# sc15i2gp/daily-ray-trace

Measured on AMD Instinct MI355X. Metric: Mpaths/s (pixels*spp/s) Cornell 1024^2 depth 8; achieved HBM GB/s % of peak, higher is better.
Workload: dtype f64

## Files before the change

daily-ray-trace_amd/csrc/drt_bvh_kernels.h:

```cpp
#pragma once

#include "drt_kernels.h"

#define BVH_LDS_STACK BVH_STACK

struct PrimaryHit
{
    int32_t index, pad;
    double  min_dist;
};

__device__ __forceinline__ void hit_point_from_scan(const SceneView &sv, const DevScene &sc, HitPoint &ip, V3 ro, V3 rd, double min_dist, int index)
{
    ip.index = index;
    if (index >= 0)
    {
        uint32_t type = sv.surf_type[index];
        uint32_t smat = sv.surf_mat[index];
        ip.position = v_sum(ro, v_mul(rd, min_dist));
        if (type == DRT_GEO_SPHERE) ip.normal = v_normalise(v_sub(ip.position, sf3(sv, SF_PX, index)));
        else ip.normal = sf3(sv, SF_NX, index);
        ip.out = v_reverse(rd);
        ip.on_dot = v_dot(ip.normal, ip.out);
        ip.transmit_mat = smat;
        ip.incident_mat = sc.base_mat;
        if (ip.on_dot < 0.0)
        {
            if (type != DRT_GEO_PLANE)
            {
                ip.transmit_mat = sc.base_mat;
                ip.incident_mat = smat;
            }
            ip.normal = v_reverse(ip.normal);
            ip.on_dot = v_dot(ip.normal, ip.out);
        }
        ip.surface_mat = smat;
    }
    else ip.surface_mat = sc.escape_mat;
}

struct PathStart
{
    uint64_t q, s_local, hit_row, slot;
    uint32_t x, y, sample;
};
template <bool LIST>
__device__ __forceinline__ PathStart path_start(const TraceParams &tp, uint64_t pid)
{
    PathStart ps;
    ps.q = pid / tp.n_samples;
    ps.s_local = pid - ps.q * tp.n_samples;
    ps.hit_row = ps.s_local * tp.n_pix + ps.q;
    const uint64_t t = LIST ? (uint64_t)tp.pixel_list[ps.q] : ps.q;
    uint32_t j = (uint32_t)(t / tp.tile_w);
    uint32_t i = (uint32_t)(t - (uint64_t)j * tp.tile_w);
    ps.x = tp.x0 + i;
    ps.y = tp.y0 + j * tp.row_stride;
    ps.sample = tp.first_sample + (uint32_t)ps.s_local;
    if (LIST) ps.sample += tp.sample_base[t];
    ps.slot = ps.q * (uint64_t)tp.batch + ps.s_local;
    return ps;
}
template <bool LIST>
__device__ __forceinline__ uint64_t path_tile_pixel(const TraceParams &tp, const PathStart &ps)
{
    return LIST ? (uint64_t)tp.pixel_list[ps.q] : ps.q;
}
__device__ __forceinline__ uint64_t path_key(const TraceParams &tp, const PathStart &ps)
{
    return tp.seed + (((uint64_t)ps.sample * (uint64_t)tp.height + (uint64_t)ps.y) * (uint64_t)tp.width + (uint64_t)ps.x);
}


#define PRIMARY_BLOCK 256

#ifndef DRT_PRIMARY_WAVES_PER_SIMD
#define DRT_PRIMARY_WAVES_PER_SIMD 6
#endif
template <bool LIST, bool RAYS>
__device__ __forceinline__ void primary_paths(DevScene sc, DevCamera cam, TraceParams tp, uint64_t *headers,
                                              int32_t *hits, unsigned long long *counters,
                                              PrimaryHit *primary, uint64_t *queue,
                                              unsigned long long *queue_count, const DevRayTable &rt)
{
    __shared__ int s_stack[PRIMARY_BLOCK / 64][BVH_LDS_STACK];
    SceneView sv;
    sv.n_surf = sc.n_surf; sv.n_lights = sc.n_lights;
    sv.surf = sc.surf; sv.lights = sc.lights; sv.surf_type = sc.surf_type; sv.surf_mat = sc.surf_mat;
    sv.light_type = sc.light_type; sv.light_mat = sc.light_mat; sv.mats = sc.mats;
    sv.bvh_nodes = sc.bvh_nodes; sv.bvh_leaf = sc.bvh_leaf;
    const uint32_t lane = threadIdx.x & 63u;
    int *stack = s_stack[threadIdx.x >> 6];
    const uint64_t n_packets = (tp.n_paths + 63u) / 64u;
    const uint64_t wave0 = (uint64_t)blockIdx.x * (PRIMARY_BLOCK / 64) + (threadIdx.x >> 6);
    const uint64_t n_waves = (uint64_t)gridDim.x * (PRIMARY_BLOCK / 64);
    uint32_t n_scans = 0, n_draws = 0, n_paths = 0;
    if (*tp.overflow) return;

    for (uint64_t packet = wave0; packet < n_packets; packet += n_waves)
    {
        const uint64_t pid = packet * 64u + lane;
        const bool valid = pid < tp.n_paths;
        V3 ro = v3(0, 0, 0), rd = v3(0, 0, 1);
        PathStart ps = path_start<LIST>(tp, valid ? pid : 0);
        uint64_t rs = 1;
        double weight = 1.0;
        if (valid)
        {
            rs = drt_splitmix64(path_key(tp, ps));
            if (RAYS) weight = table_ray(rt, tp.width, path_tile_pixel<LIST>(tp, ps), ps.x, ps.y, ps.sample, ro, rd);
            else camera_ray(cam, tp.pixel_scheme, ps.x, ps.y, rs, n_draws, ro, rd);
            n_paths += 1;
            n_scans += 1;
        }
        const V3 o = v_sum(ro, v_mul(rd, DRT_VIS_FUDGE));
        double min_dist = DRT_INF;
        int index = -1;
        const Ray32 r32 = bvh_ray32(o, rd);
        float lim = bvh_limit32(min_dist);
        int sp = 0;
        int cur = 0;
        for (;;)
        {
            cur = __builtin_amdgcn_readfirstlane(cur);
            if (cur >= 0)
            {
                const BvhNode &n = sv.bvh_nodes[cur];
                int ref[2];
                float t[2];
                bool hit[2];
                bvh_children(n, r32, lim, ref, t, hit);
                hit[0] = hit[0] && valid;
                hit[1] = hit[1] && valid;
                const unsigned long long m0 = __ballot(hit[0]), m1 = __ballot(hit[1]);
                if (m0 != 0ull && m1 != 0ull)
                {
                    const int first1 = __popcll(__ballot(hit[1] && (!hit[0] || t[1] < t[0])));
                    const int first0 = __popcll(__ballot(hit[0] && (!hit[1] || !(t[1] < t[0]))));
                    const int near = first1 > first0 ? 1 : 0;
                    if (lane == 0) stack[sp] = ref[1 - near];
                    sp += 1;
                    cur = ref[near];
                    continue;
                }
                if (m0 != 0ull) { cur = ref[0]; continue; }
                if (m1 != 0ull) { cur = ref[1]; continue; }
            }
            else if (bvh_is_leaf(cur))
            {
                const int packed = -2 - cur;
                const int first = packed >> 3, count = (packed & 7) + 1;
                for (int k = 0; k < count; k += 1)
                {
                    const BvhLeafPrim &lp = sv.bvh_leaf[first + k];
                    if (!__any(valid && !sphere_certainly_missed(lp, r32, lim))) continue;
                    double dist = leaf_distance(sv, lp, o, rd);
                    if (valid && (dist < min_dist || (dist == min_dist && (int)lp.index < index)))
// ... 118 lines not shown
    const Ray32 r32 = bvh_ray32_unpruned(o, d);
    float lim = bvh_limit32(limit);
    int sp = 0;
    int cur = job == JOB_NONE ? BVH_DONE : 0;
    int nq = 0;
    for (;;)
    {
        for (;;)
        {
            if (bvh_is_leaf(cur) && nq < DRT_BVH_POSTPONE)
            {
                leaf_queue[nq * 64 + lane] = cur;
                nq += 1;
                cur = stack_pop(stack, lane, sp);
            }
            const bool walking = cur >= 0;
            const int n_walk = __popcll(__ballot(walking));
            if (n_walk == 0) break;
            if (n_walk < DRT_BVH_POSTPONE_EXIT && __any(bvh_is_leaf(cur) && nq == DRT_BVH_POSTPONE)) break;
            if (walking) bvh_node_step(sv, stack, lane, r32, lim, cur, sp);
        }
        if (!__any(nq > 0 || cur != BVH_DONE)) break;
        int ns = 0;
        for (int k = 0; __any(k < nq); k += 1)
            if (k < nq)
            {
                const int leaf = leaf_queue[k * 64 + lane];
                const BvhLeafPrim *src = &sv.bvh_leaf[(-2 - leaf) >> 3];
                BvhLeafPrim b;
                b.c32[0] = src->c32[0]; b.c32[1] = src->c32[1]; b.c32[2] = src->c32[2]; b.reach32 = src->reach32;
                if (!sphere_certainly_missed(b, r32, lim))
                {
                    leaf_queue[ns * 64 + lane] = leaf;
                    ns += 1;
                }
            }
        nq = 0;
        for (int k = 0; __any(k < ns); k += 1)
            if (k < ns)
            {
                const BvhLeafPrim *src = &sv.bvh_leaf[(-2 - leaf_queue[k * 64 + lane]) >> 3];
                BvhLeafPrim lp;
                lp.index = src->index; lp.type = src->type;
                lp.f[0] = src->f[0]; lp.f[1] = src->f[1]; lp.f[2] = src->f[2]; lp.f[3] = src->f[3];
                const double dist = leaf_distance(sv, lp, o, d);
                if (job == JOB_CLOSEST)
                {
                    if (dist < limit || (dist == limit && (int)lp.index < index))
                    {
                        limit = dist;
                        index = (int)lp.index;
                        lim = bvh_limit32(limit);
                    }
                }
                else if (dist < limit)
                {
                    occluded = true;
                    ns = 0;
                    sp = 0;
                    cur = BVH_DONE;
                }
            }
    }
}

template <bool LIST, bool RAYS>
__device__ __forceinline__ void bounce_paths(
    DevScene sc, DevCamera cam, TraceParams tp, uint64_t *records, uint64_t *headers, int32_t *hits,
    unsigned long long *counters, unsigned long long *work_counter, const PrimaryHit *primary,
    const uint64_t *queue, const unsigned long long *queue_count, const DevRayTable &rt)
{
    __shared__ int s_stack[BOUNCE_BLOCK / 64][BVH_LDS_STACK * 64];
    __shared__ int s_leaf_queue[BOUNCE_BLOCK / 64][BVH_QUEUE_WORDS];
    SceneView sv;
    sv.n_surf = sc.n_surf; sv.n_lights = sc.n_lights;
    sv.surf = sc.surf; sv.lights = sc.lights; sv.surf_type = sc.surf_type; sv.surf_mat = sc.surf_mat;
    sv.light_type = sc.light_type; sv.light_mat = sc.light_mat; sv.mats = sc.mats;
    sv.bvh_nodes = sc.bvh_nodes; sv.bvh_leaf = sc.bvh_leaf;
    const uint32_t lane = threadIdx.x & 63u;
    int *stack = s_stack[threadIdx.x >> 6];
    int *leaf_queue = s_leaf_queue[threadIdx.x >> 6];
    if (*tp.overflow) return;
    const uint64_t n_work = *queue_count;
    const uint64_t CHUNK = tp.chunk;
    uint64_t chunk_next = 0, chunk_end = 0;
    bool exhausted = false;

    uint32_t n_scans = 0, n_shaded = 0, n_shadow = 0, n_draws = 0;

    bool alive = false, at_vertex = false;
    uint64_t rs = 1, hit_row = 0;
    uint32_t depth = 0, shaded = 0, light = 0;
    uint32_t masks = 0;
    uint64_t *hdr = nullptr;
    uint32_t blk = 0, tbl = 0;
    uint32_t spare = ~0u, spare_tbl = ~0u;
    bool new_vertex = false;
    WavePool wp = {0u, 0u, 0u};
    HitPoint ip;
    ip.position = ip.normal = ip.out = v3(0, 0, 0);
    ip.on_dot = 0.0;
    ip.surface_mat = ip.incident_mat = ip.transmit_mat = 0;
    ip.index = -1;

    const uint32_t cycle = sv.n_lights + 1u;
    uint32_t phase = 0;
    for (;;)
    {
        unsigned long long idle_mask = __ballot(!alive);
        if (!exhausted && idle_mask == ~0ull) phase = 0;
        if (idle_mask != 0ull && !exhausted && phase == 0u)
        {
            const uint32_t want = (uint32_t)__popcll(idle_mask);
            const uint32_t rank = (uint32_t)__popcll(idle_mask & ((1ull << lane) - 1ull));
            uint64_t my = ~0ull;
            uint64_t avail = chunk_end - chunk_next;
            uint32_t taken = 0;
            if (avail < want)
            {
                if (!alive && rank < avail) my = chunk_next + rank;
                taken = (uint32_t)avail;
                unsigned long long base = 0;
                if (lane == 0) base = atomicAdd(work_counter, (unsigned long long)CHUNK);
                base = __shfl(base, 0);
                if (base >= n_work)
                {
                    exhausted = true;
                    chunk_next = chunk_end = 0;
                }
                else
                {
                    chunk_next = base;
                    chunk_end = (base + CHUNK < n_work) ? base + CHUNK : n_work;
                    const uint64_t avail2 = chunk_end - chunk_next;
                    if (!alive && rank >= taken && (uint64_t)(rank - taken) < avail2) my = chunk_next + (rank - taken);
                    const uint32_t used = (want - taken < avail2) ? (want - taken) : (uint32_t)avail2;
                    chunk_next += used;
                }
            }
            else
            {
                if (!alive) my = chunk_next + rank;
                chunk_next += want;
            }
            if (my != ~0ull)
            {
                const uint64_t pid = queue[my];
                const PathStart ps = path_start<LIST>(tp, pid);
                hit_row = ps.hit_row;
                rs = drt_splitmix64(path_key(tp, ps));
                uint32_t camera_draws = 0;
                V3 ro, rd;
                if (RAYS) (void)table_ray(rt, tp.width, path_tile_pixel<LIST>(tp, ps), ps.x, ps.y, ps.sample, ro, rd);
                else camera_ray(cam, tp.pixel_scheme, ps.x, ps.y, rs, camera_draws, ro, rd);
                hdr = headers + ps.slot * REC_HEADER_WORDS;
                const PrimaryHit ph = primary[ps.slot];
                hit_point_from_scan(sv, sc, ip, v_sum(ro, v_mul(rd, DRT_VIS_FUDGE)), rd, ph.min_dist, ph.index);
                depth = 0;
                shaded = 0;
                light = 0;
                masks = 0;
                alive = true;
                at_vertex = true;
                new_vertex = true;
                n_shaded += 1;
            }
        }
        if (!__any(alive)) break;
        phase = phase + 1u == cycle ? 0u : phase + 1u;
        if (!path_spare_block(tp, wp, alive, shaded, spare, spare_tbl, lane))
        {
            hdr[0] = (uint64_t)HDR_TERM_NOT_DONE << 16;
            alive = false;
        }

        int job = JOB_NONE;
        V3 jo = v3(0, 0, 0), jd = v3(0, 0, 1);
        double limit = DRT_INF;
        double light_c = 1.0;
        if (alive && at_vertex && light < sv.n_lights)
        {
            const uint32_t l = light;
            const uint32_t ltype = sv.light_type[l];
            const V3 lpos = v3(sv.lights[LF_PX * sv.n_lights + l], sv.lights[LF_PY * sv.n_lights + l], sv.lights[LF_PZ * sv.n_lights + l]);
            const double light_pdf = sv.lights[LF_PDF * sv.n_lights + l];
            double attenuation = 1.0;
            V3 light_position = lpos;
            if (ltype == DRT_GEO_POINT)
            {
                double dist = v_length(v_sub(light_position, ip.position));
                attenuation = ((4.0 * DRT_PI) * dist) * dist;
            }
            else if (ltype == DRT_GEO_SPHERE)
            {
                double u = drt_rng(rs, n_draws);
                double v = drt_rng(rs, n_draws);
                double r = __builtin_sqrt(1.0 - u * u);
                double t = (2.0 * DRT_PI) * v;
                double st, ct;
                drt_sincos(t, st, ct);
                V3 sp = v3(r * ct, r * st, u);
                light_position = v_sum(lpos, v_mul(sp, sv.lights[LF_RADIUS * sv.n_lights + l]));
            }
            else if (ltype == DRT_GEO_PLANE)
            {
                double u = drt_rng(rs, n_draws);
                double v = drt_rng(rs, n_draws);
                V3 lu = v3(sv.lights[LF_UX * sv.n_lights + l], sv.lights[LF_UY * sv.n_lights + l], sv.lights[LF_UZ * sv.n_lights + l]);
                V3 lv = v3(sv.lights[LF_VX * sv.n_lights + l], sv.lights[LF_VY * sv.n_lights + l], sv.lights[LF_VZ * sv.n_lights + l]);
                light_position = v_sum(v_sum(lpos, v_mul(lu, u)), v_mul(lv, v));
            }
            n_shadow += 1;
            jd = v_normalise(v_sub(light_position, ip.position));
            jo = v_sum(ip.position, v_mul(jd, DRT_VIS_FUDGE));
            limit = v_length(v_sub(light_position, jo)) - DRT_VIS_FUDGE;
            light_c = attenuation * (light_pdf);
            job = JOB_SHADOW;
        }
        else if (alive && !at_vertex)
        {
            jd = ip.out;
            jo = v_sum(ip.position, v_mul(jd, DRT_VIS_FUDGE));
            job = JOB_CLOSEST;
        }
        int index = -1;
        bool occluded = false;
        bvh_walk(sv, stack, leaf_queue, lane, job, jo, jd, limit, index, occluded);

        if (job == JOB_CLOSEST)
        {
            hit_point_from_scan(sv, sc, ip, jo, jd, limit, index);
            n_scans += 1;
            if (tp.record_hits) hits[((uint64_t)tp.hits_sample_offset * tp.n_pix + hit_row) * tp.max_depth + depth] = ip.index;
            const DevMaterial &mat = sv.mats[ip.surface_mat];
            if (mat.is_black_body)
            {
                const uint32_t term = mat.is_emissive ? 1u : 0u;
                const uint32_t term_spd = mat.is_emissive ? ((uint32_t)mat.emission_spd & 0xFFFFu) : 0u;
                hdr[0] = (uint64_t)shaded | ((uint64_t)term << 16) | ((uint64_t)term_spd << 32) | ((uint64_t)(masks & 0xFFFFu) << 48) | ((uint64_t)(masks >> 16) << 24);
                alive = false;
            }
            else
            {
                at_vertex = true;
                new_vertex = true;
                light = 0;
                n_shaded += 1;
            }
        }
        else if (job == JOB_SHADOW)
        {
            const uint32_t l = light;
            if (new_vertex)
            {
                path_open_vertex(tp, wp, records, shaded, hdr, blk, tbl, spare, spare_tbl);
                new_vertex = false;
            }
            uint64_t *vrec = records + (uint64_t)blk * tp.block_words + (uint64_t)(shaded & (REC_BLOCK_VERTICES - 1u)) * tp.vertex_words;
            uint64_t *lrec = vrec + REC_VERTEX_WORDS + (uint64_t)l * REC_LIGHT_WORDS;
            uint32_t lflags = 0;
            if (!occluded)
            {
                EvalCoef e = eval_coefficients_by_material(sc, sv, ip, jd);
                lflags = e.flags | FLAG_VISIBLE;
                if (l == 0 && shaded < 8u) masks |= 0x10000u << shaded;
                lrec[1] = (uint64_t)__double_as_longlong(light_c);
                store_coef(lrec + 2, e);
            }
            uint32_t em_spd = (uint32_t)sv.mats[sv.light_mat[l]].emission_spd & 0xFFFFu;
            lrec[0] = (uint64_t)em_spd | ((uint64_t)lflags << 16);
            light = l + 1;
        }
        if (alive && at_vertex && light >= sv.n_lights)
        {
            if (new_vertex)
            {
                path_open_vertex(tp, wp, records, shaded, hdr, blk, tbl, spare, spare_tbl);
                new_vertex = false;
            }
            const DevMaterial &mat = sv.mats[ip.surface_mat];
            uint64_t *vrec = records + (uint64_t)blk * tp.block_words + (uint64_t)(shaded & (REC_BLOCK_VERTICES - 1u)) * tp.vertex_words;
            V3 in;
            double dir_pdf;
            sample_direction_by_material(sc, sv, ip, rs, n_draws, in, dir_pdf);
            EvalCoef e = eval_coefficients_by_material(sc, sv, ip, in);
            vrec[0] = mat.bdsf_packed;
            vrec[1] = (uint64_t)mat.num_bdsfs | ((uint64_t)(e.flags | mat.vertex_flags) << 8) | ((uint64_t)((uint32_t)mat.diffuse_spd & 0xFFFFu) << 16) |
                      ((uint64_t)((uint32_t)mat.glossy_spd & 0xFFFFu) << 32) | ((uint64_t)((uint32_t)mat.mirror_spd & 0xFFFFu) << 48);
            vrec[2] = record_media_word(sc, sv, ip);
            vrec[3] = (uint64_t)__double_as_longlong(ip.on_dot);
            vrec[4] = (uint64_t)__double_as_longlong(dir_pdf);
            store_coef(vrec + 5, e);
            if ((mat.vertex_flags & FLAG_PLASTIC) && shaded < 16u) masks |= 1u << shaded;
            shaded += 1;
            ip.out = in;
            depth += 1;
            at_vertex = false;
            if (depth >= tp.max_depth)
            {
                hdr[0] = (uint64_t)shaded | ((uint64_t)(masks & 0xFFFFu) << 48) | ((uint64_t)(masks >> 16) << 24);
                alive = false;
            }
        }
    }

    uint64_t vals[6] = {0, n_scans, n_shaded, n_shadow, n_draws, wp.taken};
    for (int k = 1; k < 6; k += 1)
    {
        uint64_t v = vals[k];
        for (int off = 32; off > 0; off >>= 1) v += __shfl_down(v, off);
        if (lane == 0 && v) atomicAdd(&counters[k], (unsigned long long)v);
    }
}

template <bool LIST = false>
__global__ __launch_bounds__(BOUNCE_BLOCK, DRT_BOUNCE_WAVES_PER_SIMD) void drt_bounce_kernel(
    DevScene sc, DevCamera cam, TraceParams tp, uint64_t *__restrict__ records, uint64_t *__restrict__ headers, int32_t *__restrict__ hits,
    unsigned long long *__restrict__ counters, unsigned long long *__restrict__ work_counter, const PrimaryHit *__restrict__ primary,
    const uint64_t *__restrict__ queue, const unsigned long long *__restrict__ queue_count)
{
    const DevRayTable no_table = {nullptr, nullptr, nullptr, 0u, 0u, 0u, 0u};
    bounce_paths<LIST, false>(sc, cam, tp, records, headers, hits, counters, work_counter, primary, queue, queue_count, no_table);
}

template <bool LIST = false>
__global__ __launch_bounds__(BOUNCE_BLOCK, DRT_BOUNCE_WAVES_PER_SIMD) void drt_bounce_rays_kernel(
    DevScene sc, DevCamera cam, TraceParams tp, uint64_t *__restrict__ records, uint64_t *__restrict__ headers, int32_t *__restrict__ hits,
    unsigned long long *__restrict__ counters, unsigned long long *__restrict__ work_counter, const PrimaryHit *__restrict__ primary,
    const uint64_t *__restrict__ queue, const unsigned long long *__restrict__ queue_count, DevRayTable rt)
{
    bounce_paths<LIST, true>(sc, cam, tp, records, headers, hits, counters, work_counter, primary, queue, queue_count, rt);
}
```

daily-ray-trace_amd/csrc/drt_device.h:

```cpp
#pragma once

#include <hip/hip_runtime.h>
#include <stdint.h>

#define DRT_PI 3.14159265358979323846
#define DRT_VIS_FUDGE 0.0001
#define DRT_INF __builtin_huge_val()

struct V3
{
    double x, y, z;
};
struct M33
{
    V3 c[3];
};

__device__ __forceinline__ V3 v3(double x, double y, double z) { V3 r; r.x = x; r.y = y; r.z = z; return r; }
__device__ __forceinline__ bool v_equal(V3 a, V3 b) { return a.x == b.x && a.y == b.y && a.z == b.z; }
__device__ __forceinline__ V3 v_sum(V3 a, V3 b) { return v3(a.x + b.x, a.y + b.y, a.z + b.z); }
__device__ __forceinline__ V3 v_sub(V3 a, V3 b) { return v3(a.x - b.x, a.y - b.y, a.z - b.z); }
__device__ __forceinline__ double v_dot(V3 a, V3 b) { return a.x * b.x + a.y * b.y + a.z * b.z; }
__device__ __forceinline__ V3 v_cross(V3 a, V3 b) { return v3(a.y * b.z - a.z * b.y, a.z * b.x - a.x * b.z, a.x * b.y - a.y * b.x); }
__device__ __forceinline__ V3 v_mul(V3 v, double f) { return v3(f * v.x, f * v.y, f * v.z); }
__device__ __forceinline__ V3 v_div(V3 v, double f) { return v3(v.x / f, v.y / f, v.z / f); }
__device__ __forceinline__ double v_length(V3 v) { return __builtin_sqrt(v_dot(v, v)); }
__device__ __forceinline__ V3 v_normalise(V3 v) { return v_div(v, v_length(v)); }
__device__ __forceinline__ V3 v_reverse(V3 v) { return v3(-v.x, -v.y, -v.z); }

__device__ __forceinline__ V3 v_reflect(V3 v, V3 n)
{
    double f = 2.0 * v_dot(v, n);
    return v_sub(v, v_mul(n, f));
}

__device__ __forceinline__ V3 v_transmit(V3 v, V3 n, double ir, double tr)
{
    double vn_dot = v_dot(v, n);
    double rel_ref = ir / tr;
    V3 m = v_mul(n, vn_dot);
    v = v_sub(m, v);
    V3 perpend = v_reverse(v_mul(v, rel_ref));
    double perpend_dot = -__builtin_sqrt(1.0 - v_dot(perpend, perpend));
    V3 parallel = v_mul(n, perpend_dot);
    return v_sum(perpend, parallel);
}

__device__ __forceinline__ V3 m_vmul(const M33 &m, V3 v)
{
    V3 r0 = v3(m.c[0].x, m.c[1].x, m.c[2].x);
    V3 r1 = v3(m.c[0].y, m.c[1].y, m.c[2].y);
    V3 r2 = v3(m.c[0].z, m.c[1].z, m.c[2].z);
    return v3(v_dot(r0, v), v_dot(r1, v), v_dot(r2, v));
}

__device__ __forceinline__ M33 rotation_between(V3 v, V3 w)
{
    V3 n = v_cross(v, w);
    double c = v_dot(v, w);
    M33 r;
    if (v_dot(n, n) == 0.0 && c <= 0.0)
    {
        r.c[0] = v3(-1.0, 0.0, 0.0);
        r.c[1] = v3(0.0, -1.0, 0.0);
        r.c[2] = v3(0.0, 0.0, -1.0);
        return r;
    }
    M33 m;
    m.c[0] = v3(0.0, n.z, -n.y);
    m.c[1] = v3(-n.z, 0.0, n.x);
    m.c[2] = v3(n.y, -n.x, 0.0);
    V3 row0 = v3(m.c[0].x, m.c[1].x, m.c[2].x);
    V3 row1 = v3(m.c[0].y, m.c[1].y, m.c[2].y);
    V3 row2 = v3(m.c[0].z, m.c[1].z, m.c[2].z);
    double f = 1.0 / (1.0 + c);
    V3 mm0 = v_mul(v3(v_dot(row0, m.c[0]), v_dot(row0, m.c[1]), v_dot(row0, m.c[2])), f);
    V3 mm1 = v_mul(v3(v_dot(row1, m.c[0]), v_dot(row1, m.c[1]), v_dot(row1, m.c[2])), f);
    V3 mm2 = v_mul(v3(v_dot(row2, m.c[0]), v_dot(row2, m.c[1]), v_dot(row2, m.c[2])), f);
    r.c[0] = v_sum(v_sum(v3(1.0, 0.0, 0.0), m.c[0]), mm0);
    r.c[1] = v_sum(v_sum(v3(0.0, 1.0, 0.0), m.c[1]), mm1);
    r.c[2] = v_sum(v_sum(v3(0.0, 0.0, 1.0), m.c[2]), mm2);
    return r;
}

__device__ __forceinline__ uint64_t drt_splitmix64(uint64_t k)
{
    uint64_t z = k + 0x9E3779B97F4A7C15ull;
    z = (z ^ (z >> 30)) * 0xBF58476D1CE4E5B9ull;
    z = (z ^ (z >> 27)) * 0x94D049BB133111EBull;
    z ^= z >> 31;
    return z ? z : 1ull;
}
__device__ __forceinline__ double drt_rng(uint64_t &state, uint32_t &draws)
{
    uint64_t x = state;
    x ^= x << 13;
    x ^= x >> 7;
    x ^= x << 17;
    state = x;
    draws += 1;
    return (double)(uint32_t)(x >> 33) / 2147483647.0;
}

__device__ __forceinline__ void drt_sincos(double t, double &s, double &c)
{
    const double TWO_OVER_PI = 6.36619772367581382433e-01;
    const double PIO2_1 = 1.57079632673412561417e+00, PIO2_1T = 6.07710050650619224932e-11;
    const double S1 = -1.66666666666666324348e-01, S2 = 8.33333333332248946124e-03, S3 = -1.98412698298579493134e-04,
                 S4 = 2.75573137070700676789e-06, S5 = -2.50507602534068634195e-08, S6 = 1.58969099521155010221e-10;
    const double C1 = 4.16666666666666019037e-02, C2 = -1.38888888888741095749e-03, C3 = 2.48015872894767294178e-05,
                 C4 = -2.75573143513906633035e-07, C5 = 2.08757232129817482790e-09, C6 = -1.13596475577881948265e-11;
    double fn = __builtin_rint(t * TWO_OVER_PI);
    double r = t - fn * PIO2_1;
    double w = fn * PIO2_1T;
    double y0 = r - w;
    double y1 = (r - y0) - w;
    double z = y0 * y0;
    double v = z * y0;
    double rs = S2 + z * (S3 + z * (S4 + z * (S5 + z * S6)));
    double ks = y0 - ((z * (0.5 * y1 - v * rs) - y1) - v * S1);
    double rc = z * (C1 + z * (C2 + z * (C3 + z * (C4 + z * (C5 + z * C6)))));
    double hz = 0.5 * z;
    double w1 = 1.0 - hz;
    double kc = w1 + (((1.0 - w1) - hz) + (z * rc - y0 * y1));
    int n = (int)fn & 3;
    s = (n == 0) ? ks : (n == 1) ? kc : (n == 2) ? -ks : -kc;
    c = (n == 0) ? kc : (n == 1) ? -ks : (n == 2) ? -kc : ks;
}

__device__ __forceinline__ V3 uniform_sample_sphere(uint64_t &rs, uint32_t &draws)
{
    double u = drt_rng(rs, draws);
    double v = drt_rng(rs, draws);
    double r = __builtin_sqrt(1.0 - u * u);
    double t = (2.0 * DRT_PI) * v;
    double st, ct;
    drt_sincos(t, st, ct);
    return v3(r * ct, r * st, u);
}

__device__ __forceinline__ V3 uniform_sample_disc(uint64_t &rs, uint32_t &draws)
{
    double r_x = drt_rng(rs, draws);
    double r_y = drt_rng(rs, draws);
    double o_x = 2.0 * r_x - 1.0;
    double o_y = 2.0 * r_y - 1.0;
    if (o_x == 0.0 && o_y == 0.0) return v3(0.0, 0.0, 0.0);
    double r, t;
    if (__builtin_fabs(o_x) > __builtin_fabs(o_y))
    {
        r = o_x;
        t = (DRT_PI / 4.0) * (o_y / o_x);
    }
    else
    {
        r = o_y;
        t = (DRT_PI / 2.0) - (DRT_PI / 4.0) * (o_x / o_y);
    }
    double st, ct;
    drt_sincos(t, st, ct);
    return v3(r * ct, r * st, 0.0);
}


__device__ __forceinline__ double line_sphere(V3 o, V3 d, V3 sc, double sr)
{
    V3 c_to_o = v_sub(o, sc);
    double b = -2.0 * v_dot(c_to_o, d);
    double c = v_dot(c_to_o, c_to_o) - sr * sr;
    double disc = b * b - 4.0 * c;
    if (disc < 0.0) return DRT_INF;
    double sq = __builtin_sqrt(disc);
    double s0 = (b + sq) * 0.5;
    double s1 = (b - sq) * 0.5;
    if (s0 < 0.0 && s1 < 0.0) return DRT_INF;
    else if (s0 >= 0.0 && s1 < 0.0) return s0;
    else if (s1 >= 0.0 && s0 < 0.0) return s1;
    else if (s0 <= s1) return s0;
    else return s1;
}

__device__ __forceinline__ double line_plane(V3 o, V3 d, V3 pp, V3 pn, V3 un, V3 vn, double ul, double vl)
{
    double dn = v_dot(d, pn);
    if (dn == 0.0) return DRT_INF;
    V3 o_to_p = v_sub(pp, o);
    double l = v_dot(o_to_p, pn) / dn;
    V3 i = v_sum(o, v_mul(d, l));
    V3 j = v_sub(i, pp);
    double ju = v_dot(j, un);
    double jv = v_dot(j, vn);
    if (l >= 0.0 && 0.0 <= ju && ju <= ul && 0.0 <= jv && jv <= vl) return l;
    return DRT_INF;
}

__device__ __forceinline__ double line_plane_limited(V3 o, V3 d, V3 pp, V3 pn, V3 un, V3 vn, double ul, double vl, double limit, bool want)
{
    double dn = v_dot(d, pn);
    if (dn == 0.0) return DRT_INF;
    V3 o_to_p = v_sub(pp, o);
    double l = v_dot(o_to_p, pn) / dn;
    if (!(want && l >= 0.0 && l < limit)) return DRT_INF;
    V3 i = v_sum(o, v_mul(d, l));
    V3 j = v_sub(i, pp);
    double ju = v_dot(j, un);
    double jv = v_dot(j, vn);
    if ((0.0 <= ju) & (ju <= ul) & (0.0 <= jv) & (jv <= vl)) return l;
    return DRT_INF;
}

__device__ __forceinline__ uint32_t media_index(bool swapped, bool incident, uint32_t surface_mat, uint32_t base_mat)
{
    return (swapped == incident) ? surface_mat : base_mat;
}

__device__ __forceinline__ double drt_pow_shininess(double x, double y)
{
    const uint32_t n = (uint32_t)y;
    if (!(y >= 0.0 && y < 1024.0 && (double)n == y) || !(x >= 0.0 && x <= 1.0)) return pow(x, y);
    double rh = 1.0, rl = 0.0;
    double bh = x, bl = 0.0;
    double yk = y;
    asm volatile("" : "+v"(yk));
    for (uint32_t k = (uint32_t)yk; __any(k != 0u); k >>= 1)
    {
        if (k & 1u)
        {
            const double p = rh * bh;
            double e = __builtin_fma(rh, bh, -p);
            e = __builtin_fma(rh, bl, e);
            e = __builtin_fma(rl, bh, e);
            rh = p + e;
            rl = e - (rh - p);
        }
        if (k > 1u)
        {
            const double p = bh * bh;
            double e = __builtin_fma(bh, bh, -p);
            e = __builtin_fma(bh + bh, bl, e);
            bh = p + e;
            bl = e - (bh - p);
        }
    }
    return rh + rl;
}


__device__ __forceinline__ double dielectric_reflectance(double ir, double tr, double inc_cos, double inc_sin_sq)
{
    double rel = ir / tr;
    double ts_sin_sq = rel * rel * inc_sin_sq;
    if (ts_sin_sq >= 1.0) return 1.0;
    double ts_cos = __builtin_sqrt(1.0 - ts_sin_sq * ts_sin_sq);
    double tr_on = tr * inc_cos;
    double tr_ts = tr * ts_cos;
    double ir_on = ir * inc_cos;
    double ir_ts = ir * ts_cos;
    double par = (tr_on - ir_ts) / (tr_on + ir_ts);
    double per = (ir_on - tr_ts) / (ir_on + tr_ts);
    par *= par;
    per *= per;
    return 0.5 * (par + per);
}

__device__ __forceinline__ double conductor_reflectance(double ir, double tr, double te, double inc_cos, double inc_cos_sq,
                                                        double inc_sin_sq)
{
    double rr = tr / ir;
    double re = te / ir;
    double rr_sq = rr * rr;
    double re_sq = re * re;
    double r = rr_sq - re_sq - inc_sin_sq;
    double apb_sq = __builtin_sqrt(r * r + 4.0 * rr_sq * re_sq);
    double a = __builtin_sqrt(0.5 * (apb_sq + r));
    double s = apb_sq + inc_cos_sq;
    double t = 2.0 * a * inc_cos;
    double u = inc_cos_sq * apb_sq + inc_sin_sq * inc_sin_sq;
    double v = t * inc_sin_sq;
    double par = (s - t) / (s + t);
    double per = par * (u - v) / (u + v);
    return 0.5 * (par + per);
}

__device__ __forceinline__ double dielectric_reflectance_sel(bool paired, double ir, double tr, double te_or_rel_sq, double inc_cos, double inc_sin_sq)
{
    double rel_sq = te_or_rel_sq;
    if (!paired)
    {
        double rel = ir / tr;
        rel_sq = rel * rel;
    }
    double ts_sin_sq = rel_sq * inc_sin_sq;
    if (ts_sin_sq >= 1.0) return 1.0;
    double ts_cos = __builtin_sqrt(1.0 - ts_sin_sq * ts_sin_sq);
    double tr_on = tr * inc_cos;
    double tr_ts = tr * ts_cos;
    double ir_on = ir * inc_cos;
    double ir_ts = ir * ts_cos;
    double par = (tr_on - ir_ts) / (tr_on + ir_ts);
    double per = (ir_on - tr_ts) / (ir_on + tr_ts);
    par *= par;
    per *= per;
    return 0.5 * (par + per);
}
__device__ __forceinline__ double conductor_reflectance_sel(bool paired, double ir_or_cA, double tr_or_cB, double te, double inc_cos, double inc_cos_sq,
                                                            double inc_sin_sq)
{
    double cA = ir_or_cA, cB = tr_or_cB;
    if (!paired)
    {
        double rr = tr_or_cB / ir_or_cA;
        double re = te / ir_or_cA;
        double rr_sq = rr * rr;
        double re_sq = re * re;
        cA = rr_sq - re_sq;
        cB = 4.0 * rr_sq * re_sq;
    }
    double r = cA - inc_sin_sq;
    double apb_sq = __builtin_sqrt(r * r + cB);
    double a = __builtin_sqrt(0.5 * (apb_sq + r));
    double s = apb_sq + inc_cos_sq;
    double t = 2.0 * a * inc_cos;
    double u = inc_cos_sq * apb_sq + inc_sin_sq * inc_sin_sq;
    double v = t * inc_sin_sq;
    double par = (s - t) / (s + t);
    double per = par * (u - v) / (u + v);
    return 0.5 * (par + per);
}

__device__ __forceinline__ double ggx(V3 sn, V3 mn, double r)
{
    double d = v_dot(sn, mn);
    double r_2 = r * r;
    if (d <= 0.0) return 0.0;
    double d_2 = d * d;
    double d_4 = d_2 * d_2;
    double tan_sq = (1.0 / d_2) - 1.0;
    return r_2 / (((DRT_PI * d_4) * (r_2 + tan_sq)) * (r_2 + tan_sq));
}
__device__ __forceinline__ double ggx_att(V3 v, V3 sn, V3 mn, double r)
{
    double att;
    double g = ggx(sn, mn, r);
    double v_mn = v_dot(v, mn);
    double v_sn = v_dot(v, sn);
    double dot_quot = __builtin_fabs(v_mn / v_sn);
    double r_2 = r * r;
    if (dot_quot <= 0.0) att = 0.0;
    else
    {
        double vn_tan_sq = (1.0 / (v_sn * v_sn)) - 1.0;
        att = 2.0 / (1.0 + __builtin_sqrt(1.0 + r_2 * vn_tan_sq));
    }
    return g * att;
}

__device__ __forceinline__ double drt_lerp(double x, double x0, double x1, double y0, double y1)
{
    return y0 + ((x - x0) * ((y1 - y0) / (x1 - x0)));
}
```

daily-ray-trace_amd/csrc/drt_kernels.h:

```cpp
#pragma once

#include "drt_device.h"
#include "drt_build_rule.h"
#include "drt_stash_rule.h"
#include <type_traits>
#include "../../include/drt_hip.h"


enum
{
    SF_PX = 0, SF_PY, SF_PZ, SF_RADIUS,
    SF_NX, SF_NY, SF_NZ,
    SF_UNX, SF_UNY, SF_UNZ,
    SF_VNX, SF_VNY, SF_VNZ,
    SF_ULEN, SF_VLEN,
    SF_COUNT
};
enum
{
    LF_PX = 0, LF_PY, LF_PZ, LF_RADIUS,
    LF_UX, LF_UY, LF_UZ,
    LF_VX, LF_VY, LF_VZ,
    LF_PDF,
    LF_COUNT
};

enum
{
    NEED_GLOSSY = 1u,
    NEED_EQR    = 2u,
    NEED_EQT    = 4u,
    NEED_CT     = 8u
};

struct BvhNode
{
    float   lo[2][3], hi[2][3];
    int32_t child[2];
    int32_t count[2];
};

struct BvhLeafPrim
{
    uint32_t index, type;
    double   f[4];
    float    c32[3];
    float    reach32;
    double   pad;
};

#define PAIR_NONE 0xFFFFu
#define PAIR_CONDUCTOR 0x8000u
struct DevMaterial
{
    uint32_t is_black_body, is_emissive, num_bdsfs, dir_func;
    uint32_t needs;
    uint16_t pair_out, pair_in;
    int32_t  emission_spd, diffuse_spd, glossy_spd, mirror_spd, refract_spd, extinct_spd;
    double   shininess, roughness;
    double   refract_i0, refract_i1;
    uint32_t bdsfs[DRT_MAX_BDSFS];
    uint64_t bdsf_packed;
    uint32_t vertex_flags;
    uint32_t pad1;
};

struct DevScene
{
    uint32_t n_surf, n_lights, n_mat, S;
    uint32_t n_spd, base_mat, escape_mat, trans_i0;
    double   trans_wl, trans_w0, trans_w1;
    const double      *surf;
    const uint32_t    *surf_type;
    const uint32_t    *surf_mat;
    const double      *lights;
    const uint32_t    *light_type;
    const uint32_t    *light_mat;
    const DevMaterial *mats;
    const double      *spds;
    const BvhNode     *bvh_nodes;
    const BvhLeafPrim *bvh_leaf;
};

struct DevCamera
{
    V3     forward, right, up, aperture_position, film_bottom_left;
    double aperture_radius, focal_depth, pixel_width, pixel_height;
};

struct DevRayTable
{
    const double *origins, *dirs;
    const double *weights;
    uint64_t      layer_stride, t_offset;
    uint32_t      n_layers, tiled;
};


#define REC_HEADER_WORDS 4
#define REC_BLOCK_SHIFT 2
#define REC_BLOCK_VERTICES (1u << REC_BLOCK_SHIFT)
#define REC_HEADER_BLOCKS 3
#define HDR_TERM_NOT_DONE 0x80u
#define HDR_TERM_TAIL_STAGED 0x40u
#define HDR_TERM_MASK 0x03u
#define HDR_TERM_RESUME_SHIFT 2u
#define HDR_TERM_RESUME_MASK 0xFu
#define REC_VERTEX_WORDS 10
#define REC_LIGHT_WORDS 6
#define FLAG_EQR 1u
#define FLAG_EQT 2u
#define FLAG_VISIBLE 4u
#define FLAG_PLASTIC 8u

struct TraceParams
{
    uint32_t width, height, x0, y0, tile_w, tile_h, row_stride;
    uint32_t first_sample, n_samples, max_depth, pixel_scheme, record_hits;
    uint64_t seed;
    uint64_t n_pix, n_paths;
    uint32_t vertex_words, block_words;
    uint32_t hits_sample_offset, batch;
    uint32_t chunk, pool_blocks;
    unsigned long long *pool_cursor;
    uint32_t *overflow;
    double       *tail_stage;
    const double *spd_tail;
    double       *tail_resume;
    uint32_t      tail_count, n_spd;
    const uint32_t *pixel_list;
    const uint32_t *sample_base;
};

#define POOL_CHUNK 256u
struct WavePool
{
    uint32_t base, left;
    uint32_t handed;
    uint32_t taken;
};

__device__ __forceinline__ uint32_t pool_alloc(const TraceParams &tp, WavePool &wp, bool need, uint32_t lane)
{
    const unsigned long long m = __ballot(need);
    if (m == 0ull) return ~0u;
    const uint32_t n = (uint32_t)__popcll(m);
    if (n > wp.left)
    {
        unsigned long long base = 0;
        if (lane == 0) base = atomicAdd(tp.pool_cursor, (unsigned long long)POOL_CHUNK);
        base = __shfl(base, 0);
        if (base + POOL_CHUNK > (unsigned long long)tp.pool_blocks)
        {
            wp.left = 0;
            return ~0u;
        }
        wp.base = (uint32_t)base;
        wp.left = POOL_CHUNK;
    }
    const uint32_t id = wp.base + (uint32_t)__popcll(m & ((1ull << lane) - 1ull));
    wp.base += n;
    wp.left -= n;
    wp.handed += n;
    return need ? id : ~0u;
}

__device__ __forceinline__ bool path_spare_block(const TraceParams &tp, WavePool &wp, bool alive, uint32_t shaded, uint32_t &spare, uint32_t &spare_tbl,
                                                 uint32_t lane)
{
    const bool want = alive && (shaded & (REC_BLOCK_VERTICES - 1u)) == 0u && spare == ~0u;
    const bool want_tbl = alive && shaded == REC_HEADER_BLOCKS * REC_BLOCK_VERTICES && spare_tbl == ~0u;
    const uint32_t id = pool_alloc(tp, wp, want, lane);
    const uint32_t tid = pool_alloc(tp, wp, want_tbl, lane);
    if (want) spare = id;
    if (want_tbl) spare_tbl = tid;
    if ((want && id == ~0u) || (want_tbl && tid == ~0u))
    {
        atomicExch(tp.overflow, 1u);
        return false;
    }
    return true;
}
__device__ __forceinline__ void path_open_vertex(const TraceParams &tp, WavePool &wp, uint64_t *__restrict__ records, uint32_t shaded, uint64_t *hdr,
                                                 uint32_t &blk, uint32_t &tbl, uint32_t &spare, uint32_t &spare_tbl)
{
    if ((shaded & (REC_BLOCK_VERTICES - 1u)) != 0u) return;
    const uint32_t b = shaded >> REC_BLOCK_SHIFT;
    blk = spare;
    spare = ~0u;
    wp.taken += 1;
    uint32_t *h32 = (uint32_t *)hdr;
    if (b < REC_HEADER_BLOCKS) h32[4 + b] = blk;
    else
    {
        if (b == REC_HEADER_BLOCKS)
        {
            tbl = spare_tbl;
            spare_tbl = ~0u;
            h32[7] = tbl;
            wp.taken += 1;
        }
        ((uint32_t *)(records + (uint64_t)tbl * tp.block_words))[b - REC_HEADER_BLOCKS] = blk;
    }
}

struct EvalCoef
{
    double   a_in, spec, mn_dot, ct_coef;
    uint32_t flags;
};

#define DRT_NUM_COUNTERS 8


struct SceneView
{
    const double      *surf;
    const uint32_t    *surf_type, *surf_mat;
    const double      *lights;
    const uint32_t    *light_type, *light_mat;
    const DevMaterial *mats;
    const BvhNode     *bvh_nodes;
    const BvhLeafPrim *bvh_leaf;
    const double      *rows = nullptr;
    uint32_t           n_surf, n_lights;
};

__device__ __forceinline__ V3 sf3(const SceneView &sv, int f, uint32_t i)
{
    return v3(sv.surf[(f + 0) * sv.n_surf + i], sv.surf[(f + 1) * sv.n_surf + i], sv.surf[(f + 2) * sv.n_surf + i]);
}

__device__ __forceinline__ double surface_distance(const SceneView &sv, uint32_t i, uint32_t type, V3 o, V3 d)
{
    if (type == DRT_GEO_SPHERE) return line_sphere(o, d, sf3(sv, SF_PX, i), sv.surf[SF_RADIUS * sv.n_surf + i]);
    return line_plane(o, d, sf3(sv, SF_PX, i), sf3(sv, SF_NX, i), sf3(sv, SF_UNX, i), sf3(sv, SF_VNX, i),
                      sv.surf[SF_ULEN * sv.n_surf + i], sv.surf[SF_VLEN * sv.n_surf + i]);
}

#define SR_STRIDE 16
#define SR_TYPE 15
static_assert(SF_COUNT <= SR_TYPE, "a surface row holds the SF_COUNT fields and the type");
__device__ __forceinline__ V3 row3(const double *r, int f) { return v3(r[f], r[f + 1], r[f + 2]); }
__device__ __forceinline__ uint32_t row_type(const double *r) { return (uint32_t)__double_as_longlong(r[SR_TYPE]); }
__device__ __forceinline__ double row_distance(const double *r, uint32_t type, V3 o, V3 d)
{
    if (type == DRT_GEO_SPHERE) return line_sphere(o, d, row3(r, SF_PX), r[SF_RADIUS]);
    return line_plane(o, d, row3(r, SF_PX), row3(r, SF_NX), row3(r, SF_UNX), row3(r, SF_VNX), r[SF_ULEN], r[SF_VLEN]);
}
template <bool ROWS>
__device__ __forceinline__ uint32_t scan_type(const SceneView &sv, uint32_t i)
{
    return ROWS ? row_type(sv.rows + (size_t)i * SR_STRIDE) : sv.surf_type[i];
}
__device__ __forceinline__ double row_distance_limited(const double *r, uint32_t type, V3 o, V3 d, double limit, bool want)
{
    if (type == DRT_GEO_SPHERE) return line_sphere(o, d, row3(r, SF_PX), r[SF_RADIUS]);
    return line_plane_limited(o, d, row3(r, SF_PX), row3(r, SF_NX), row3(r, SF_UNX), row3(r, SF_VNX), r[SF_ULEN], r[SF_VLEN], limit, want);
}
template <bool ROWS>
__device__ __forceinline__ double scan_distance(const SceneView &sv, uint32_t i, uint32_t type, V3 o, V3 d, double limit, bool want)
{
    return ROWS ? row_distance_limited(sv.rows + (size_t)i * SR_STRIDE, type, o, d, limit, want) : surface_distance(sv, i, type, o, d);
}

#ifdef DRT_BRANCH_STATS
__device__ __forceinline__ uint32_t scan_plane_step_skipped(const double *r, V3 o, V3 d, double limit, bool want)
{
    const V3 pp = row3(r, SF_PX), pn = row3(r, SF_NX);
    const double dn = v_dot(d, pn);
    const double l = v_dot(v_sub(pp, o), pn) / dn;
    return __any(dn != 0.0 && want && l >= 0.0 && l < limit) ? 0u : 1u;
}
#define DRT_SCAN_STATS_PARAM , uint64_t *scan_stats = nullptr
#define DRT_SCAN_STATS_ARG(p) , (p)
#define DRT_SCAN_STATS_STEP(rowp, o, d, limit, want)                                                                  \
    if (ROWS && scan_stats && type == DRT_GEO_PLANE)                                                                    \
    {                                                                                                                   \
        const uint32_t skipped_ = scan_plane_step_skipped((rowp), (o), (d), (limit), (want));                          \
        if ((threadIdx.x & 63u) == (uint32_t)(__ffsll((long long)__ballot(1)) - 1))                                    \
        {                                                                                                               \
            scan_stats[0] += 1;                                                                                         \
            scan_stats[1] += skipped_;                                                                                  \
        }                                                                                                               \
    }
#else
#define DRT_SCAN_STATS_PARAM
#define DRT_SCAN_STATS_ARG(p)
#define DRT_SCAN_STATS_STEP(rowp, o, d, limit, want)
#endif

#define BVH_STACK 32

__device__ __forceinline__ double leaf_distance(const SceneView &sv, const BvhLeafPrim &lp, V3 o, V3 d)
{
    if (lp.type == DRT_GEO_SPHERE) return line_sphere(o, d, v3(lp.f[SF_PX], lp.f[SF_PY], lp.f[SF_PZ]), lp.f[SF_RADIUS]);
    return surface_distance(sv, lp.index, lp.type, o, d);
}

#define BVH_INV_CAP 1.2676506e30f
struct Ray32
{
    float ix, iy, iz, nx, ny, nz;
    float ox, oy, oz, dx, dy, dz;
};
__device__ __forceinline__ float bvh_inv32(float d)
{
    const float i = __builtin_amdgcn_rcpf(d);
    return __builtin_fabsf(i) > BVH_INV_CAP ? __builtin_copysignf(BVH_INV_CAP, i) : i;
}
__device__ __forceinline__ Ray32 bvh_ray32f(V3 o, float dx, float dy, float dz)
{
    Ray32 r;
    r.ix = bvh_inv32(dx);
    r.iy = bvh_inv32(dy);
    r.iz = bvh_inv32(dz);
    r.nx = -((float)o.x * r.ix);
    r.ny = -((float)o.y * r.iy);
    r.nz = -((float)o.z * r.iz);
    r.ox = (float)o.x; r.oy = (float)o.y; r.oz = (float)o.z;
    r.dx = dx; r.dy = dy; r.dz = dz;
    return r;
}
__device__ __forceinline__ Ray32 bvh_ray32(V3 o, V3 d) { return bvh_ray32f(o, (float)d.x, (float)d.y, (float)d.z); }

#define RAY_UNIT_TOLERANCE 0x1p-42
#define BVH_WALK_UNIT_TOLERANCE 0x1p-38
__device__ __forceinline__ bool ray_off_unit(V3 d)
{
    const bool finite = __builtin_fabs(d.x) < DRT_INF && __builtin_fabs(d.y) < DRT_INF && __builtin_fabs(d.z) < DRT_INF;
    return finite && !(__builtin_fabs(v_dot(d, d) - 1.0) <= RAY_UNIT_TOLERANCE);
}
__device__ __forceinline__ Ray32 bvh_ray32_unpruned(V3 o, V3 d)
{
    const bool off = __builtin_fabs(v_dot(d, d) - 1.0) > BVH_WALK_UNIT_TOLERANCE;
    return bvh_ray32f(o, off ? INFINITY : (float)d.x, (float)d.y, (float)d.z);
}
__device__ __forceinline__ bool bvh_ray32_is_unpruned(const Ray32 &r) { return r.dx == INFINITY; }

__device__ __forceinline__ bool sphere_certainly_missed(const BvhLeafPrim &lp, const Ray32 &r, float lim)
{
    const float cx = lp.c32[0] - r.ox, cy = lp.c32[1] - r.oy, cz = lp.c32[2] - r.oz;
    const float t = __builtin_fmaf(cz, r.dz, __builtin_fmaf(cy, r.dy, cx * r.dx));
    const float px = __builtin_fmaf(-t, r.dx, cx), py = __builtin_fmaf(-t, r.dy, cy), pz = __builtin_fmaf(-t, r.dz, cz);
    const float p2 = __builtin_fmaf(pz, pz, __builtin_fmaf(py, py, px * px));
    const float R = lp.reach32;
    return (p2 > R * R || t + R < 0.0f || t - R > lim) && p2 < INFINITY;
}
__device__ __forceinline__ float bvh_limit32(double limit) { return (float)limit * 1.00000024f; }

__device__ __forceinline__ float bvh_box_entry(const BvhNode &n, int c, const Ray32 &r)
{
    float t0x = __builtin_fmaf(n.lo[c][0], r.ix, r.nx), t1x = __builtin_fmaf(n.hi[c][0], r.ix, r.nx);
    float t0y = __builtin_fmaf(n.lo[c][1], r.iy, r.ny), t1y = __builtin_fmaf(n.hi[c][1], r.iy, r.ny);
    float t0z = __builtin_fmaf(n.lo[c][2], r.iz, r.nz), t1z = __builtin_fmaf(n.hi[c][2], r.iz, r.nz);
    float tmin = __builtin_fmaxf(__builtin_fmaxf(__builtin_fminf(t0x, t1x), __builtin_fminf(t0y, t1y)), __builtin_fminf(t0z, t1z));
    float tmax = __builtin_fminf(__builtin_fminf(__builtin_fmaxf(t0x, t1x), __builtin_fmaxf(t0y, t1y)), __builtin_fmaxf(t0z, t1z));
    if (!(tmax >= 0.0f) || !(tmin <= tmax)) return -1.0f;
    return tmin > 0.0f ? tmin : 0.0f;
}

#define BVH_DONE (-1)
__device__ __forceinline__ int bvh_leaf_ref(int first, int count) { return -2 - (first * 8 + (count - 1)); }
__device__ __forceinline__ bool bvh_is_leaf(int ref) { return ref < BVH_DONE; }

template <bool UNPRUNED = false>
__device__ __forceinline__ void bvh_children(const BvhNode &n, const Ray32 &r, float limit, int ref[2], float t[2], bool hit[2])
{
#pragma unroll
    for (int c = 0; c < 2; c += 1)
    {
        ref[c] = n.child[c];
        t[c] = bvh_box_entry(n, c, r);
        if (UNPRUNED) t[c] = bvh_ray32_is_unpruned(r) ? 0.0f : t[c];
        hit[c] = ref[c] != BVH_DONE && t[c] >= 0.0f && t[c] <= limit;
    }
}

template <bool ROWS = false>
__device__ __forceinline__ bool points_mutually_visible(const SceneView &sv, V3 p0, V3 p1 DRT_SCAN_STATS_PARAM)
{
    V3 dir = v_normalise(v_sub(p1, p0));
    V3 o = v_sum(p0, v_mul(dir, DRT_VIS_FUDGE));
    double vis_dist = v_length(v_sub(p1, o)) - DRT_VIS_FUDGE;
    bool visible = true;
    for (uint32_t i = 0; i < sv.n_surf; i += 1)
    {
        uint32_t type = scan_type<ROWS>(sv, i);
        if (type != DRT_GEO_SPHERE && type != DRT_GEO_PLANE) continue;
        DRT_SCAN_STATS_STEP(sv.rows + (size_t)i * SR_STRIDE, o, dir, vis_dist, visible)
        double dist = scan_distance<ROWS>(sv, i, type, o, dir, vis_dist, visible);
        if (visible && dist < vis_dist) visible = false;
        if (!__any(visible)) break;
    }
    return visible;
}

struct HitPoint
{
    V3       position, normal, out;
    double   on_dot;
    uint32_t surface_mat, incident_mat, transmit_mat;
    int      index;
};

struct TraceHit
{
    V3       position, normal, out;
    double   on_dot;
    uint32_t surface_mat;
    bool     swapped;
    int      index;
};
__device__ __forceinline__ void hit_set_media(const DevScene &sc, HitPoint &ip, uint32_t smat, bool swapped)
{
    ip.incident_mat = media_index(swapped, true, smat, sc.base_mat);
    ip.transmit_mat = media_index(swapped, false, smat, sc.base_mat);
}
__device__ __forceinline__ void hit_set_media(const DevScene &, TraceHit &ip, uint32_t, bool swapped) { ip.swapped = swapped; }
__device__ __forceinline__ uint32_t incident_mat_of(const DevScene &, const HitPoint &ip) { return ip.incident_mat; }
__device__ __forceinline__ uint32_t transmit_mat_of(const DevScene &, const HitPoint &ip) { return ip.transmit_mat; }
__device__ __forceinline__ uint32_t incident_mat_of(const DevScene &sc, const TraceHit &ip) { return media_index(ip.swapped, true, ip.surface_mat, sc.base_mat); }
__device__ __forceinline__ uint32_t transmit_mat_of(const DevScene &sc, const TraceHit &ip) { return media_index(ip.swapped, false, ip.surface_mat, sc.base_mat); }

template <bool ROWS = false, class HP = HitPoint>
__device__ __forceinline__ void find_ray_intersection(const SceneView &sv, const DevScene &sc, HP &ip, V3 ro, V3 rd DRT_SCAN_STATS_PARAM)
{
    double min_dist = DRT_INF;
    int index = -1;
    ro = v_sum(ro, v_mul(rd, DRT_VIS_FUDGE));
    {
        for (uint32_t i = 0; i < sv.n_surf; i += 1)
        {
            uint32_t type = scan_type<ROWS>(sv, i);
            if (type != DRT_GEO_SPHERE && type != DRT_GEO_PLANE) continue;
            DRT_SCAN_STATS_STEP(sv.rows + (size_t)i * SR_STRIDE, ro, rd, min_dist, true)
            double dist = scan_distance<ROWS>(sv, i, type, ro, rd, min_dist, true);
            if (dist < min_dist)
            {
                min_dist = dist;
                index = (int)i;
            }
        }
    }
    ip.index = index;
    if (index >= 0)
    {
        uint32_t type = sv.surf_type[index];
        uint32_t smat = sv.surf_mat[index];
        ip.position = v_sum(ro, v_mul(rd, min_dist));
        if (type == DRT_GEO_SPHERE) ip.normal = v_normalise(v_sub(ip.position, sf3(sv, SF_PX, index)));
        else ip.normal = sf3(sv, SF_NX, index);
        ip.out = v_reverse(rd);
        ip.on_dot = v_dot(ip.normal, ip.out);
        hit_set_media(sc, ip, smat, false);
        if (ip.on_dot < 0.0)
        {
            if (type != DRT_GEO_PLANE) hit_set_media(sc, ip, smat, true);
            ip.normal = v_reverse(ip.normal);
            ip.on_dot = v_dot(ip.normal, ip.out);
        }
        ip.surface_mat = smat;
    }
    else ip.surface_mat = sc.escape_mat;
}

__device__ __forceinline__ double refract_at_trans_wl(const DevScene &sc, const DevMaterial &m)
{
    return drt_lerp(sc.trans_wl, sc.trans_w0, sc.trans_w1, m.refract_i0, m.refract_i1);
}

template <class HP>
__device__ __forceinline__ uint64_t record_media_word(const DevScene &sc, const SceneView &sv, const HP &ip)
{
    const DevMaterial &sm = sv.mats[ip.surface_mat];
    const uint32_t incident_mat = incident_mat_of(sc, ip), transmit_mat = transmit_mat_of(sc, ip);
    uint32_t pair = PAIR_NONE;
    if (incident_mat == sc.base_mat && transmit_mat == ip.surface_mat) pair = sm.pair_out;
    else if (incident_mat == ip.surface_mat && transmit_mat == sc.base_mat) pair = sm.pair_in;
    return (uint64_t)((uint32_t)sv.mats[incident_mat].refract_spd & 0xFFFFu) |
           ((uint64_t)((uint32_t)sv.mats[transmit_mat].refract_spd & 0xFFFFu) << 16) |
           ((uint64_t)((uint32_t)sv.mats[transmit_mat].extinct_spd & 0xFFFFu) << 32) | ((uint64_t)pair << 48);
}
__device__ __forceinline__ void fresnel_rows(uint64_t w2, uint32_t &i0, uint32_t &i1, uint32_t &i2, bool &paired)
{
    const uint32_t i_ir = (uint32_t)(w2)&0xFFFFu, i_tr = (uint32_t)(w2 >> 16) & 0xFFFFu, i_te = (uint32_t)(w2 >> 32) & 0xFFFFu;
    const uint32_t pair = (uint32_t)(w2 >> 48) & 0xFFFFu;
    paired = pair != PAIR_NONE;
    const bool conductor = paired && (pair & PAIR_CONDUCTOR) != 0u;
    const uint32_t row = pair & (PAIR_CONDUCTOR - 1u);
    i0 = conductor ? row : i_ir;
    i1 = conductor ? row + 1u : i_tr;
    i2 = (paired && !conductor) ? row : i_te;
}

struct VertexDirs
{
    V3 refl, trans;
};

__device__ __forceinline__ bool dirs_need_refl(const DevMaterial &m)
{
    return (m.needs & NEED_EQR) || m.dir_func == DRT_DIRF_sample_specular_direction || m.dir_func == DRT_DIRF_sample_reflect_or_transmit_direction;
}
__device__ __forceinline__ bool dirs_need_trans(const DevMaterial &m)
{
    return (m.needs & NEED_EQT) || m.dir_func == DRT_DIRF_sample_transmit_direction || m.dir_func == DRT_DIRF_sample_reflect_or_transmit_direction;
}

template <class HP>
__device__ __forceinline__ VertexDirs vertex_dirs(const DevScene &sc, const SceneView &sv, const HP &ip)
{
    const DevMaterial &mat = sv.mats[ip.surface_mat];
    VertexDirs vd;
    vd.refl = v3(0.0, 0.0, 0.0);
    vd.trans = v3(0.0, 0.0, 0.0);
    const V3 w = v_reverse(ip.out);
    if (dirs_need_refl(mat)) vd.refl = v_reflect(w, ip.normal);
    if (dirs_need_trans(mat))
    {
        double ir = refract_at_trans_wl(sc, sv.mats[incident_mat_of(sc, ip)]);
        double tr = refract_at_trans_wl(sc, sv.mats[transmit_mat_of(sc, ip)]);
        vd.trans = v_transmit(w, ip.normal, ir, tr);
    }
    return vd;
}

template <class HP>
__device__ __forceinline__ EvalCoef eval_coefficients(const SceneView &sv, const HP &ip, const VertexDirs &vd, V3 in)
{
    const DevMaterial &mat = sv.mats[ip.surface_mat];
    EvalCoef e;
    e.a_in = __builtin_fabs(v_dot(ip.normal, in));
    e.spec = 0.0;
    e.mn_dot = 0.0;
    e.ct_coef = 0.0;
    e.flags = 0;
    uint32_t needs = mat.needs;
    V3 half = v3(0.0, 0.0, 0.0);
    double n_half = 0.0;
    if (needs & (NEED_GLOSSY | NEED_CT))
    {
        half = v_normalise(v_sum(ip.out, in));
        n_half = v_dot(ip.normal, half);
    }
    if (needs & NEED_GLOSSY) e.spec = drt_pow_shininess((0.0 > n_half) ? 0.0 : n_half, mat.shininess);
    if ((needs & NEED_EQR) && v_equal(in, vd.refl)) e.flags |= FLAG_EQR;
    if ((needs & NEED_EQT) && v_equal(in, vd.trans)) e.flags |= FLAG_EQT;
    if (needs & NEED_CT)
    {
        e.mn_dot = __builtin_fabs(n_half);
        e.ct_coef = ggx_att(ip.out, ip.normal, half, mat.roughness) * (1.0 / (4.0 * ip.on_dot));
    }
    return e;
}

template <class HP>
__device__ __forceinline__ void sample_direction(const DevScene &sc, const SceneView &sv, const HP &ip, const VertexDirs &vd, uint64_t &rs,
                                                 uint32_t &draws, V3 &dir, double &recip_pdf)
{
    const DevMaterial &mat = sv.mats[ip.surface_mat];
    const uint32_t df = mat.dir_func;
    const bool disc = df == DRT_DIRF_cos_weighted_sample_hemisphere;
    const bool sphere = df == DRT_DIRF_uniform_sample_hemisphere;
    const bool ggx_mn = df == DRT_DIRF_sample_ct_direction;
    const bool coin = df == DRT_DIRF_sample_reflect_or_transmit_direction;
    dir = v3(0.0, 0.0, 0.0);
    recip_pdf = 0.0;
    if (df == DRT_DIRF_sample_specular_direction)
    {
        dir = vd.refl;
        recip_pdf = 1.0;
    }
    if (df == DRT_DIRF_sample_transmit_direction)
    {
        dir = vd.trans;
        recip_pdf = 1.0;
    }
    double num = 0.0, den = 1.0;
    if (coin)
    {
        const DevMaterial &im = sv.mats[incident_mat_of(sc, ip)];
        const DevMaterial &tm = sv.mats[transmit_mat_of(sc, ip)];
        double inc_sin_sq = 1.0 - ip.on_dot * ip.on_dot;
        double r0 = dielectric_reflectance(im.refract_i0, tm.refract_i0, ip.on_dot, inc_sin_sq);
        double r1 = dielectric_reflectance(im.refract_i1, tm.refract_i1, ip.on_dot, inc_sin_sq);
        double rd = drt_lerp(sc.trans_wl, sc.trans_w0, sc.trans_w1, r0, r1);
        double f = drt_rng(rs, draws);
        const bool reflect = f < rd;
        dir = reflect ? vd.refl : vd.trans;
        num = 1.0;
        den = reflect ? rd : 1.0 - rd;
    }
    if (disc || sphere || ggx_mn)
    {
        const M33 r = rotation_between(v3(0.0, 0.0, 1.0), ip.normal);
        const double rough = mat.roughness;
        bool accepted;
        double o_mn_dot = 0.0, d = 1.0;
        do
        {
            const double u = drt_rng(rs, draws);
            const double v = drt_rng(rs, draws);
            const double o_x = 2.0 * u - 1.0;
            const double o_y = 2.0 * v - 1.0;
            const bool x_major = __builtin_fabs(o_x) > __builtin_fabs(o_y);
            const double sqrt_u = __builtin_sqrt(sphere ? 1.0 - u * u : u);
            const double q_num = ggx_mn ? rough * sqrt_u : (x_major ? o_y : o_x);
            const double q_den = ggx_mn ? __builtin_sqrt(1.0 - u) : (x_major ? o_x : o_y);
            const double q = q_num / q_den;
            double t = x_major ? (DRT_PI / 4.0) * q : (DRT_PI / 2.0) - (DRT_PI / 4.0) * q;
            if (!disc) t = (2.0 * DRT_PI) * v;
            double radius = x_major ? o_x : o_y;
            double z = u;
            if (sphere) radius = sqrt_u;
            if (ggx_mn)
            {
                const double cos_mn = 1.0 / __builtin_sqrt(1.0 + q * q);
                radius = __builtin_sqrt(1.0 - cos_mn * cos_mn);
                z = cos_mn;
            }
            double st, ct;
            drt_sincos(t, st, ct);
            V3 p = v3(radius * ct, radius * st, 0.0);
            if (disc)
            {
                if (o_x == 0.0 && o_y == 0.0) p = v3(0.0, 0.0, 0.0);
                const double qq = v_dot(p, p);
                accepted = qq < 1.0;
                z = __builtin_sqrt(1.0 - qq);
            }
            p.z = z;
            V3 w = m_vmul(r, p);
            dir = w;
            if (sphere)
            {
                recip_pdf = 2.0 * DRT_PI;
                accepted = true;
            }
            if (ggx_mn)
            {
                double sn_mn_dot = v_dot(ip.normal, w);
                if (sn_mn_dot < 0.0)
                {
                    w = v_reverse(w);
                    sn_mn_dot = -sn_mn_dot;
                }
                o_mn_dot = v_dot(ip.out, w);
                dir = v_reflect(v_reverse(ip.out), w);
                d = ggx(ip.normal, w, rough) * sn_mn_dot;
                accepted = !(v_dot(dir, ip.normal) < 0.0);
            }
        } while (!accepted);
        if (disc)
        {
            num = DRT_PI;
            den = v_dot(ip.normal, dir);
        }
        if (ggx_mn)
        {
            num = 4.0 * o_mn_dot;
            den = d;
        }
    }
    if (disc || ggx_mn || coin) recip_pdf = num / den;
}

__device__ __forceinline__ EvalCoef eval_coefficients_by_material(const DevScene &sc, const SceneView &sv, const HitPoint &ip, V3 in)
{
    const DevMaterial &mat = sv.mats[ip.surface_mat];
    EvalCoef e;
    e.a_in = __builtin_fabs(v_dot(ip.normal, in));
    e.spec = 0.0;
    e.mn_dot = 0.0;
    e.ct_coef = 0.0;
    e.flags = 0;
    uint32_t needs = mat.needs;
    if (needs & NEED_GLOSSY)
    {
        V3 bisector = v_normalise(v_sum(ip.out, in));
        double nb = v_dot(ip.normal, bisector);
        e.spec = drt_pow_shininess((0.0 > nb) ? 0.0 : nb, mat.shininess);
    }
    if (needs & NEED_EQR)
    {
        if (v_equal(in, v_reflect(v_reverse(ip.out), ip.normal))) e.flags |= FLAG_EQR;
    }
    if (needs & NEED_EQT)
    {
        double ir = refract_at_trans_wl(sc, sv.mats[ip.incident_mat]);
        double tr = refract_at_trans_wl(sc, sv.mats[ip.transmit_mat]);
        if (v_equal(in, v_transmit(v_reverse(ip.out), ip.normal, ir, tr))) e.flags |= FLAG_EQT;
    }
    if (needs & NEED_CT)
    {
        V3 micro_normal = v_normalise(v_sum(ip.out, in));
        e.mn_dot = __builtin_fabs(v_dot(ip.normal, micro_normal));
        e.ct_coef = ggx_att(ip.out, ip.normal, micro_normal, mat.roughness) * (1.0 / (4.0 * ip.on_dot));
    }
    return e;
}

__device__ __forceinline__ void sample_direction_by_material(const DevScene &sc, const SceneView &sv, const HitPoint &ip, uint64_t &rs,
                                                 uint32_t &draws, V3 &dir, double &recip_pdf)
{
    const DevMaterial &mat = sv.mats[ip.surface_mat];
    const V3 zaxis = v3(0.0, 0.0, 1.0);
    switch (mat.dir_func)
    {
        case DRT_DIRF_cos_weighted_sample_hemisphere:
        {
            V3 q;
            for (;;)
            {
                q = uniform_sample_disc(rs, draws);
                if (v_dot(q, q) < 1.0) break;
            }
            q.z = __builtin_sqrt(1.0 - v_dot(q, q));
            M33 r = rotation_between(zaxis, ip.normal);
            dir = m_vmul(r, q);
            recip_pdf = DRT_PI / v_dot(ip.normal, dir);
            break;
        }
        case DRT_DIRF_uniform_sample_hemisphere:
        {
            V3 s = uniform_sample_sphere(rs, draws);
            M33 r = rotation_between(zaxis, ip.normal);
            dir = m_vmul(r, s);
            recip_pdf = 2.0 * DRT_PI;
            break;
        }
        case DRT_DIRF_sample_specular_direction:
        {
            dir = v_reflect(v_reverse(ip.out), ip.normal);
            recip_pdf = 1.0;
            break;
        }
        case DRT_DIRF_sample_transmit_direction:
        {
            double ir = refract_at_trans_wl(sc, sv.mats[ip.incident_mat]);
            double tr = refract_at_trans_wl(sc, sv.mats[ip.transmit_mat]);
            dir = v_transmit(v_reverse(ip.out), ip.normal, ir, tr);
            recip_pdf = 1.0;
            break;
        }
        case DRT_DIRF_sample_reflect_or_transmit_direction:
        {
            const DevMaterial &im = sv.mats[ip.incident_mat];
            const DevMaterial &tm = sv.mats[ip.transmit_mat];
            double inc_sin_sq = 1.0 - ip.on_dot * ip.on_dot;
            double r0 = dielectric_reflectance(im.refract_i0, tm.refract_i0, ip.on_dot, inc_sin_sq);
            double r1 = dielectric_reflectance(im.refract_i1, tm.refract_i1, ip.on_dot, inc_sin_sq);
            double rd = drt_lerp(sc.trans_wl, sc.trans_w0, sc.trans_w1, r0, r1);
            double ir = refract_at_trans_wl(sc, im);
            double tr = refract_at_trans_wl(sc, tm);
            double f = drt_rng(rs, draws);
            V3 w = v_reverse(ip.out);
            if (f < rd)
            {
                dir = v_reflect(w, ip.normal);
                recip_pdf = 1.0 / rd;
            }
            else
            {
                dir = v_transmit(w, ip.normal, ir, tr);
                recip_pdf = 1.0 / (1.0 - rd);
            }
            break;
        }
        case DRT_DIRF_sample_ct_direction:
        {
            do
            {
                double f = drt_rng(rs, draws);
                double g = drt_rng(rs, draws);
                double phi_mn = (2.0 * DRT_PI) * g;
                double tan_mn = (mat.roughness * __builtin_sqrt(f)) / __builtin_sqrt(1.0 - f);
                double cos_mn = 1.0 / __builtin_sqrt(1.0 + tan_mn * tan_mn);
                double sin_mn = __builtin_sqrt(1.0 - cos_mn * cos_mn);
                double sp, cp;
                drt_sincos(phi_mn, sp, cp);
                V3 micro_normal = v3(sin_mn * cp, sin_mn * sp, cos_mn);
                M33 r = rotation_between(zaxis, ip.normal);
                micro_normal = m_vmul(r, micro_normal);
                double sn_mn_dot = v_dot(ip.normal, micro_normal);
                if (sn_mn_dot < 0.0)
                {
                    micro_normal = v_reverse(micro_normal);
                    sn_mn_dot = -sn_mn_dot;
                }
                double o_mn_dot = v_dot(ip.out, micro_normal);
                dir = v_reflect(v_reverse(ip.out), micro_normal);
                double d = ggx(ip.normal, micro_normal, mat.roughness) * sn_mn_dot;
                recip_pdf = ((4.0 * o_mn_dot) / d);
            } while (v_dot(dir, ip.normal) < 0.0);
            break;
        }
        default:
            dir = v3(0.0, 0.0, 0.0);
            recip_pdf = 0.0;
            break;
    }
}

__device__ __forceinline__ void store_coef(uint64_t *w, const EvalCoef &e)
{
    w[0] = (uint64_t)__double_as_longlong(e.a_in);
    w[1] = (uint64_t)__double_as_longlong(e.spec);
    w[2] = (uint64_t)__double_as_longlong(e.mn_dot);
    w[3] = (uint64_t)__double_as_longlong(e.ct_coef);
}

__device__ __forceinline__ void camera_ray(const DevCamera &cam, uint32_t scheme, uint32_t x, uint32_t y, uint64_t &rs,
                                           uint32_t &draws, V3 &ro, V3 &rd)
{
    double px = 0.0, py = 0.0;
    if (scheme == DRT_FILM_SAMPLE_CENTER) { px = 0.5; py = 0.5; }
    else if (scheme == DRT_FILM_SAMPLE_RANDOM) { px = drt_rng(rs, draws); py = drt_rng(rs, draws); }
    double film_x = ((double)x + px) * cam.pixel_width;
    double film_y = ((double)y + py) * cam.pixel_height;
    V3 bottom = v_mul(cam.up, film_y);
    V3 left = v_mul(cam.right, film_x);
    V3 pixel_point = v_sum(v_sum(left, bottom), cam.film_bottom_left);
    if (cam.aperture_radius > 0.0)
    {
        V3 focus_dir = v_normalise(v_sub(cam.aperture_position, pixel_point));
        focus_dir = v_mul(focus_dir, cam.focal_depth / v_dot(focus_dir, cam.forward));
        V3 focus_point = v_sum(pixel_point, focus_dir);
        M33 r = rotation_between(v3(0.0, 0.0, 1.0), cam.forward);
        V3 disc_point = v_mul(uniform_sample_disc(rs, draws), cam.aperture_radius);
        V3 lens_point = m_vmul(r, disc_point);
        ro = v_sum(cam.aperture_position, lens_point);
        rd = v_normalise(v_sub(focus_point, ro));
    }
    else
    {
        ro = pixel_point;
        rd = v_normalise(v_sub(cam.aperture_position, ro));
    }
}

__device__ __forceinline__ double table_ray(const DevRayTable &rt, uint32_t width, uint64_t t, uint32_t x, uint32_t y, uint32_t sample,
                                            V3 &ro, V3 &rd)
{
    const uint32_t l = sample % rt.n_layers;
    const uint64_t r = (uint64_t)l * rt.layer_stride + (rt.tiled ? rt.t_offset + t : (uint64_t)y * (uint64_t)width + (uint64_t)x);
    const double *o = rt.origins + 3u * r, *d = rt.dirs + 3u * r;
    ro = v3(o[0], o[1], o[2]);
    rd = v3(d[0], d[1], d[2]);
    return rt.weights ? rt.weights[r] : 1.0;
}

struct PathPos
{
    uint64_t q;
    uint32_t s;
};
__device__ __forceinline__ PathPos path_pos_of_id(uint64_t id, uint32_t n_samples)
{
    PathPos p;
    p.q = id / n_samples;
    p.s = (uint32_t)(id - p.q * n_samples);
    return p;
}
__device__ __forceinline__ PathPos path_pos_step(PathPos p, uint32_t r, uint32_t n_samples)
{
    const uint32_t room = n_samples - p.s;
    if (r < room) p.s += r;
    else
    {
        const uint32_t over = r - room;
        uint32_t dq = 0u;
        if (over >= n_samples) dq = over / n_samples;
        p.q += 1u + dq;
        p.s = over - dq * n_samples;
    }
    return p;
}
__device__ __forceinline__ void tile_pixel_ij(uint64_t t, uint32_t tile_w, uint32_t &i, uint32_t &j)
{
    if (t <= 0xFFFFFFFFull)
    {
        const uint32_t t32 = (uint32_t)t;
        j = t32 / tile_w;
        i = t32 - j * tile_w;
    }
    else
    {
        j = (uint32_t)(t / tile_w);
        i = (uint32_t)(t - (uint64_t)j * tile_w);
    }
}


#define TRACE_BLOCK 256

struct TraceConst
{
    DevScene    sc;
    DevCamera   cam;
    TraceParams tp;
    uint64_t           *records, *headers;
    int32_t            *hits;
    unsigned long long *counters, *work_counter;
};
static_assert(sizeof(DevScene) % 8 == 0 && sizeof(DevCamera) % 8 == 0 && sizeof(TraceParams) % 8 == 0,
              "TraceConst mirrors the kernarg segment only while every argument ends on an 8-byte boundary");
struct TraceRaysConst
{
    TraceConst  k;
    DevRayTable rt;
};
static_assert(sizeof(TraceConst) % 8 == 0 && sizeof(DevRayTable) % 8 == 0, "the table follows the last pointer without padding");
#ifndef DRT_TRACE_CONST
#define DRT_TRACE_CONST 2
#endif
#if DRT_TRACE_CONST == 1
#define TRACE_CONST_BYTES ((sizeof(TraceConst) + 127u) & ~(size_t)127u)
#else
#define TRACE_CONST_BYTES ((size_t)0)
#endif
__device__ __forceinline__ uint32_t pinned_scalar(uint32_t v)
{
    asm volatile("" : "+s"(v));
    return v;
}
__device__ __forceinline__ const TraceConst &trace_const(const double *lds)
{
#if DRT_TRACE_CONST == 2
    uint32_t off = 0;
    asm volatile("" : "+s"(off));
    return *(const TraceConst *)((const char *)__builtin_amdgcn_kernarg_segment_ptr() + off);
#else
    uint32_t off = 0;
    asm volatile("" : "+v"(off));
    return *(const TraceConst *)((const char *)lds + off);
#endif
}
#define TRACE_LANE_ROWS 2u
#define TRACE_LW_BLK 0u
#define TRACE_LW_DRAWS 1u
#define TRACE_LW_SCANS 128u
#define TRACE_LW_SHADED 129u
__device__ __forceinline__ void lane_word_add(uint32_t *w, uint32_t v)
{
    (void)__hip_atomic_fetch_add(w, v, __ATOMIC_RELAXED, __HIP_MEMORY_SCOPE_WAVEFRONT);
}
#define TRACE_ST_OX 0u
#define TRACE_ST_DX 3u
#define TRACE_ST_RS 6u
#define TRACE_ST_VIG 7u
#define TRACE_ST_Q 8u
#define TRACE_ST_SD 9u
#define TRACE_STASH_ROWS 10u
#define TRACE_STASH_WAVE_WORDS (TRACE_STASH_ROWS * 64u + 2u)
#define TRACE_STASH_BYTES ((size_t)(TRACE_BLOCK / 64) * TRACE_STASH_WAVE_WORDS * 8u)
#define DRT_TRACE_TAIL_MAX 8u
#ifndef DRT_TRACE_WAVES_PER_SIMD
#define DRT_TRACE_WAVES_PER_SIMD 3
#endif


#ifdef DRT_BRANCH_STATS
#define DRT_BS_WORDS 23
__device__ unsigned long long drt_branch_stats[DRT_BS_WORDS];
__device__ unsigned int drt_branch_waves_done;
#endif

template <bool SCENE_IN_LDS, bool TAIL, bool LIST, bool RAYS, bool STASH>
__device__ __forceinline__ void trace_paths_form(DevScene k_sc, DevCamera k_cam, TraceParams k_tp,
                                            uint64_t *records, uint64_t *headers,
                                            int32_t *k_hits, unsigned long long *k_counters,
                                            unsigned long long *k_work_counter, const DevRayTable &k_rt)
{
    extern __shared__ double lds_raw[];
#if DRT_TRACE_CONST == 1
    if (threadIdx.x == 0)
    {
        TraceConst *c = (TraceConst *)lds_raw;
        c->sc = k_sc;
        c->cam = k_cam;
        c->tp = k_tp;
        c->hits = k_hits;
        c->counters = k_counters;
        c->work_counter = k_work_counter;
    }
#endif
#if DRT_TRACE_CONST == 0
    const TraceConst k_all = {k_sc, k_cam, k_tp, records, headers, k_hits, k_counters, k_work_counter};
#define LC k_all
#else
#define LC trace_const(lds_raw)
#endif
#if DRT_TRACE_CONST == 2
#define LC_RT (((const TraceRaysConst &)trace_const(lds_raw)).rt)
#else
#define LC_RT k_rt
#endif
    SceneView sv;
    double *l_spd_tail = nullptr, *tail_state = nullptr;
    double *lane_area = nullptr;
    double *stash = nullptr;
    uint32_t *lane_words = nullptr;
    uint32_t TR, max_depth, vertex_words, block_words;
    bool tail_on, record_hits;
    {
    const DevScene &sc = k_sc;
    const TraceParams &tp = k_tp;
    sv.n_surf = sc.n_surf;
    sv.n_lights = sc.n_lights;
    if (SCENE_IN_LDS)
    {
        double *l_rows = lds_raw + TRACE_CONST_BYTES / 8;
        double *l_surf = l_rows + (size_t)SR_STRIDE * sc.n_surf;
        for (uint32_t k = threadIdx.x; k < SR_STRIDE * sc.n_surf; k += TRACE_BLOCK)
        {
            const uint32_t i = k / SR_STRIDE, f = k % SR_STRIDE;
            l_rows[k] = f < SF_COUNT ? sc.surf[f * sc.n_surf + i] : f == SR_TYPE ? __longlong_as_double((long long)sc.surf_type[i]) : 0.0;
        }
        double *l_lights = l_surf + (size_t)SF_COUNT * sc.n_surf;
        uint32_t *l_u32 = (uint32_t *)(l_lights + (size_t)LF_COUNT * sc.n_lights);
        uint32_t n_u32 = 2 * sc.n_surf + 2 * sc.n_lights;
        DevMaterial *l_mats = (DevMaterial *)((char *)l_u32 + (((size_t)n_u32 * 4 + 7) & ~(size_t)7));
        for (uint32_t k = threadIdx.x; k < SF_COUNT * sc.n_surf; k += TRACE_BLOCK) l_surf[k] = sc.surf[k];
        for (uint32_t k = threadIdx.x; k < LF_COUNT * sc.n_lights; k += TRACE_BLOCK) l_lights[k] = sc.lights[k];
        for (uint32_t k = threadIdx.x; k < sc.n_surf; k += TRACE_BLOCK)
        {
            l_u32[k] = sc.surf_type[k];
            l_u32[sc.n_surf + k] = sc.surf_mat[k];
        }
        for (uint32_t k = threadIdx.x; k < sc.n_lights; k += TRACE_BLOCK)
        {
            l_u32[2 * sc.n_surf + k] = sc.light_type[k];
            l_u32[2 * sc.n_surf + sc.n_lights + k] = sc.light_mat[k];
        }
        const uint64_t *src = (const uint64_t *)sc.mats;
        uint64_t *dst = (uint64_t *)l_mats;
        for (uint32_t k = threadIdx.x; k < sc.n_mat * (uint32_t)(sizeof(DevMaterial) / 8); k += TRACE_BLOCK) dst[k] = src[k];
        __syncthreads();
        sv.surf = l_surf;
        sv.lights = l_lights;
        sv.surf_type = l_u32;
        sv.surf_mat = l_u32 + sc.n_surf;
        sv.light_type = l_u32 + 2 * sc.n_surf;
        sv.light_mat = l_u32 + 2 * sc.n_surf + sc.n_lights;
        sv.mats = l_mats;
        sv.rows = l_rows;
        sv.bvh_nodes = nullptr;
        sv.bvh_leaf = nullptr;
    }
    else
    {
        sv.surf = sc.surf;
        sv.lights = sc.lights;
        sv.surf_type = sc.surf_type;
        sv.surf_mat = sc.surf_mat;
        sv.light_type = sc.light_type;
        sv.light_mat = sc.light_mat;
        sv.mats = sc.mats;
        sv.bvh_nodes = sc.bvh_nodes;
        sv.bvh_leaf = sc.bvh_leaf;
        __syncthreads();
    }

    TR = tp.tail_count;
    tail_on = TAIL && SCENE_IN_LDS && tp.tail_stage != nullptr;
    lane_area = SCENE_IN_LDS ? (double *)(sv.mats + sc.n_mat) : lds_raw + TRACE_CONST_BYTES / 8;
    if (tail_on)
    {
        l_spd_tail = lane_area;
        for (uint32_t k = threadIdx.x; k < tp.n_spd * TR; k += TRACE_BLOCK) l_spd_tail[k] = tp.spd_tail[k];
        lane_area += (size_t)tp.n_spd * TR;
    }
    if (STASH) stash = lane_area + (size_t)(TRACE_BLOCK / 64) * ((TRACE_LANE_ROWS + (tail_on ? 1u + 2u * TR : 0u)) * 64u) + (size_t)(threadIdx.x >> 6) * TRACE_STASH_WAVE_WORDS;
    lane_area += (size_t)(threadIdx.x >> 6) * ((TRACE_LANE_ROWS + (tail_on ? 1u + 2u * TR : 0u)) * 64u) + (threadIdx.x & 63u);
    lane_words = (uint32_t *)lane_area;
    lane_words[TRACE_LW_BLK] = 0u;
    lane_words[TRACE_LW_DRAWS] = 0u;
    lane_words[TRACE_LW_SCANS] = 0u;
    lane_words[TRACE_LW_SHADED] = 0u;
    if (tail_on)
    {
        tail_state = lane_area + (TRACE_LANE_ROWS + 1u) * 64u;
        __syncthreads();
    }
    max_depth = tp.max_depth;
    vertex_words = tp.vertex_words;
    block_words = tp.block_words;
    record_hits = tp.record_hits != 0u;
    if (*tp.overflow) return;
    }
    bool tail_ok = false;
    const uint32_t lane = threadIdx.x & 63u;
    uint64_t chunk_next = 0, chunk_end = 0;
    PathPos chunk_pos = {0, 0};
    StashState st = {0u, 0u};

    uint32_t w_paths = 0;
#ifdef DRT_BRANCH_STATS
    uint64_t bs[DRT_BS_WORDS] = {};
#endif

    bool alive = false;
    bool exhausted = false;
    uint64_t rs = 1, hit_row = 0;
    uint32_t depth = 0, shaded = 0;
    uint32_t vis0_mask = 0;
    uint32_t plastic_mask = 0;
    V3 ro = v3(0, 0, 0), rd = v3(0, 0, 0);
    uint64_t *hdr = nullptr;
    uint32_t tbl = 0;
    uint32_t spare = ~0u, spare_tbl = ~0u;
    WavePool wp = {0u, 0u, 0u, 0u};

    for (;;)
    {
        unsigned long long idle_mask = __ballot(!alive);
        if constexpr (STASH)
        {
        if (idle_mask != 0ull && !exhausted)
        {
            const uint32_t want = (uint32_t)__popcll(idle_mask);
            const uint32_t rank = (uint32_t)__popcll(idle_mask & ((1ull << lane) - 1ull));
            bool started = false;
            auto pick = [&](uint32_t entry) __attribute__((always_inline)) {
                const TraceConst &c = LC;
                const double *e = stash + entry;
                ro = v3(e[(TRACE_ST_OX + 0u) * 64u], e[(TRACE_ST_OX + 1u) * 64u], e[(TRACE_ST_OX + 2u) * 64u]);
                rd = v3(e[(TRACE_ST_DX + 0u) * 64u], e[(TRACE_ST_DX + 1u) * 64u], e[(TRACE_ST_DX + 2u) * 64u]);
                rs = (uint64_t)__double_as_longlong(e[TRACE_ST_RS * 64u]);
                const double vignette = e[TRACE_ST_VIG * 64u];
                const uint64_t q = (uint64_t)__double_as_longlong(e[TRACE_ST_Q * 64u]);
                const uint64_t sd = (uint64_t)__double_as_longlong(e[TRACE_ST_SD * 64u]);
                const uint64_t s_local = sd & 0xFFFFFFFFull;
                lane_word_add(lane_words + TRACE_LW_DRAWS, (uint32_t)(sd >> 32));
                if (record_hits) hit_row = s_local * c.tp.n_pix + q;
                const uint64_t slot = q * (uint64_t)c.tp.batch + s_local;
                hdr = headers + slot * REC_HEADER_WORDS;
                hdr[1] = (uint64_t)__double_as_longlong(vignette);
                if (tail_on) lane_area[TRACE_LANE_ROWS * 64u] = vignette;
                started = true;
            };
            const int32_t e1 = stash_first_entry(st, want, rank);
            if (!alive && e1 >= 0) pick((uint32_t)e1);
            const uint32_t take1 = stash_after_first(st, want);
            if (take1 < want)
            {
                uint64_t *pos_slot = (uint64_t *)(stash + TRACE_STASH_ROWS * 64u);
                if (chunk_next == chunk_end)
                {
                    const TraceConst &c = LC;
                    const uint64_t CHUNK = c.tp.chunk, n_paths_all = c.tp.n_paths;
                    unsigned long long base = 0;
                    if (lane == 0) base = atomicAdd(c.work_counter, (unsigned long long)CHUNK);
                    base = (unsigned long long)(uint32_t)__builtin_amdgcn_readfirstlane((int)(uint32_t)base) |
                           ((unsigned long long)(uint32_t)__builtin_amdgcn_readfirstlane((int)(uint32_t)(base >> 32)) << 32);
                    if (base >= n_paths_all)
                    {
                        exhausted = true;
                        chunk_next = chunk_end = 0;
                    }
                    else
                    {
                        chunk_next = base;
                        chunk_end = (base + CHUNK < n_paths_all) ? base + CHUNK : n_paths_all;
                        const PathPos p0 = path_pos_of_id(base, c.tp.n_samples);
                        if (lane == 0)
                        {
                            pos_slot[0] = p0.q;
                            pos_slot[1] = (uint64_t)p0.s;
                        }
                        __builtin_amdgcn_fence(__ATOMIC_SEQ_CST, "wavefront");
                        __builtin_amdgcn_wave_barrier();
                    }
                }
                if (!exhausted)
                {
                    const uint32_t n = stash_fill_size(chunk_next, chunk_end);
                    PathPos from;
                    from.q = pos_slot[0];
                    from.s = (uint32_t)pos_slot[1];
                    const uint32_t n_samples = LC.tp.n_samples;
                    if (lane < n)
                    {
                        const TraceConst &c = LC;
                        const PathPos me = path_pos_step(from, lane, n_samples);
                        const uint64_t q = me.q;
                        const uint64_t s_local = me.s;
                        const uint64_t t = LIST ? (uint64_t)c.tp.pixel_list[q] : q;
                        uint32_t i, j;
                        tile_pixel_ij(t, c.tp.tile_w, i, j);
                        const uint32_t x = c.tp.x0 + i;
// ... 106 lines not shown
                        ahead = rank - taken;
                    }
                    uint32_t used = (want - taken < avail2) ? (want - taken) : (uint32_t)avail2;
                    chunk_next += used;
                    chunk_pos = path_pos_step(chunk_pos, used, n_samples);
                }
            }
            else
            {
                if (!alive) alive = true;
                chunk_next += want;
                chunk_pos = path_pos_step(chunk_pos, want, n_samples);
            }
            bool started = alive && ((idle_mask >> lane) & 1ull);
            w_paths += (uint32_t)__popcll(__ballot(started));
#ifdef DRT_BRANCH_STATS
            {
                const unsigned long long m_started = __ballot(started);
                if (m_started != 0ull && lane == 0u)
                {
                    bs[20] += 1;
                    bs[21] += __popcll(m_started);
                }
            }
#endif
            if (started)
            {
                const TraceConst &c = LC;
                const PathPos me = path_pos_step(from, ahead, n_samples);
                const uint64_t q = me.q;
                const uint64_t s_local = me.s;
                if (record_hits) hit_row = s_local * c.tp.n_pix + q;
                const uint64_t t = LIST ? (uint64_t)c.tp.pixel_list[q] : q;
                uint32_t i, j;
                tile_pixel_ij(t, c.tp.tile_w, i, j);
                uint32_t x = c.tp.x0 + i;
                uint32_t y = c.tp.y0 + j * c.tp.row_stride;
                uint32_t sample = c.tp.first_sample + (uint32_t)s_local;
                if (LIST) sample += c.tp.sample_base[t];
                uint64_t key = c.tp.seed + (((uint64_t)sample * (uint64_t)c.tp.height + (uint64_t)y) * (uint64_t)c.tp.width + (uint64_t)x);
                rs = drt_splitmix64(key);
                double weight = 1.0;
                if (RAYS) weight = table_ray(LC_RT, c.tp.width, t, x, y, sample, ro, rd);
                else
                {
                    uint32_t drawn = 0;
                    camera_ray(c.cam, c.tp.pixel_scheme, x, y, rs, drawn, ro, rd);
                    lane_word_add(lane_words + TRACE_LW_DRAWS, drawn);
                }
                depth = 0;
                shaded = 0;
                plastic_mask = 0;
                vis0_mask = 0;
                tail_ok = tail_on;
                if (tail_on)
                {
                    const uint32_t tr = pinned_scalar(TR);
#pragma unroll
                    for (uint32_t j = 0; j < DRT_TRACE_TAIL_MAX; j += 1)
                    {
                        if (j >= tr) break;
                        tail_state[(2u * j) * 64u] = 1.0;
                        tail_state[(2u * j + 1u) * 64u] = 0.0;
                    }
                }
                uint64_t slot = q * (uint64_t)c.tp.batch + s_local;
                hdr = headers + slot * REC_HEADER_WORDS;
                const double vignette = (RAYS ? weight : v_dot(rd, c.cam.forward)) * 1.0;
                hdr[1] = (uint64_t)__double_as_longlong(vignette);
                if (tail_on) lane_area[TRACE_LANE_ROWS * 64u] = vignette;
                if (record_hits)
                {
                    int32_t *h = c.hits + ((uint64_t)c.tp.hits_sample_offset * c.tp.n_pix + hit_row) * max_depth;
                    for (uint32_t d = 0; d < max_depth; d += 1) h[d] = -2;
                }
            }
        }
        if (!__any(alive)) break;
#ifdef DRT_BRANCH_STATS
        if (lane == 0u) bs[22] += 1;
#endif

        if (!path_spare_block(LC.tp, wp, alive, shaded, spare, spare_tbl, lane))
        {
            hdr[0] = (uint64_t)HDR_TERM_NOT_DONE << 16;
            alive = false;
            lane_word_add(lane_words + TRACE_LW_SCANS, depth);
            lane_word_add(lane_words + TRACE_LW_SHADED, shaded);
        }
        if (alive)
        {
            TraceHit ip;
            find_ray_intersection<SCENE_IN_LDS>(sv, LC.sc, ip, ro, rd DRT_SCAN_STATS_ARG(bs + 16));
            if (record_hits)
            {
                const TraceConst &c = LC;
                c.hits[((uint64_t)c.tp.hits_sample_offset * c.tp.n_pix + hit_row) * max_depth + depth] = ip.index;
            }
            const DevMaterial &mat = sv.mats[ip.surface_mat];
            bool terminal = false;
            uint32_t term = 0, term_spd = 0;
            if (mat.is_black_body && !mat.is_emissive) terminal = true;
            else if (mat.is_black_body && mat.is_emissive)
            {
                terminal = true;
                term = 1;
                term_spd = (uint32_t)mat.emission_spd;
            }
            else
            {
                uint32_t blk = lane_words[TRACE_LW_BLK];
                path_open_vertex(LC.tp, wp, records, shaded, hdr, blk, tbl, spare, spare_tbl);
                lane_words[TRACE_LW_BLK] = blk;
                uint64_t *vrec = records + (uint64_t)blk * block_words + (uint64_t)(shaded & (REC_BLOCK_VERTICES - 1u)) * vertex_words;
                const VertexDirs vd = vertex_dirs(LC.sc, sv, ip);
                bool t_vis = false;
                double t_c = 0.0, t_a_in = 0.0, t_spec = 0.0;
                uint32_t t_em = 0, t_flags = 0;
                for (uint32_t l = 0; l < sv.n_lights; l += 1)
                {
                    uint32_t ltype = sv.light_type[l];
                    V3 lpos = v3(sv.lights[LF_PX * sv.n_lights + l], sv.lights[LF_PY * sv.n_lights + l], sv.lights[LF_PZ * sv.n_lights + l]);
                    double light_pdf = sv.lights[LF_PDF * sv.n_lights + l];
                    double attenuation = 1.0;
                    V3 light_position = lpos;
                    if (ltype == DRT_GEO_POINT)
                    {
                        double dist = v_length(v_sub(light_position, ip.position));
                        attenuation = ((4.0 * DRT_PI) * dist) * dist;
                    }
                    else if (ltype == DRT_GEO_SPHERE)
                    {
                        uint32_t drawn = 0;
                        double u = drt_rng(rs, drawn);
                        double v = drt_rng(rs, drawn);
                        lane_word_add(lane_words + TRACE_LW_DRAWS, drawn);
                        double r = __builtin_sqrt(1.0 - u * u);
                        double t = (2.0 * DRT_PI) * v;
                        double st, ct;
                        drt_sincos(t, st, ct);
                        V3 sp = v3(r * ct, r * st, u);
                        light_position = v_sum(lpos, v_mul(sp, sv.lights[LF_RADIUS * sv.n_lights + l]));
                    }
                    else if (ltype == DRT_GEO_PLANE)
                    {
                        uint32_t drawn = 0;
                        double u = drt_rng(rs, drawn);
                        double v = drt_rng(rs, drawn);
                        lane_word_add(lane_words + TRACE_LW_DRAWS, drawn);
                        V3 lu = v3(sv.lights[LF_UX * sv.n_lights + l], sv.lights[LF_UY * sv.n_lights + l], sv.lights[LF_UZ * sv.n_lights + l]);
                        V3 lv = v3(sv.lights[LF_VX * sv.n_lights + l], sv.lights[LF_VY * sv.n_lights + l], sv.lights[LF_VZ * sv.n_lights + l]);
                        light_position = v_sum(v_sum(lpos, v_mul(lu, u)), v_mul(lv, v));
                    }
                    bool visible = points_mutually_visible<SCENE_IN_LDS>(sv, ip.position, light_position DRT_SCAN_STATS_ARG(bs + 18));
                    uint64_t *lrec = vrec + REC_VERTEX_WORDS + (uint64_t)l * REC_LIGHT_WORDS;
                    uint32_t lflags = 0;
                    if (visible)
                    {
                        V3 incoming = v_normalise(v_sub(light_position, ip.position));
                        EvalCoef e = eval_coefficients(sv, ip, vd, incoming);
                        lflags = e.flags | FLAG_VISIBLE;
                        if (l == 0 && shaded < 8u) vis0_mask |= 1u << shaded;
                        double c = attenuation * (light_pdf);
                        lrec[1] = (uint64_t)__double_as_longlong(c);
                        store_coef(lrec + 2, e);
                        if (l == 0) { t_vis = true; t_c = c; t_a_in = e.a_in; t_spec = e.spec; t_flags = e.flags; }
                    }
                    uint32_t em_spd = (uint32_t)sv.mats[sv.light_mat[l]].emission_spd & 0xFFFFu;
                    lrec[0] = (uint64_t)em_spd | ((uint64_t)lflags << 16);
                    if (l == 0) t_em = em_spd;
                }
                V3 in;
                double dir_pdf;
                uint32_t drawn = 0;
                sample_direction(LC.sc, sv, ip, vd, rs, drawn, in, dir_pdf);
                lane_word_add(lane_words + TRACE_LW_DRAWS, drawn);
                EvalCoef e = eval_coefficients(sv, ip, vd, in);
#ifdef DRT_BRANCH_STATS
                {
                    const uint32_t df = mat.dir_func;
                    const bool in_loop = df == DRT_DIRF_cos_weighted_sample_hemisphere || df == DRT_DIRF_uniform_sample_hemisphere ||
                                         df == DRT_DIRF_sample_ct_direction;
                    const unsigned long long m_all = __ballot(1);
                    const unsigned long long m_disc = __ballot(df == DRT_DIRF_cos_weighted_sample_hemisphere);
                    const unsigned long long m_ggx = __ballot(df == DRT_DIRF_sample_ct_direction);
                    const unsigned long long m_coin = __ballot(df == DRT_DIRF_sample_reflect_or_transmit_direction);
                    const unsigned long long m_spec = __ballot(df == DRT_DIRF_sample_specular_direction);
                    const unsigned long long m_loop = __ballot(in_loop);
                    const unsigned long long m_again = __ballot(in_loop && drawn > 2u);
                    const unsigned long long m_half = __ballot((mat.needs & (NEED_GLOSSY | NEED_CT)) != 0u);
                    const unsigned long long m_eqt = __ballot((mat.needs & NEED_EQT) != 0u);
                    if (lane == (uint32_t)(__ffsll((long long)m_all) - 1))
                    {
                        bs[0] += 1;
                        bs[1] += __popcll(m_all);
                        bs[2] += m_disc != 0ull;
                        bs[3] += __popcll(m_disc);
                        bs[4] += m_ggx != 0ull;
                        bs[5] += __popcll(m_ggx);
                        bs[6] += m_coin != 0ull;
                        bs[7] += __popcll(m_coin);
                        bs[8] += m_spec != 0ull;
                        bs[9] += __popcll(m_spec);
                        bs[10] += (m_disc != 0ull && m_ggx != 0ull && m_coin != 0ull && m_spec != 0ull);
                        bs[11] += m_loop != 0ull;
                        bs[12] += m_again != 0ull;
                        bs[13] += m_half != 0ull;
                        bs[14] += m_eqt != 0ull;
                        bs[15] += (m_disc == m_all || m_ggx == m_all || m_coin == m_all || m_spec == m_all);
                    }
                }
#endif
                if (tail_ok)
                {
                    if (mat.vertex_flags & FLAG_PLASTIC)
                    {
                        const double *row_d = l_spd_tail + ((uint32_t)mat.diffuse_spd & 0xFFFFu) * TR;
                        const double *row_g = l_spd_tail + ((uint32_t)mat.glossy_spd & 0xFFFFu) * TR;
                        const double *row_e = l_spd_tail + t_em * TR;
                        const uint32_t tr = pinned_scalar(TR);
#pragma unroll
                        for (uint32_t j = 0; j < DRT_TRACE_TAIL_MAX; j += 1)
                        {
                            if (j >= tr) break;
                            const double diffuse_pi = row_d[j], glossy = row_g[j];
                            double throughput = tail_state[(2u * j) * 64u], dst = tail_state[(2u * j + 1u) * 64u];
                            double contribution = 0.0;
                            if (t_vis)
                            {
                                double reflectance = diffuse_pi * t_a_in + 0.0;
                                reflectance = (glossy * t_spec) * t_a_in + reflectance;
                                contribution = contribution + reflectance;
                                contribution = contribution * row_e[j];
                                contribution = contribution * t_c;
                            }
                            dst = dst + throughput * contribution;
                            double reflectance = diffuse_pi * e.a_in + 0.0;
                            reflectance = (glossy * e.spec) * e.a_in + reflectance;
                            reflectance = reflectance * dir_pdf;
                            throughput = throughput * reflectance;
                            tail_state[(2u * j) * 64u] = throughput;
                            tail_state[(2u * j + 1u) * 64u] = dst;
                        }
                    }
                    else if (mat.num_bdsfs == 1u && mat.bdsfs[0] == DRT_BDSF_mirror_bdsf)
                    {
                        const double *row_m = l_spd_tail + ((uint32_t)mat.mirror_spd & 0xFFFFu) * TR;
                        const double *row_e = l_spd_tail + t_em * TR;
                        const uint32_t tr = pinned_scalar(TR);
#pragma unroll
                        for (uint32_t j = 0; j < DRT_TRACE_TAIL_MAX; j += 1)
                        {
                            if (j >= tr) break;
                            const double mirror = row_m[j];
                            double throughput = tail_state[(2u * j) * 64u], dst = tail_state[(2u * j + 1u) * 64u];
                            double contribution = 0.0;
                            if (t_vis)
                            {
                                double bdsf_result = (t_flags & FLAG_EQR) ? mirror : 0.0;
                                double reflectance = bdsf_result + 0.0;
                                contribution = contribution + reflectance;
                                contribution = contribution * row_e[j];
                                contribution = contribution * t_c;
                            }
                            dst = dst + throughput * contribution;
                            double bdsf_result = (e.flags & FLAG_EQR) ? mirror : 0.0;
                            double reflectance = bdsf_result + 0.0;
                            reflectance = reflectance * dir_pdf;
                            throughput = throughput * reflectance;
                            tail_state[(2u * j) * 64u] = throughput;
                            tail_state[(2u * j + 1u) * 64u] = dst;
                        }
                    }
                    else
                    {
                        tail_ok = false;
                        if (shaded <= HDR_TERM_RESUME_MASK) plastic_mask |= shaded << 16;
                    }
                }
                vrec[0] = mat.bdsf_packed;
                vrec[1] = (uint64_t)mat.num_bdsfs | ((uint64_t)(e.flags | mat.vertex_flags) << 8) | ((uint64_t)((uint32_t)mat.diffuse_spd & 0xFFFFu) << 16) |
                          ((uint64_t)((uint32_t)mat.glossy_spd & 0xFFFFu) << 32) | ((uint64_t)((uint32_t)mat.mirror_spd & 0xFFFFu) << 48);
                vrec[2] = record_media_word(LC.sc, sv, ip);
                vrec[3] = (uint64_t)__double_as_longlong(ip.on_dot);
                vrec[4] = (uint64_t)__double_as_longlong(dir_pdf);
                store_coef(vrec + 5, e);
                if ((mat.vertex_flags & FLAG_PLASTIC) && shaded < 16u) plastic_mask |= 1u << shaded;
                shaded += 1;
                rd = in;
                ro = ip.position;
            }
            depth += 1;
            if (terminal || depth >= max_depth)
            {
                uint32_t staged = 0;
                if (tail_ok)
                {
                    const double vignette = lane_area[TRACE_LANE_ROWS * 64u];
                    double *st = LC.tp.tail_stage + (uint64_t)(hdr - headers) / REC_HEADER_WORDS * TR;
                    const double *row_t = l_spd_tail + (term_spd & 0xFFFFu) * TR;
                    const uint32_t tr = pinned_scalar(TR);
#pragma unroll
                    for (uint32_t j = 0; j < DRT_TRACE_TAIL_MAX; j += 1)
                    {
                        if (j >= tr) break;
                        double dst = tail_state[(2u * j + 1u) * 64u];
                        if (term == 1) dst = dst + tail_state[(2u * j) * 64u] * row_t[j];
                        st[j] = dst * vignette;
                    }
                    staged = HDR_TERM_TAIL_STAGED;
                }
                else if (TAIL && (plastic_mask >> 16) != 0u)
// ... 1290 lines not shown
        next += n;
    }
}

__global__ void drt_selftest_kernel(int op, const double *a, const double *b, double *out, uint64_t n)
{
    uint64_t i = (uint64_t)blockIdx.x * blockDim.x + threadIdx.x;
    if (i >= n) return;
    switch (op)
    {
        case 0: out[i] = __builtin_sqrt(a[i]); break;
        case 1: out[i] = a[i] / b[i]; break;
        case 2:
        {
            double s, c;
            drt_sincos(a[i], s, c);
            out[2 * i] = s;
            out[2 * i + 1] = c;
            break;
        }
        case 3: out[i] = pow(a[i], b[i]); break;
        case 7: out[i] = drt_pow_shininess(a[i], b[i]); break;
        case 4:
        {
            uint64_t key = (uint64_t)__double_as_longlong(a[i]);
            uint64_t rs = drt_splitmix64(key);
            uint32_t draws = 0;
            double v = 0.0;
            for (int k = 0; k < 4; k += 1) v = drt_rng(rs, draws);
            out[i] = v;
            break;
        }
        case 5:
        case 6:
        {
            double x = a[i], y = b[i];
            if (op == 5 || (threadIdx.x & 63u) < 5u)
            {
                for (int k = 0; k < 65536; k += 1) x = __builtin_fma(x, y, 1.0e-3);
            }
            out[i] = x;
            break;
        }
        default: out[i] = 0.0; break;
    }
}

enum
{
    DRT_UNIT_LINE_SPHERE = 0,
    DRT_UNIT_LINE_PLANE,
    DRT_UNIT_REFLECT,
    DRT_UNIT_TRANSMIT,
    DRT_UNIT_ROTATION_BETWEEN,
    DRT_UNIT_SAMPLE_SPHERE,
    DRT_UNIT_SAMPLE_DISC,
    DRT_UNIT_GGX,
    DRT_UNIT_GGX_ATT,
    DRT_UNIT_FS_DIELECTRIC,
    DRT_UNIT_FS_CONDUCTOR,
    DRT_UNIT_SEED_AND_DRAW,
    DRT_UNIT_BVH_BOX,
    DRT_UNIT_LINE_PLANE_LIMITED,
    DRT_UNIT_BVH_SPHERE,
    DRT_UNIT_COUNT
};

__global__ void drt_unit_kernel(int func, const double *__restrict__ in, uint32_t in_stride, double *__restrict__ out,
                                uint32_t out_stride, uint64_t n)
{
    uint64_t i = (uint64_t)blockIdx.x * blockDim.x + threadIdx.x;
    if (i >= n) return;
    const double *a = in + i * in_stride;
    double *o = out + i * out_stride;
    auto V = [&](int k) { return v3(a[k], a[k + 1], a[k + 2]); };
    auto put = [&](int k, V3 v) { o[k] = v.x; o[k + 1] = v.y; o[k + 2] = v.z; };
    switch (func)
    {
        case DRT_UNIT_LINE_SPHERE: o[0] = line_sphere(V(0), V(3), V(6), a[9]); break;
        case DRT_UNIT_LINE_PLANE:
        {
            V3 u = V(12), v = V(15);
            double ul = v_length(u), vl = v_length(v);
            o[0] = line_plane(V(0), V(3), V(6), V(9), v_div(u, ul), v_div(v, vl), ul, vl);
            break;
        }
        case DRT_UNIT_REFLECT: put(0, v_reflect(V(0), V(3))); break;
        case DRT_UNIT_TRANSMIT: put(0, v_transmit(V(0), V(3), a[6], a[7])); break;
        case DRT_UNIT_ROTATION_BETWEEN:
        {
            M33 m = rotation_between(V(0), V(3));
            put(0, m.c[0]); put(3, m.c[1]); put(6, m.c[2]);
            break;
        }
        case DRT_UNIT_SAMPLE_SPHERE:
        case DRT_UNIT_SAMPLE_DISC:
        {
            uint64_t rs = (uint64_t)__double_as_longlong(a[0]);
            uint32_t draws = 0;
            put(0, func == DRT_UNIT_SAMPLE_SPHERE ? uniform_sample_sphere(rs, draws) : uniform_sample_disc(rs, draws));
            o[3] = __longlong_as_double((long long)rs);
            break;
        }
        case DRT_UNIT_GGX: o[0] = ggx(V(0), V(3), a[6]); break;
        case DRT_UNIT_GGX_ATT: o[0] = ggx_att(V(0), V(3), V(6), a[9]); break;
        case DRT_UNIT_FS_DIELECTRIC: o[0] = dielectric_reflectance(a[0], a[1], a[2], 1.0 - a[2] * a[2]); break;
        case DRT_UNIT_FS_CONDUCTOR:
        {
            double c2 = a[3] * a[3];
            o[0] = conductor_reflectance(a[0], a[1], a[2], a[3], c2, 1.0 - c2);
            break;
        }
        case DRT_UNIT_SEED_AND_DRAW:
        {
            uint64_t rs = drt_splitmix64((uint64_t)__double_as_longlong(a[0]));
            uint32_t draws = 0;
            o[0] = __longlong_as_double((long long)rs);
            o[1] = drt_rng(rs, draws);
            break;
        }
        case DRT_UNIT_BVH_BOX:
        {
            BvhNode n;
            for (int k = 0; k < 3; k += 1)
            {
                n.lo[0][k] = (float)a[6 + k];
                n.hi[0][k] = (float)a[9 + k];
            }
            o[0] = (double)bvh_box_entry(n, 0, bvh_ray32(V(0), V(3)));
            break;
        }
        case DRT_UNIT_LINE_PLANE_LIMITED:
        {
            V3 u = V(12), v = V(15);
            double ul = v_length(u), vl = v_length(v);
            o[0] = line_plane_limited(V(0), V(3), V(6), V(9), v_div(u, ul), v_div(v, vl), ul, vl, a[18], a[19] != 0.0);
            break;
        }
        case DRT_UNIT_BVH_SPHERE:
        {
            BvhLeafPrim lp;
            for (int k = 0; k < 3; k += 1) lp.c32[k] = (float)a[6 + k];
            lp.reach32 = bvh_sphere_reach32(a[9], a[10]);
            o[0] = sphere_certainly_missed(lp, bvh_ray32(V(0), V(3)), bvh_limit32(a[11])) ? 1.0 : 0.0;
            o[1] = line_sphere(V(0), V(3), V(6), a[9]);
            break;
        }
        default: break;
    }
}

enum
{
    DRT_MAT_EVALUATE = 0,
    DRT_MAT_SAMPLE,
    DRT_MAT_COUNT
};
#define DRT_MAT_EVAL_IN 18
#define DRT_MAT_SAMPLE_IN 15
#define DRT_MAT_SAMPLE_OUT 6
#define DRT_MAT_MODE_UNPAIRED 1u
#define DRT_MAT_MODE_SIMPLE 2u
#define DRT_MAT_VARIANTS (DRT_NUM_BDSFS + DRT_NUM_DIRFS)

__global__ void drt_material_kernel(DevScene sc, const DevMaterial *__restrict__ variants, int func, const double *__restrict__ in,
                                    uint32_t in_stride, double *__restrict__ out, uint32_t out_stride, uint64_t n)
{
    uint64_t i = (uint64_t)blockIdx.x * blockDim.x + threadIdx.x;
    if (i >= n) return;
    const double *a = in + i * in_stride;
    double *o = out + i * out_stride;
    SceneView sv;
    sv.surf = sc.surf;
    sv.lights = sc.lights;
    sv.surf_type = sc.surf_type;
    sv.surf_mat = sc.surf_mat;
    sv.light_type = sc.light_type;
    sv.light_mat = sc.light_mat;
    sv.bvh_nodes = sc.bvh_nodes;
    sv.bvh_leaf = sc.bvh_leaf;
    sv.n_surf = sc.n_surf;
    sv.n_lights = sc.n_lights;
    HitPoint ip;
    ip.position = v3(a[0], a[1], a[2]);
    ip.normal = v3(a[3], a[4], a[5]);
    ip.out = v3(a[6], a[7], a[8]);
    ip.on_dot = a[9];
    ip.surface_mat = (uint32_t)a[10];
    ip.incident_mat = (uint32_t)a[11];
    ip.transmit_mat = (uint32_t)a[12];
    ip.index = 0;
    const int sel = (int)a[13];
    if (func == DRT_MAT_SAMPLE)
    {
        sv.mats = sel < 0 ? sc.mats : variants + (uint64_t)(DRT_NUM_BDSFS + sel) * sc.n_mat;
        uint64_t rs = (uint64_t)__double_as_longlong(a[14]);
        uint32_t draws = 0;
        V3 dir;
        double recip_pdf;
        sample_direction(sc, sv, ip, vertex_dirs(sc, sv, ip), rs, draws, dir, recip_pdf);
        o[0] = dir.x; o[1] = dir.y; o[2] = dir.z;
        o[3] = recip_pdf;
        o[4] = __longlong_as_double((long long)rs);
        o[5] = (double)draws;
        return;
    }
    sv.mats = sel < 0 ? sc.mats : variants + (uint64_t)sel * sc.n_mat;
    const uint32_t mode = (uint32_t)a[17];
    const V3 incoming = v3(a[14], a[15], a[16]);
    const DevMaterial &mat = sv.mats[ip.surface_mat];
    const EvalCoef e = eval_coefficients(sv, ip, vertex_dirs(sc, sv, ip), incoming);
    uint64_t w2 = record_media_word(sc, sv, ip);
    if (mode & DRT_MAT_MODE_UNPAIRED) w2 |= (uint64_t)PAIR_NONE << 48;
    const uint32_t flags = e.flags | mat.vertex_flags;
    uint32_t i_ir, i_tr, i_te;
    bool paired;
    fresnel_rows(w2, i_ir, i_tr, i_te, paired);
    const uint32_t i_diffuse = (uint32_t)mat.diffuse_spd & 0xFFFFu, i_glossy = (uint32_t)mat.glossy_spd & 0xFFFFu;
    const uint32_t i_mirror = (uint32_t)mat.mirror_spd & 0xFFFFu;
    const bool simple = (mode & DRT_MAT_MODE_SIMPLE) != 0u;
    for (uint32_t lam = 0; lam < sc.S; lam += 1)
    {
        const double diffuse = spd_at(sc.spds, sc.S, i_diffuse, lam), glossy = spd_at(sc.spds, sc.S, i_glossy, lam);
        const double mirror = spd_at(sc.spds, sc.S, i_mirror, lam);
        double r;
        if (simple) r = bdsf_at_wavelength<true>(mat.bdsf_packed, mat.num_bdsfs, diffuse, glossy, mirror, 0.0, 0.0, 0.0, ip.on_dot, e.a_in,
                                                 e.spec, e.mn_dot, e.ct_coef, flags, paired);
        else
        {
            const double ir = spd_at(sc.spds, sc.S, i_ir, lam), tr = spd_at(sc.spds, sc.S, i_tr, lam), te = spd_at(sc.spds, sc.S, i_te, lam);
            r = bdsf_at_wavelength<false>(mat.bdsf_packed, mat.num_bdsfs, diffuse, glossy, mirror, ir, tr, te, ip.on_dot, e.a_in, e.spec,
                                          e.mn_dot, e.ct_coef, flags, paired);
        }
        o[lam] = r;
    }
    o[sc.S] = (double)e.flags;
}
```

daily-ray-trace_amd/csrc/drt_launcher.hip:

```cpp
#include "drt_kernels.h"
#include "drt_bvh_kernels.h"
#include "drt_adaptive_kernels.h"
#include "drt_sample_map_kernels.h"
#include "drt_denoise_kernels.h"
#include "drt_feature_kernels.h"
#include "drt_matte_kernels.h"
#include "drt_ray_kernels.h"
#include "drt_update_kernels.h"
#include "drt_build_kernels.h"
#include "drt_material_kernels.h"
#include "drt_depth_kernels.h"
#include "drt_window_kernels.h"
#include "drt_window_rule.h"
#include "drt_pair_rule.h"
#include "drt_owned.h"

#include <algorithm>
#include <cmath>
#include <cstdarg>
#include <cstdio>
#include <cstdlib>
#include <cstring>
#include <map>
#include <string>
// ... 5118 lines not shown

#define BUILD_SELFTEST_MAX (1u << 24)
#define BUILD_SELFTEST_GUARD 64u

extern "C" int drt_selftest_build_sort(int device, const uint64_t *keys, uint32_t m, uint64_t *keys_out, uint32_t *pos_out)
{
    g_last_error.clear();
    if (!keys || !keys_out || !pos_out) return fail(-1, "drt_selftest_build_sort: null argument");
    if (m == 0u || m > BUILD_SELFTEST_MAX) return fail(-1, "drt_selftest_build_sort: %u keys, not in 1..%u", m, BUILD_SELFTEST_MAX);
    for (uint32_t k = 0; k < m; k += 1)
        if (keys[k] > BUILD_KEY_UNBOUNDED) return fail(-1, "drt_selftest_build_sort: key %u has bit 63 set", k);
    HIP_TRY(hipSetDevice(device));
    const size_t G = BUILD_SELFTEST_GUARD, room = (size_t)m + 2 * G;
    const uint64_t key_guard = 0xA5A5A5A5A5A5A5A5ull;
    const uint32_t pos_guard = 0xA5A5A5A5u;
    std::vector<uint64_t> hk(room, key_guard);
    std::vector<uint32_t> hp(room, pos_guard);
    DevBuf<uint64_t> dk[2];
    DevBuf<uint32_t> dp[2], d_table;
    uint64_t *d_keys[2];
    uint32_t *d_pos[2];
    for (int k = 0; k < 2; k += 1)
    {
        HIP_TRY(dk[k].need(room));
        HIP_TRY(dp[k].need(room));
        HIP_TRY(hipMemcpy(dk[k], hk.data(), room * sizeof(uint64_t), hipMemcpyHostToDevice));
        HIP_TRY(hipMemcpy(dp[k], hp.data(), room * sizeof(uint32_t), hipMemcpyHostToDevice));
        d_keys[k] = dk[k] + G;
        d_pos[k] = dp[k] + G;
    }
    HIP_TRY(d_table.need((size_t)SORT_DIGITS * ((m + SORT_TILE - 1) / SORT_TILE)));
    for (uint32_t k = 0; k < m; k += 1) hp[G + k] = k;
    HIP_TRY(hipMemcpy(d_keys[0], keys, (size_t)m * sizeof(uint64_t), hipMemcpyHostToDevice));
    HIP_TRY(hipMemcpy(d_pos[0], hp.data() + G, (size_t)m * sizeof(uint32_t), hipMemcpyHostToDevice));
    int rc = hierarchy_enqueue_sort(0, d_keys, d_pos, d_table, m);
    if (rc) return rc;
    HIP_TRY(hipDeviceSynchronize());
    for (int k = 0; k < 2; k += 1)
    {
        HIP_TRY(hipMemcpy(hk.data(), dk[k], room * sizeof(uint64_t), hipMemcpyDeviceToHost));
        HIP_TRY(hipMemcpy(hp.data(), dp[k], room * sizeof(uint32_t), hipMemcpyDeviceToHost));
        for (size_t g = 0; g < G; g += 1)
            if (hk[g] != key_guard || hk[G + m + g] != key_guard || hp[g] != pos_guard || hp[G + m + g] != pos_guard)
                return fail(-3, "drt_selftest_build_sort: buffer %d was written outside its %u elements", k, m);
    }
    HIP_TRY(hipMemcpy(keys_out, d_keys[0], (size_t)m * sizeof(uint64_t), hipMemcpyDeviceToHost));
    HIP_TRY(hipMemcpy(pos_out, d_pos[0], (size_t)m * sizeof(uint32_t), hipMemcpyDeviceToHost));
    return 0;
}

extern "C" int drt_selftest_live_resources(uint64_t out[4])
{
    g_last_error.clear();
    if (!out) return fail(-1, "drt_selftest_live_resources: null argument");
    out[0] = DeviceMem::live();
    out[1] = PinnedMem::live();
    out[2] = Event::live();
    out[3] = Stream::live();
    return 0;
}

extern "C" int drt_selftest_build_topology(int device, const uint64_t *sorted_keys, uint32_t m, int32_t *child, int32_t *count, uint32_t *level_count,
                                           uint32_t *levels_out)
{
    g_last_error.clear();
    if (!sorted_keys || !child || !count || !level_count || (m > 2u && !levels_out)) return fail(-1, "drt_selftest_build_topology: null argument");
    if (m < 2u || m > BUILD_SELFTEST_MAX) return fail(-1, "drt_selftest_build_topology: %u keys, not in 2..%u (a build launches nothing below 2)", m, BUILD_SELFTEST_MAX);
    for (uint32_t k = 0; k < m; k += 1)
        if (sorted_keys[k] > BUILD_KEY_UNBOUNDED || (k > 0u && sorted_keys[k - 1] > sorted_keys[k]))
            return fail(-1, "drt_selftest_build_topology: key %u is out of order or has bit 63 set", k);
    HIP_TRY(hipSetDevice(device));
    DevBuf<uint64_t> d_keys;
    DevBuf<uint32_t> d_same, d_type, d_leaf_parent, d_order;
    DevBuf<BvhNode> d_nodes;
    DevBuf<BvhLeafPrim> d_leaf;
    DevBuf<uint2> d_levels;
    DevBuf<uint4> d_items[2];
    DevBuf<unsigned char> d_status;
    HIP_TRY(d_keys.need(m));
    HIP_TRY(d_same.need(m));
    HIP_TRY(d_type.need(m));
    HIP_TRY(d_leaf_parent.need(m));
    HIP_TRY(d_order.need(m));
    HIP_TRY(d_nodes.need((size_t)m - 1));
    HIP_TRY(d_leaf.need(m));
    HIP_TRY(d_levels.need((size_t)m - 2));
    for (int k = 0; k < 2; k += 1) HIP_TRY(d_items[k].need((size_t)m / 2 + 1));
    HIP_TRY(d_status.need(BUILD_STATUS_BYTES));
    std::vector<uint32_t> same(m), type(m, (uint32_t)DRT_GEO_SPHERE);
    for (uint32_t k = 0; k < m; k += 1) same[k] = k;
    HIP_TRY(hipMemcpy(d_keys, sorted_keys, (size_t)m * sizeof(uint64_t), hipMemcpyHostToDevice));
    HIP_TRY(hipMemcpy(d_same, same.data(), (size_t)m * sizeof(uint32_t), hipMemcpyHostToDevice));
    HIP_TRY(hipMemcpy(d_type, type.data(), (size_t)m * sizeof(uint32_t), hipMemcpyHostToDevice));
    HIP_TRY(hipMemset(d_nodes, 0xFF, ((size_t)m - 1) * sizeof(BvhNode)));
    HIP_TRY(hipMemset(d_levels, 0xFF, std::max<size_t>((size_t)m - 2, 1) * sizeof(uint2)));
    BuildTables bt;
    bt.boxes = nullptr;
    bt.tree_surf = d_same;
    bt.bounds = (unsigned long long *)d_status.get();
    bt.level_count = (uint32_t *)(d_status + BUILD_BOUND_WORDS * 8);
    bt.m = m;
    TopologyTables tt;
    tt.keys = d_keys;
    tt.pos = d_same;
    tt.tree_surf = d_same;
    tt.surf_type = d_type;
    tt.nodes = d_nodes;
    tt.leaf = d_leaf;
    tt.leaf_parent = d_leaf_parent;
    tt.order = d_order;
    tt.levels = d_levels;
    tt.level_count = bt.level_count;
    tt.m = m;
    int rc = hierarchy_enqueue_init(0, bt, d_items[0]);
    uint4 *const items[2] = {d_items[0], d_items[1]};
    if (rc || (rc = hierarchy_enqueue_topology(0, tt, items))) return rc;
    HIP_TRY(hipDeviceSynchronize());
    std::vector<BvhNode> nodes((size_t)m - 1);
    HIP_TRY(hipMemcpy(nodes.data(), d_nodes, nodes.size() * sizeof(BvhNode), hipMemcpyDeviceToHost));
    for (size_t i = 0; i < nodes.size(); i += 1)
        for (int c = 0; c < 2; c += 1)
        {
            child[2 * i + c] = nodes[i].child[c];
            count[2 * i + c] = nodes[i].count[c];
        }
    HIP_TRY(hipMemcpy(level_count, bt.level_count, (BUILD_LEVELS + 1) * sizeof(uint32_t), hipMemcpyDeviceToHost));
    if (m > 2u) HIP_TRY(hipMemcpy(levels_out, d_levels, ((size_t)m - 2) * sizeof(uint2), hipMemcpyDeviceToHost));
    return 0;
}

extern "C" int drt_selftest_unit(int device, int func, const double *in, uint32_t in_stride, double *out, uint32_t out_stride, uint64_t n)
{
    g_last_error.clear();
    if (func < 0 || func >= DRT_UNIT_COUNT) return fail(-1, "unknown unit function %d", func);
    if (!in || !out || in_stride == 0 || out_stride == 0) return fail(-1, "null argument");
    static const uint32_t need_in[DRT_UNIT_COUNT] = {10, 18, 6, 8, 6, 1, 1, 7, 10, 3, 4, 1, 12, 20, 12};
    static const uint32_t need_out[DRT_UNIT_COUNT] = {1, 1, 3, 3, 9, 4, 4, 1, 1, 1, 1, 2, 1, 1, 2};
    if (in_stride < need_in[func] || out_stride < need_out[func])
        return fail(-1, "unit function %d needs %u doubles in and %u out per record", func, need_in[func], need_out[func]);
    if (n == 0) return 0;
    HIP_TRY(hipSetDevice(device));
    DevBuf<double> din, dout;
    HIP_TRY(din.need(n * in_stride));
    HIP_TRY(dout.need(n * out_stride));
    HIP_TRY(hipMemcpy(din, in, n * in_stride * 8, hipMemcpyHostToDevice));
    HIP_TRY(hipMemset(dout, 0, n * out_stride * 8));
    hipLaunchKernelGGL(drt_unit_kernel, dim3((unsigned)((n + 255) / 256)), dim3(256), 0, 0, func, din, in_stride, dout, out_stride, n);
    HIP_TRY(hipGetLastError());
    HIP_TRY(hipDeviceSynchronize());
    HIP_TRY(hipMemcpy(out, dout, n * out_stride * 8, hipMemcpyDeviceToHost));
    return 0;
}

static int bdsf_fresnel_kind(uint32_t b)
{
    if (b == DRT_BDSF_fs_dielectric_reflectance_bdsf || b == DRT_BDSF_fs_dielectric_transmittance_bdsf) return 1;
    if (b == DRT_BDSF_fs_conductor_bdsf || b == DRT_BDSF_ct_conductor_bdsf) return 2;
    return 0;
}

static int material_variants(drt_context *ctx)
{
    int rc = spectra_read_back(ctx);
    if (rc) return rc;
    if (ctx->d_mat_variants && !ctx->variants_stale) return 0;
    const uint32_t n_mat = ctx->dsc.n_mat;
    std::vector<DevMaterial> v((size_t)DRT_MAT_VARIANTS * n_mat);
    for (uint32_t k = 0; k < (uint32_t)DRT_MAT_VARIANTS; k += 1)
        for (uint32_t m = 0; m < n_mat; m += 1)
        {
            DevMaterial dm = ctx->host_mats[m];
            if (k < (uint32_t)DRT_NUM_BDSFS)
            {
                memset(dm.bdsfs, 0, sizeof(dm.bdsfs));
                dm.bdsfs[0] = k;
                dm.num_bdsfs = 1;
                dm.bdsf_packed = k;
                dm.needs = bdsf_needs(k);
                dm.vertex_flags = 0;
                const int rows = dm.pair_out == PAIR_NONE ? 0 : (dm.pair_out & PAIR_CONDUCTOR) ? 2 : 1;
                if (rows == 0 || rows != bdsf_fresnel_kind(k)) dm.pair_out = dm.pair_in = PAIR_NONE;
            }
            else dm.dir_func = k - (uint32_t)DRT_NUM_BDSFS;
            v[(size_t)k * n_mat + m] = dm;
        }
    if (!ctx->d_mat_variants)
    {
        DevBuf<unsigned char> buf;
        HIP_TRY(buf.need(v.size() * sizeof(DevMaterial)));
        ctx->d_mat_variants = (DevMaterial *)(unsigned char *)buf;
        ctx->allocations.push_back(std::move(buf));
    }
    HIP_TRY(hipMemcpy(ctx->d_mat_variants, v.data(), v.size() * sizeof(DevMaterial), hipMemcpyHostToDevice));
    ctx->variants_stale = false;
    return 0;
}

extern "C" int drt_selftest_material(drt_context *ctx, int func, const double *in, uint32_t in_stride, double *out, uint32_t out_stride,
                                     uint64_t n)
{
    g_last_error.clear();
    if (!ctx || !in || !out) return fail(-1, "null argument");
    if (func < 0 || func >= DRT_MAT_COUNT) return fail(-1, "unknown material function %d", func);
    const uint32_t S = ctx->dsc.S, n_mat = ctx->dsc.n_mat;
    const uint32_t need_in = func == DRT_MAT_EVALUATE ? DRT_MAT_EVAL_IN : DRT_MAT_SAMPLE_IN;
    const uint32_t need_out = func == DRT_MAT_EVALUATE ? S + 1u : DRT_MAT_SAMPLE_OUT;
    if (in_stride < need_in || out_stride < need_out)
        return fail(-1, "material function %d needs %u doubles in and %u out per record", func, need_in, need_out);
    auto index_ok = [](double x, double lo, double hi) { return x >= lo && x < hi && x == (double)(int64_t)x; };
    for (uint64_t r = 0; r < n; r += 1)
    {
        const double *a = in + r * in_stride;
        for (int k = 10; k < 13; k += 1)
            if (!index_ok(a[k], 0.0, (double)n_mat)) return fail(-1, "record %llu: material index %g (the scene has %u)", (unsigned long long)r, a[k], n_mat);
        const DevMaterial &sm = ctx->host_mats[(uint32_t)a[10]];
        if (func == DRT_MAT_EVALUATE)
        {
            if (!index_ok(a[13], -1.0, (double)DRT_NUM_BDSFS)) return fail(-1, "record %llu: unknown bdsf id %g", (unsigned long long)r, a[13]);
            if (!index_ok(a[17], 0.0, 4.0)) return fail(-1, "record %llu: unknown mode %g", (unsigned long long)r, a[17]);
            if ((uint32_t)a[17] & DRT_MAT_MODE_SIMPLE)
            {
                bool fresnel = a[13] >= 0.0 ? bdsf_fresnel_kind((uint32_t)a[13]) != 0 : false;
                for (uint32_t j = 0; a[13] < 0.0 && j < sm.num_bdsfs; j += 1) fresnel = fresnel || bdsf_fresnel_kind(sm.bdsfs[j]) != 0;
                if (fresnel) return fail(-1, "record %llu: the SIMPLE instantiation has no Fresnel functions", (unsigned long long)r);
            }
        }
        else
        {
            if (!index_ok(a[13], -1.0, (double)DRT_NUM_DIRFS)) return fail(-1, "record %llu: unknown dir_func id %g", (unsigned long long)r, a[13]);
            if (a[13] < 0.0 && sm.dir_func >= (uint32_t)DRT_NUM_DIRFS)
                return fail(-1, "record %llu: material %u has no direction sampler (dir_func %u)", (unsigned long long)r, (uint32_t)a[10], sm.dir_func);
        }
    }
    if (n == 0) return 0;
    HIP_TRY(hipSetDevice(ctx->device));
    int rc = material_variants(ctx);
    if (rc) return rc;
    DevBuf<double> din, dout;
    HIP_TRY(din.need(n * in_stride));
    HIP_TRY(dout.need(n * out_stride));
    HIP_TRY(hipMemcpy(din, in, n * in_stride * 8, hipMemcpyHostToDevice));
    HIP_TRY(hipMemset(dout, 0, n * out_stride * 8));
    hipLaunchKernelGGL(drt_material_kernel, dim3((unsigned)((n + 255) / 256)), dim3(256), 0, 0, ctx->dsc, ctx->d_mat_variants, func, din, in_stride,
                       dout, out_stride, n);
    HIP_TRY(hipGetLastError());
    HIP_TRY(hipDeviceSynchronize());
    HIP_TRY(hipMemcpy(out, dout, n * out_stride * 8, hipMemcpyDeviceToHost));
    return 0;
}
```

daily-ray-trace_amd/pydrt.py:

```python
import ctypes as C
import os
import sys

import numpy as np

HERE = os.path.dirname(os.path.abspath(__file__))
REPO = os.path.dirname(HERE)

DRT_MAX_BDSFS = 16
GEO_POINT, GEO_SPHERE, GEO_PLANE = 1, 2, 3
FILM_SAMPLE_CENTER, FILM_SAMPLE_RANDOM = 1, 2
MODE_SPECTRAL, MODE_XYZ = 0, 1
FLAG_RECORD_HITS = 1
BATCH_RESIDENT = 0xFFFFFFFF
FLAG_FILM_ZERO = 2
PATH_BVH, PATH_TRACE_TAIL, PATH_RAYS, PATH_RAY_STASH = 1, 2, 4, 8

BDSF_NAMES = ["bp_diffuse_bdsf", "bp_glossy_bdsf", "mirror_bdsf", "fs_conductor_bdsf",
              "fs_dielectric_reflectance_bdsf", "fs_dielectric_transmittance_bdsf", "ct_conductor_bdsf"]
DIRF_NAMES = ["cos_weighted_sample_hemisphere", "uniform_sample_hemisphere", "sample_specular_direction",
              "sample_transmit_direction", "sample_reflect_or_transmit_direction", "sample_ct_direction"]
BDSF = {n: i for i, n in enumerate(BDSF_NAMES)}
DIRF = {n: i for i, n in enumerate(DIRF_NAMES)}

# ... 537 lines not shown

_hip = None


def _share_torch_hip_runtime():
    if os.environ.get("DRT_NO_TORCH_RUNTIME") or "torch" in sys.modules:
        return
    try:
        import importlib.util
        spec = importlib.util.find_spec("torch")
    except (ImportError, ValueError):
        return
    if spec is None or not spec.origin:
        return
    cand = os.path.join(os.path.dirname(spec.origin), "lib", "libamdhip64.so")
    if os.path.exists(cand):
        try:
            C.CDLL(cand, mode=C.RTLD_GLOBAL)
        except OSError:
            pass


def hip_lib():
    global _hip
    if _hip is None:
        path = os.environ.get("DRT_HIP_LIB") or os.path.join(HERE, "libdrt_hip.so")
        if not os.path.exists(path):
            raise RuntimeError("libdrt_hip.so is not built (no fallback exists): run __graft_entry__.build()")
        _share_torch_hip_runtime()
        L = C.CDLL(path)
        L.drt_last_error.restype = C.c_char_p
        L.drt_device_count.restype = C.c_int
        L.drt_create.restype = C.c_void_p
        L.drt_create.argtypes = [C.POINTER(Scene), C.POINTER(Camera), C.POINTER(Params)]
        L.drt_destroy.argtypes = [C.c_void_p]
        L.drt_bind_film.argtypes = [C.c_void_p, C.c_void_p, C.c_void_p, C.c_void_p]
        L.drt_set_stream.argtypes = [C.c_void_p, C.c_void_p]
        L.drt_render.argtypes = [C.c_void_p, C.c_uint32, C.c_uint32]
        L.drt_synchronize.argtypes = [C.c_void_p]
        L.drt_reset_film.argtypes = [C.c_void_p]
        L.drt_film_device_ptrs.argtypes = [C.c_void_p, C.POINTER(C.c_void_p), C.POINTER(C.c_void_p), C.POINTER(C.c_void_p)]
        L.drt_read_film.argtypes = [C.c_void_p, C.POINTER(C.c_double), C.POINTER(C.c_double), C.POINTER(C.c_double)]
        L.drt_read_xyz.argtypes = [C.c_void_p, C.POINTER(C.c_double)]
        L.drt_read_bgra.argtypes = [C.c_void_p, C.c_int, C.POINTER(C.c_uint8)]
        L.drt_group_read_bgra.argtypes = [C.c_void_p, C.c_int, C.POINTER(C.c_uint8)]
        f64p, i32p = C.POINTER(C.c_double), C.POINTER(C.c_int32)
        L.drt_group_create.restype = C.c_void_p
        L.drt_group_create.argtypes = [C.POINTER(Scene), C.POINTER(Camera), C.POINTER(Params), i32p, C.c_uint32]
        L.drt_group_destroy.argtypes = [C.c_void_p]
        L.drt_group_destroy.restype = None
        L.drt_group_size.argtypes = [C.c_void_p]
        L.drt_group_size.restype = C.c_uint32
        L.drt_group_render.argtypes = [C.c_void_p, C.c_uint32, C.c_uint32]
        L.drt_group_synchronize.argtypes = [C.c_void_p]
        L.drt_group_read_film.argtypes = [C.c_void_p, f64p, f64p, f64p]
        L.drt_group_write_film.argtypes = [C.c_void_p, f64p, f64p, f64p]
        L.drt_group_get_stats.argtypes = [C.c_void_p, C.POINTER(Stats)]
        L.drt_render_tile_multi.argtypes = [C.POINTER(Scene), C.POINTER(Camera), C.POINTER(Params), i32p, C.c_uint32, f64p, f64p, f64p,
                                            C.POINTER(Stats)]
        L.drt_write_film.argtypes = [C.c_void_p, C.POINTER(C.c_double), C.POINTER(C.c_double), C.POINTER(C.c_double)]
        L.drt_read_hit_indices.argtypes = [C.c_void_p, C.POINTER(C.c_int32), C.c_uint64]
        L.drt_get_stats.argtypes = [C.c_void_p, C.POINTER(Stats)]
        L.drt_render_adaptive.argtypes = [C.c_void_p, C.POINTER(Adaptive)]
        L.drt_read_sample_counts.argtypes = [C.c_void_p, C.POINTER(C.c_uint32)]
        L.drt_read_active_list.argtypes = [C.c_void_p, C.POINTER(C.c_uint32), C.c_uint32, C.POINTER(C.c_uint32)]
        L.drt_group_render_adaptive.argtypes = [C.c_void_p, C.POINTER(Adaptive)]
        L.drt_group_read_sample_counts.argtypes = [C.c_void_p, C.POINTER(C.c_uint32)]
        L.drt_render_adaptive_continue.argtypes = [C.c_void_p, C.POINTER(Adaptive), C.c_uint32, C.POINTER(C.c_uint32)]
        L.drt_group_render_adaptive_continue.argtypes = [C.c_void_p, C.POINTER(Adaptive), C.c_uint32, C.POINTER(C.c_uint32)]
        if hasattr(L, "drt_render_sample_map"):
            L.drt_render_sample_map.argtypes = [C.c_void_p, C.POINTER(SampleMap)]
            L.drt_group_render_sample_map.argtypes = [C.c_void_p, C.POINTER(SampleMap)]
        if hasattr(L, "drt_denoise_film"):
            L.drt_denoise_film.argtypes = [C.c_void_p, C.POINTER(Denoise)]
            L.drt_read_denoised.argtypes = [C.c_void_p, f64p, f64p]
            L.drt_read_denoised_bgra.argtypes = [C.c_void_p, C.POINTER(C.c_uint8)]
            L.drt_denoise_buffers.argtypes = [C.POINTER(Scene), C.POINTER(Params), C.POINTER(Denoise), f64p, f64p, f64p, f64p, f64p]
            L.drt_group_denoise.argtypes = [C.c_void_p, C.POINTER(Denoise), f64p, f64p]
        if hasattr(L, "drt_render_features"):
            L.drt_render_features.argtypes = [C.c_void_p, C.POINTER(Features)]
            L.drt_read_features.argtypes = [C.c_void_p, f64p, f64p, i32p]
            L.drt_read_feature_bgra.argtypes = [C.c_void_p, C.c_int, C.c_double, C.c_double, C.POINTER(C.c_uint8)]
            L.drt_group_render_features.argtypes = [C.c_void_p, C.POINTER(Features), f64p, f64p, i32p]
        if hasattr(L, "drt_cast_rays"):
            vp = C.c_void_p
            L.drt_cast_rays.argtypes = [C.c_void_p, vp, vp, C.c_uint64, vp, C.c_uint32]
            L.drt_test_visibility.argtypes = [C.c_void_p, vp, vp, C.c_uint64, vp, C.c_uint32]
            L.drt_cast_pixels.argtypes = [C.c_void_p, vp, vp, C.c_uint64, vp, vp, vp, C.c_uint32]
            L.drt_group_cast_rays.argtypes = [C.c_void_p, vp, vp, C.c_uint64, vp]
            L.drt_group_test_visibility.argtypes = [C.c_void_p, vp, vp, C.c_uint64, vp]
            L.drt_group_cast_pixels.argtypes = [C.c_void_p, vp, vp, C.c_uint64, vp, vp, vp]
        if hasattr(L, "drt_render_mattes"):
            u32p = C.POINTER(C.c_uint32)
            L.drt_render_mattes.argtypes = [C.c_void_p, C.POINTER(Mattes)]
            L.drt_read_mattes.argtypes = [C.c_void_p, i32p, u32p, u32p]
            L.drt_read_matte.argtypes = [C.c_void_p, C.c_int, i32p, C.c_uint32, f64p]
            L.drt_read_matte_bgra.argtypes = [C.c_void_p, C.c_int, C.POINTER(C.c_uint8)]
            L.drt_group_render_mattes.argtypes = [C.c_void_p, C.POINTER(Mattes), i32p, u32p, u32p]
        L.drt_batch_spp.restype = C.c_uint32
        if hasattr(L, "drt_bind_rays"):
            L.drt_bind_rays.argtypes = [C.c_void_p, C.POINTER(RayTable)]
            L.drt_group_bind_rays.argtypes = [C.c_void_p, C.POINTER(RayTable)]
        L.drt_batch_spp.argtypes = [C.c_void_p]
        if hasattr(L, "drt_shade_instantiation"):
            L.drt_shade_instantiation.argtypes = [C.c_void_p]
            L.drt_shade_instantiation.restype = C.c_int
        if hasattr(L, "drt_update_surfaces"):
            L.drt_set_camera.argtypes = [C.c_void_p, C.POINTER(Camera)]
            L.drt_update_surfaces.argtypes = [C.c_void_p, C.c_void_p, C.c_uint32, C.c_uint32, C.c_uint32]
            L.drt_get_update_report.argtypes = [C.c_void_p, C.POINTER(UpdateReport)]
            L.drt_group_set_camera.argtypes = [C.c_void_p, C.POINTER(Camera)]
            L.drt_group_update_surfaces.argtypes = [C.c_void_p, C.c_void_p, C.c_uint32, C.c_uint32, C.c_uint32]
            L.drt_group_reset_film.argtypes = [C.c_void_p]
        if hasattr(L, "drt_update_spectra"):
            L.drt_update_spectra.argtypes = [C.c_void_p, C.c_void_p, C.c_uint32, C.c_uint32, C.c_uint32]
            L.drt_update_materials.argtypes = [C.c_void_p, C.c_void_p, C.c_uint32, C.c_uint32, C.c_uint32]
            L.drt_group_update_spectra.argtypes = [C.c_void_p, C.c_void_p, C.c_uint32, C.c_uint32, C.c_uint32]
            L.drt_group_update_materials.argtypes = [C.c_void_p, C.c_void_p, C.c_uint32, C.c_uint32, C.c_uint32]
        if hasattr(L, "drt_bind_depth_cuts"):
            u32p, vpp = C.POINTER(C.c_uint32), C.POINTER(C.c_void_p)
            L.drt_bind_depth_cuts.argtypes = [C.c_void_p, u32p, C.c_uint32]
            L.drt_read_depth_film.argtypes = [C.c_void_p, C.c_uint32, f64p, f64p, f64p]
            L.drt_depth_film_device_ptrs.argtypes = [C.c_void_p, C.c_uint32, vpp, vpp, vpp]
            L.drt_read_depth_xyz.argtypes = [C.c_void_p, C.c_uint32, f64p]
            L.drt_read_depth_bgra.argtypes = [C.c_void_p, C.c_uint32, C.c_int, C.POINTER(C.c_uint8)]
            L.drt_group_bind_depth_cuts.argtypes = [C.c_void_p, u32p, C.c_uint32]
            L.drt_group_read_depth_film.argtypes = [C.c_void_p, C.c_uint32, f64p, f64p, f64p]
        if hasattr(L, "drt_rebuild_hierarchy"):
            L.drt_rebuild_hierarchy.argtypes = [C.c_void_p, C.c_uint32]
            L.drt_group_rebuild_hierarchy.argtypes = [C.c_void_p, C.c_uint32]
            L.drt_get_hierarchy_report.argtypes = [C.c_void_p, C.POINTER(HierarchyReport)]
            L.drt_read_hierarchy.argtypes = [C.c_void_p, C.c_void_p, C.c_uint32, C.POINTER(C.c_uint32), C.c_uint32]
        if hasattr(L, "drt_live_window_of"):
            L.drt_live_window_of.argtypes = [C.POINTER(Scene), C.POINTER(Camera), C.POINTER(Params), C.POINTER(C.c_uint32)]
            L.drt_live_window.argtypes = [C.c_void_p, C.POINTER(C.c_uint32)]
        L.drt_render_tile.argtypes = [C.POINTER(Scene), C.POINTER(Camera), C.POINTER(Params), C.POINTER(C.c_double),
                                      C.POINTER(C.c_double), C.POINTER(C.c_double), C.POINTER(Stats)]
        L.drt_selftest_arith.argtypes = [C.c_int, C.c_int, C.POINTER(C.c_double), C.POINTER(C.c_double),
                                         C.POINTER(C.c_double), C.c_uint64]
        if hasattr(L, "drt_selftest_path_ids"):
            L.drt_selftest_path_ids.argtypes = [C.c_int, C.POINTER(C.c_uint64), C.c_uint32, C.POINTER(C.c_uint32), C.c_uint32, C.c_uint32,
                                                C.c_uint32, C.POINTER(C.c_uint64)]
        L.drt_bvh_stats.argtypes = [C.POINTER(Scene)] + [C.POINTER(C.c_uint32)] * 4
        L.drt_selftest_unit.argtypes = [C.c_int, C.c_int, C.POINTER(C.c_double), C.c_uint32, C.POINTER(C.c_double), C.c_uint32,
                                        C.c_uint64]
        L.drt_selftest_material.argtypes = [C.c_void_p, C.c_int, C.POINTER(C.c_double), C.c_uint32, C.POINTER(C.c_double), C.c_uint32,
                                            C.c_uint64]
        if hasattr(L, "drt_selftest_build_sort"):
            u32p, u64p = C.POINTER(C.c_uint32), C.POINTER(C.c_uint64)
            L.drt_selftest_build_sort.argtypes = [C.c_int, u64p, C.c_uint32, u64p, u32p]
            L.drt_selftest_build_topology.argtypes = [C.c_int, u64p, C.c_uint32, C.POINTER(C.c_int32), C.POINTER(C.c_int32), u32p, u32p]
        if hasattr(L, "drt_selftest_live_resources"):
            L.drt_selftest_live_resources.argtypes = [C.POINTER(C.c_uint64)]
        _hip = L
    return _hip


SHADE_INSTANTIATIONS = ("general", "simple", "closed")

HIP_SYMBOLS = ["drt_shade_instantiation",
               "drt_last_error", "drt_device_count", "drt_create", "drt_destroy", "drt_bind_film", "drt_set_stream",
               "drt_render", "drt_synchronize", "drt_reset_film", "drt_film_device_ptrs", "drt_read_film", "drt_write_film",
               "drt_read_xyz", "drt_read_bgra", "drt_read_hit_indices", "drt_get_stats", "drt_batch_spp", "drt_render_tile", "drt_selftest_arith",
               "drt_selftest_unit", "drt_selftest_material", "drt_selftest_path_ids", "drt_bvh_stats",
               "drt_selftest_build_sort", "drt_selftest_build_topology", "drt_selftest_live_resources",
               "drt_group_create", "drt_group_destroy", "drt_group_size", "drt_group_render", "drt_group_synchronize",
               "drt_group_read_film", "drt_group_write_film", "drt_group_read_bgra", "drt_group_get_stats", "drt_render_tile_multi",
               "drt_render_adaptive", "drt_read_sample_counts", "drt_group_render_adaptive", "drt_group_read_sample_counts",
               "drt_read_active_list", "drt_render_adaptive_continue", "drt_group_render_adaptive_continue",
               "drt_denoise_film", "drt_read_denoised", "drt_read_denoised_bgra", "drt_denoise_buffers", "drt_group_denoise",
               "drt_render_features", "drt_read_features", "drt_read_feature_bgra", "drt_group_render_features",
               "drt_render_mattes", "drt_read_mattes", "drt_read_matte", "drt_read_matte_bgra", "drt_group_render_mattes",
               "drt_cast_rays", "drt_test_visibility", "drt_cast_pixels", "drt_group_cast_rays", "drt_group_test_visibility",
               "drt_group_cast_pixels", "drt_bind_rays", "drt_group_bind_rays",
               "drt_set_camera", "drt_update_surfaces", "drt_get_update_report", "drt_group_set_camera", "drt_group_update_surfaces",
               "drt_group_reset_film",
               "drt_rebuild_hierarchy", "drt_group_rebuild_hierarchy", "drt_get_hierarchy_report", "drt_read_hierarchy",
               "drt_update_spectra", "drt_update_materials", "drt_group_update_spectra", "drt_group_update_materials",
               "drt_bind_depth_cuts", "drt_read_depth_film", "drt_depth_film_device_ptrs", "drt_read_depth_xyz", "drt_read_depth_bgra",
               "drt_group_bind_depth_cuts", "drt_group_read_depth_film",
               "drt_render_sample_map", "drt_group_render_sample_map",
               "drt_live_window_of", "drt_live_window"]

MAX_DEPTH_CUTS = 8


def _depth_array(depths):
    depths = [] if depths is None else [int(d) for d in depths]
    if any(d < 0 or d > 0xFFFFFFFF for d in depths):
        raise ValueError("bind_depth_cuts: depths are unsigned 32-bit numbers")
    return ((C.c_uint32 * len(depths))(*depths) if depths else None), len(depths)


def depth_layers(means):
    m = np.asarray(means, dtype=np.float64)
    if m.ndim < 1 or m.shape[0] < 1:
        raise ValueError("depth_layers: at least one cut")
    out = m.copy()
    out[1:] = m[1:] - m[:-1]
    return out


def _check(rc, what):
    if rc != 0:
        raise RuntimeError("%s failed (%d): %s" % (what, rc, hip_lib().drt_last_error().decode()))


def live_window_of(bundle, params, camera=None):
    out = (C.c_uint32 * 4)()
    cam = bundle.camera if camera is None else camera
    _check(hip_lib().drt_live_window_of(C.byref(bundle.scene), C.byref(cam), C.byref(params), out), "drt_live_window_of")
    return tuple(int(v) for v in out)


class Renderer:

    def __init__(self, bundle, params):
        self.L = hip_lib()
        self.bundle = bundle
        self.params = params
        self.S = bundle.S
        self.n_pixels = int(params.tile_w) * int(params.tile_h)
        self.ctx = self.L.drt_create(C.byref(bundle.scene), C.byref(bundle.camera), C.byref(params))
        if not self.ctx:
            raise RuntimeError("drt_create failed: " + self.L.drt_last_error().decode())

    def close(self):
        if self.ctx:
            self.L.drt_destroy(self.ctx)
            self.ctx = None

    def __del__(self):
        try:
            self.close()
        except Exception:
            pass

    def live_window(self):
        out = (C.c_uint32 * 4)()
        _check(self.L.drt_live_window(self.ctx, out), "drt_live_window")
        return tuple(int(v) for v in out)

    def bind_film(self, d_pixels, d_avgs, d_vars):
        _check(self.L.drt_bind_film(self.ctx, d_pixels, d_avgs, d_vars), "drt_bind_film")

    def set_stream(self, stream_handle):
        _check(self.L.drt_set_stream(self.ctx, stream_handle), "drt_set_stream")

    def render(self, first_sample=None, num_samples=None):
        fs = int(self.params.first_sample) if first_sample is None else first_sample
        ns = int(self.params.spp) if num_samples is None else num_samples
        _check(self.L.drt_render(self.ctx, fs, ns), "drt_render")

    def synchronize(self):
        _check(self.L.drt_synchronize(self.ctx), "drt_synchronize")

    def reset_film(self):
        _check(self.L.drt_reset_film(self.ctx), "drt_reset_film")

    def film_device_ptrs(self):
        a, b, c = C.c_void_p(), C.c_void_p(), C.c_void_p()
        _check(self.L.drt_film_device_ptrs(self.ctx, C.byref(a), C.byref(b), C.byref(c)), "drt_film_device_ptrs")
        return a.value, b.value, c.value

    def read_xyz_film(self):
        acc = np.empty((self.n_pixels, 8), dtype=np.float64)
        _check(self.L.drt_read_film(self.ctx, _ptr(acc, C.c_double), None, None), "drt_read_film")
        return acc

    def write_xyz_film(self, acc):
        acc = np.ascontiguousarray(acc, dtype=np.float64)
        _check(self.L.drt_write_film(self.ctx, _ptr(acc, C.c_double), None, None), "drt_write_film")

    def read_film(self):
        px = np.empty((self.n_pixels, self.S + 1), dtype=np.float64)
        av = np.empty((self.n_pixels, self.S), dtype=np.float64)
        va = np.empty((self.n_pixels, self.S), dtype=np.float64)
        _check(self.L.drt_read_film(self.ctx, _ptr(px, C.c_double), _ptr(av, C.c_double), _ptr(va, C.c_double)), "drt_read_film")
        return px, av, va

    def write_film(self, px, av, va):
        px, av, va = (np.ascontiguousarray(a, dtype=np.float64) for a in (px, av, va))
        _check(self.L.drt_write_film(self.ctx, _ptr(px, C.c_double), _ptr(av, C.c_double), _ptr(va, C.c_double)), "drt_write_film")

    def read_xyz(self):
        xyz = np.empty((self.n_pixels, 3), dtype=np.float64)
        _check(self.L.drt_read_xyz(self.ctx, _ptr(xyz, C.c_double)), "drt_read_xyz")
        return xyz

    def read_bgra(self, which=0):
        out = np.empty((self.n_pixels, 4), dtype=np.uint8)
        _check(self.L.drt_read_bgra(self.ctx, int(which), _ptr(out, C.c_uint8)), "drt_read_bgra")
        return out

    def bind_depth_cuts(self, depths):
        arr, n = _depth_array(depths)
        _check(self.L.drt_bind_depth_cuts(self.ctx, arr, n), "drt_bind_depth_cuts")

    def read_depth_film(self, cut):
        px = np.empty((self.n_pixels, self.S + 1), dtype=np.float64)
        av = np.empty((self.n_pixels, self.S), dtype=np.float64)
        va = np.empty((self.n_pixels, self.S), dtype=np.float64)
        _check(self.L.drt_read_depth_film(self.ctx, int(cut), _ptr(px, C.c_double), _ptr(av, C.c_double), _ptr(va, C.c_double)), "drt_read_depth_film")
        return px, av, va

    def depth_film_device_ptrs(self, cut):
        a, b, c = C.c_void_p(), C.c_void_p(), C.c_void_p()
        _check(self.L.drt_depth_film_device_ptrs(self.ctx, int(cut), C.byref(a), C.byref(b), C.byref(c)), "drt_depth_film_device_ptrs")
        return a.value, b.value, c.value

    def read_depth_xyz(self, cut):
        xyz = np.empty((self.n_pixels, 3), dtype=np.float64)
        _check(self.L.drt_read_depth_xyz(self.ctx, int(cut), _ptr(xyz, C.c_double)), "drt_read_depth_xyz")
        return xyz

    def read_depth_bgra(self, cut, which=0):
        out = np.empty((self.n_pixels, 4), dtype=np.uint8)
        _check(self.L.drt_read_depth_bgra(self.ctx, int(cut), int(which), _ptr(out, C.c_uint8)), "drt_read_depth_bgra")
        return out

    def read_hit_indices(self, num_samples):
        n = self.n_pixels * num_samples
        out = np.empty((n, int(self.params.max_depth)), dtype=np.int32)
        _check(self.L.drt_read_hit_indices(self.ctx, _ptr(out, C.c_int32), n), "drt_read_hit_indices")
        return out

    def batch_spp(self):
        return int(self.L.drt_batch_spp(self.ctx))

    def shade_instantiation(self):
        return SHADE_INSTANTIATIONS[int(self.L.drt_shade_instantiation(self.ctx))]

    def stats(self):
        st = Stats()
        _check(self.L.drt_get_stats(self.ctx, C.byref(st)), "drt_get_stats")
# ... 315 lines not shown
    def test_visibility(self, p0, p1):
        a, b = _rays_f64(p0, "p0"), _rays_f64(p1, "p1")
        if a.shape != b.shape:
            raise ValueError("p0 and p1: the same shape")
        vis = np.zeros(a.shape[0], dtype=np.uint8)
        _check(self.L.drt_group_test_visibility(self.g, a.ctypes.data, b.ctypes.data, a.shape[0], vis.ctypes.data), "drt_group_test_visibility")
        return vis

    def cast_pixels(self, xy, samples):
        xy, samples = _pixels_u32(xy, samples)
        n = xy.shape[0]
        o, d, hits = np.zeros((n, 3)), np.zeros((n, 3)), np.zeros(n, dtype=RAY_HIT_DTYPE)
        _check(self.L.drt_group_cast_pixels(self.g, xy.ctypes.data, samples.ctypes.data, n, o.ctypes.data, d.ctypes.data, hits.ctypes.data),
               "drt_group_cast_pixels")
        return o, d, hits

    def bind_rays(self, origins, dirs=None, weights=None):
        if origins is None:
            _check(self.L.drt_group_bind_rays(self.g, None), "drt_group_bind_rays")
            return
        if _is_tensor(origins) or _is_tensor(dirs) or _is_tensor(weights):
            raise ValueError("Group.bind_rays: numpy arrays (a group takes host pointers only)")
        t, _ = _ray_table(origins, dirs, weights, int(self.params.width), int(self.params.height), 0)
        _check(self.L.drt_group_bind_rays(self.g, C.byref(t)), "drt_group_bind_rays")

    def bind_depth_cuts(self, depths):
        arr, n = _depth_array(depths)
        _check(self.L.drt_group_bind_depth_cuts(self.g, arr, n), "drt_group_bind_depth_cuts")

    def read_depth_film(self, cut):
        px = np.empty((self.n_pixels, self.S + 1)); av = np.empty((self.n_pixels, self.S)); va = np.empty((self.n_pixels, self.S))
        f64p = C.POINTER(C.c_double)
        _check(self.L.drt_group_read_depth_film(self.g, int(cut), px.ctypes.data_as(f64p), av.ctypes.data_as(f64p), va.ctypes.data_as(f64p)),
               "drt_group_read_depth_film")
        return px, av, va

    def reset_film(self):
        _check(self.L.drt_group_reset_film(self.g), "drt_group_reset_film")

    def set_camera(self, camera_or_bundle):
        cam = _camera_of(camera_or_bundle)
        _check(self.L.drt_group_set_camera(self.g, C.byref(cam)), "drt_group_set_camera")

    def update_surfaces(self, surfaces, first=0, rebuild=False):
        if _is_tensor(surfaces):
            raise ValueError("Group.update_surfaces: a Surface array or numpy rows (a group takes host pointers only)")
        ptr, n, flags, _keep = _update_args(surfaces, 0)
        _check(self.L.drt_group_update_surfaces(self.g, ptr, first, n, flags | (SURFACES_REBUILD if rebuild else 0)), "drt_group_update_surfaces")

    def update_spectra(self, rows, first=0):
        if _is_tensor(rows):
            raise ValueError("Group.update_spectra: numpy rows (a group takes host pointers only)")
        ptr, n, flags, _keep = _spectra_args(rows, self.S, 0)
        _check(self.L.drt_group_update_spectra(self.g, ptr, first, n, flags), "drt_group_update_spectra")

    def update_materials(self, materials, first=0):
        ptr, n, _keep = _materials_args(materials)
        _check(self.L.drt_group_update_materials(self.g, ptr, first, n, 0), "drt_group_update_materials")

    def rebuild_hierarchy(self):
        _check(self.L.drt_group_rebuild_hierarchy(self.g, 0), "drt_group_rebuild_hierarchy")

    def close(self):
        if self.g:
            self.L.drt_group_destroy(self.g)
            self.g = None


def render_tile(bundle, params):
    L = hip_lib()
    n = int(params.tile_w) * int(params.tile_h)
    S = bundle.S
    px = np.zeros((n, S + 1), dtype=np.float64)
    av = np.zeros((n, S), dtype=np.float64)
    va = np.zeros((n, S), dtype=np.float64)
    st = Stats()
    rc = L.drt_render_tile(C.byref(bundle.scene), C.byref(bundle.camera), C.byref(params), _ptr(px, C.c_double),
                           _ptr(av, C.c_double), _ptr(va, C.c_double), C.byref(st))
    _check(rc, "drt_render_tile")
    return px, av, va, st


def denoise_buffers(bundle, params, pixels, avgs, vars_, radius=5, patch=1, k=1.0, alpha=1.0):
    n, S = int(params.tile_w) * int(params.tile_h), bundle.S
    px = np.ascontiguousarray(pixels, dtype=np.float64).reshape(n, S + 1)
    av = np.ascontiguousarray(avgs, dtype=np.float64).reshape(n, S)
    va = np.ascontiguousarray(vars_, dtype=np.float64).reshape(n, S)
    d = make_denoise(radius, patch, k, alpha)
    mean = np.empty((n, S), dtype=np.float64)
    var = np.empty((n, S), dtype=np.float64)
    _check(hip_lib().drt_denoise_buffers(C.byref(bundle.scene), C.byref(params), C.byref(d), _ptr(px, C.c_double), _ptr(av, C.c_double),
                                         _ptr(va, C.c_double), _ptr(mean, C.c_double), _ptr(var, C.c_double)), "drt_denoise_buffers")
    return mean, var, {"unusable": d.unusable, "kernel_ms": d.kernel_ms}


def selftest_arith(op, a, b=None, device=0):
    a = np.ascontiguousarray(a, dtype=np.float64)
    n = a.size
    b = np.ascontiguousarray(b if b is not None else np.zeros_like(a), dtype=np.float64)
    out = np.empty(2 * n if op == 2 else n, dtype=np.float64)
    _check(hip_lib().drt_selftest_arith(device, op, _ptr(a, C.c_double), _ptr(b, C.c_double), _ptr(out, C.c_double), n),
           "drt_selftest_arith")
    return out


def selftest_path_ids(bases, steps, n_samples, tile_w, device=0):
    bases = np.ascontiguousarray(bases, dtype=np.uint64)
    steps = np.ascontiguousarray(steps, dtype=np.uint32)
    out = np.zeros((bases.size, int(steps.sum()), 4), dtype=np.uint64)
    _check(hip_lib().drt_selftest_path_ids(device, _ptr(bases, C.c_uint64), bases.size, _ptr(steps, C.c_uint32), steps.size, n_samples,
                                           tile_w, _ptr(out, C.c_uint64)), "drt_selftest_path_ids")
    return out


(UNIT_LINE_SPHERE, UNIT_LINE_PLANE, UNIT_REFLECT, UNIT_TRANSMIT, UNIT_ROTATION_BETWEEN, UNIT_SAMPLE_SPHERE, UNIT_SAMPLE_DISC,
 UNIT_GGX, UNIT_GGX_ATT, UNIT_FS_DIELECTRIC, UNIT_FS_CONDUCTOR, UNIT_SEED_AND_DRAW, UNIT_BVH_BOX, UNIT_LINE_PLANE_LIMITED,
 UNIT_BVH_SPHERE) = range(15)
_UNIT_OUT = {UNIT_LINE_SPHERE: 1, UNIT_LINE_PLANE: 1, UNIT_REFLECT: 3, UNIT_TRANSMIT: 3, UNIT_ROTATION_BETWEEN: 9,
             UNIT_SAMPLE_SPHERE: 4, UNIT_SAMPLE_DISC: 4, UNIT_GGX: 1, UNIT_GGX_ATT: 1, UNIT_FS_DIELECTRIC: 1, UNIT_FS_CONDUCTOR: 1,
             UNIT_SEED_AND_DRAW: 2, UNIT_BVH_BOX: 1, UNIT_LINE_PLANE_LIMITED: 1, UNIT_BVH_SPHERE: 2}


MAT_EVALUATE, MAT_SAMPLE = 0, 1
MAT_MODE_UNPAIRED, MAT_MODE_SIMPLE = 1, 2


def selftest_material(renderer, func, records):
    rec = np.ascontiguousarray(records, dtype=np.float64)
    n, k = rec.shape
    m = renderer.S + 1 if func == MAT_EVALUATE else 6
    out = np.zeros((n, m), dtype=np.float64)
    _check(hip_lib().drt_selftest_material(renderer.ctx, func, _ptr(rec, C.c_double), k, _ptr(out, C.c_double), m, n),
           "drt_selftest_material")
    return out


def bvh_stats(bundle):
    v = [C.c_uint32() for _ in range(4)]
    _check(hip_lib().drt_bvh_stats(C.byref(bundle.scene), *[C.byref(x) for x in v]), "drt_bvh_stats")
    return tuple(x.value for x in v)


def selftest_unit(func, records, device=0):
    rec = np.ascontiguousarray(records, dtype=np.float64)
    if rec.ndim == 1:
        rec = rec.reshape(-1, 1)
    n, k = rec.shape
    m = _UNIT_OUT[func]
    out = np.zeros((n, m), dtype=np.float64)
    _check(hip_lib().drt_selftest_unit(device, func, _ptr(rec, C.c_double), k, _ptr(out, C.c_double), m, n), "drt_selftest_unit")
    return out


BUILD_LEVEL_COUNTS = 33


def selftest_build_sort(keys, keys_out=None, pos_out=None, device=0):
    keys = np.ascontiguousarray(keys, dtype=np.uint64)
    m = keys.size
    keys_out = np.zeros(m, dtype=np.uint64) if keys_out is None else keys_out
    pos_out = np.zeros(m, dtype=np.uint32) if pos_out is None else pos_out
    for a, t in ((keys_out, np.uint64), (pos_out, np.uint32)):
        if a.dtype != t or a.shape != (m,) or not a.flags["C_CONTIGUOUS"] or not a.flags["WRITEABLE"]:
            raise ValueError("selftest_build_sort: an output array is not a contiguous %s[%d]" % (np.dtype(t).name, m))
    _check(hip_lib().drt_selftest_build_sort(device, _ptr(keys, C.c_uint64), m, _ptr(keys_out, C.c_uint64), _ptr(pos_out, C.c_uint32)),
           "drt_selftest_build_sort")
    return keys_out, pos_out


def selftest_build_topology(sorted_keys, device=0):
    keys = np.ascontiguousarray(sorted_keys, dtype=np.uint64)
    m = keys.size
    child, count = np.zeros((max(m - 1, 1), 2), dtype=np.int32), np.zeros((max(m - 1, 1), 2), dtype=np.int32)
    level_count = np.zeros(BUILD_LEVEL_COUNTS, dtype=np.uint32)
    levels = np.zeros((max(m - 2, 0), 2), dtype=np.uint32)
    _check(hip_lib().drt_selftest_build_topology(device, _ptr(keys, C.c_uint64), m, _ptr(child, C.c_int32), _ptr(count, C.c_int32),
                                                 _ptr(level_count, C.c_uint32), _ptr(levels, C.c_uint32) if m > 2 else None),
           "drt_selftest_build_topology")
    return child, count, level_count, levels


def selftest_live_resources():
    out = (C.c_uint64 * 4)()
    _check(hip_lib().drt_selftest_live_resources(out), "drt_selftest_live_resources")
    return tuple(int(v) for v in out)



def _xorshift64_stream(seed):
    x = seed & 0xFFFFFFFFFFFFFFFF
    while True:
        x ^= (x << 13) & 0xFFFFFFFFFFFFFFFF
        x ^= x >> 7
        x ^= (x << 17) & 0xFFFFFFFFFFFFFFFF
        yield (x >> 33) / 2147483647.0


def synthetic_sphere_scene(n_spheres, width, height, seed=0x5EED, spectra_dir=None):
    base = load_scene(os.path.join(REPO, "scenes", "cornell_plane_light.scn"), width, height, spectra_dir=spectra_dir)
    names = base.material_names()
    mats = []
    for i in range(int(base.scene.num_materials)):
        m = base.scene.materials[i]
        mats.append({k: getattr(m, k) for k in ("is_black_body", "is_emissive", "shininess", "roughness", "emission_spd",
                                                 "diffuse_spd", "glossy_spd", "mirror_spd", "refract_spd", "extinct_spd",
                                                 "dir_func")} | {"bdsfs": [m.bdsfs[j] for j in range(m.num_bdsfs)]})
    cycle = [names.index(n) for n in ("blue_plastic", "green_plastic", "red_plastic", "white_plastic", "teal_plastic",
                                      "mirror", "gold")]
    g = _xorshift64_stream(seed)
    surfaces = []
    for i in range(n_spheres):
        cx = -20.0 + 40.0 * next(g)
        cy = -20.0 + 40.0 * next(g)
        cz = -40.0 + 40.0 * next(g)
        r = 0.05 + 0.30 * next(g)
        surfaces.append({"type": GEO_SPHERE, "material": cycle[i % len(cycle)], "position": (cx, cy, cz), "radius": r})
    u, v, n = plane_from_points((-5.0, 25.0, 5.0), (5.0, 25.0, 5.0), (-5.0, 25.0, -5.0))
    surfaces.append({"type": GEO_PLANE, "material": names.index("light"), "position": (-5.0, 25.0, 5.0), "u": u, "v": v, "normal": n})
    cam = init_camera((0.0, 0.0, 30.0), (0.0, 0.0, -20.0), 0.0, 60.0, 6.0, 0.3, 0.0, width, height)
    return build_scene(surfaces, mats, base.spds(), int(base.scene.base_material), int(base.scene.escape_material), cam)
```

include/drt_hip.h:

```cpp
#ifndef DRT_HIP_H
#define DRT_HIP_H

#include <stdint.h>

#ifdef __cplusplus
extern "C" {
#endif

#define DRT_MAX_BDSFS 16

enum
{
    DRT_GEO_NONE   = 0,
    DRT_GEO_POINT  = 1,
    DRT_GEO_SPHERE = 2,
    DRT_GEO_PLANE  = 3
};

enum
{
    DRT_FILM_SAMPLE_CENTER = 1,
    DRT_FILM_SAMPLE_RANDOM = 2
};

// ... 168 lines not shown
int drt_group_render(drt_group *g, uint32_t first_sample, uint32_t num_samples);
int drt_group_synchronize(drt_group *g);
int drt_group_read_film(drt_group *g, double *pixels, double *avgs, double *vars);
int drt_group_write_film(drt_group *g, const double *pixels, const double *avgs, const double *vars);
int drt_group_read_bgra(drt_group *g, int which, uint8_t *bgra);
int drt_group_get_stats(drt_group *g, drt_stats *out);
int drt_render_tile_multi(const drt_scene *scene, const drt_camera *camera, const drt_params *params,
                          const int32_t *devices, uint32_t n_devices,
                          double *dst_pixels, double *dst_avgs, double *dst_vars, drt_stats *stats);

typedef struct drt_adaptive
{
    uint32_t min_spp, max_spp, step, flags;
    double   rel_error, floor;
    uint32_t rounds, pixels_at_max;
    uint64_t paths;
} drt_adaptive;
int drt_render_adaptive(drt_context *ctx, drt_adaptive *a);
int drt_read_sample_counts(drt_context *ctx, uint32_t *counts);
int drt_read_active_list(drt_context *ctx, uint32_t *list, uint32_t capacity, uint32_t *count);
int drt_group_render_adaptive(drt_group *g, drt_adaptive *a);
int drt_group_read_sample_counts(drt_group *g, uint32_t *counts);

int drt_render_adaptive_continue(drt_context *ctx, drt_adaptive *a, uint32_t max_rounds, uint32_t *still_active);
int drt_group_render_adaptive_continue(drt_group *g, drt_adaptive *a, uint32_t max_rounds, uint32_t *still_active);

#define DRT_MAP_DEVICE 1u
#define DRT_MAP_ADD    2u
typedef struct drt_sample_map
{
    const uint32_t *targets;
    uint32_t flags;
    uint32_t rounds, pixels_rendered, pixels_above, max_count;
    uint64_t paths;
} drt_sample_map;
int drt_render_sample_map(drt_context *ctx, drt_sample_map *map);
int drt_group_render_sample_map(drt_group *g, drt_sample_map *map);

typedef struct drt_denoise
{
    uint32_t radius, patch, flags;
    uint32_t unusable;
    double   k, alpha;
    double   kernel_ms;
} drt_denoise;
int drt_denoise_film(drt_context *ctx, drt_denoise *d);
int drt_read_denoised(drt_context *ctx, double *mean, double *var);
int drt_read_denoised_bgra(drt_context *ctx, uint8_t *bgra);
int drt_denoise_buffers(const drt_scene *scene, const drt_params *params, drt_denoise *d, const double *pixels, const double *avgs,
                        const double *vars, double *mean, double *var);
int drt_group_denoise(drt_group *g, drt_denoise *d, double *mean, double *var);

#define DRT_FEATURE_CHANNELS 8
typedef struct drt_features
{
    uint32_t n_samples;
    uint32_t first_sample;
    uint32_t flags;
    uint32_t empty_pixels;
    uint64_t rays;
    double   kernel_ms;
} drt_features;
int drt_render_features(drt_context *ctx, drt_features *f);
int drt_read_features(drt_context *ctx, double *mean, double *m2, int32_t *ids);
int drt_read_feature_bgra(drt_context *ctx, int which, double lo, double hi, uint8_t *bgra);
int drt_group_render_features(drt_group *g, drt_features *f, double *mean, double *m2, int32_t *ids);

#define DRT_MATTE_SLOTS   6
#define DRT_MATTE_ID_MISS (-1)
enum { DRT_MATTE_SURFACE = 0, DRT_MATTE_MATERIAL = 1, DRT_MATTE_LAYERS = 2 };
typedef struct drt_mattes
{
    uint32_t n_samples;
    uint32_t first_sample;
    uint32_t flags;
    uint32_t empty_pixels;
    uint32_t overflow_pixels[2];
    uint64_t rays;
    double   kernel_ms;
} drt_mattes;
int drt_render_mattes(drt_context *ctx, drt_mattes *m);
int drt_read_mattes(drt_context *ctx, int32_t *ids, uint32_t *counts, uint32_t *tail);
int drt_read_matte(drt_context *ctx, int layer, const int32_t *id_list, uint32_t n_ids, double *coverage);
int drt_read_matte_bgra(drt_context *ctx, int layer, uint8_t *bgra);
int drt_group_render_mattes(drt_group *g, drt_mattes *m, int32_t *ids, uint32_t *counts, uint32_t *tail);

typedef struct drt_ray_hit
{
    double   position[3], normal[3], out[3];
    double   on_dot;
    double   distance;
    int32_t  index;
    uint32_t surface_material, incident_material, transmit_material;
} drt_ray_hit;

#define DRT_RAYS_DEVICE 1u

int drt_cast_rays(drt_context *ctx, const double *origins, const double *dirs, uint64_t n, drt_ray_hit *hits, uint32_t flags);
int drt_test_visibility(drt_context *ctx, const double *p0, const double *p1, uint64_t n, uint8_t *visible, uint32_t flags);
int drt_cast_pixels(drt_context *ctx, const uint32_t *xy, const uint32_t *samples, uint64_t n, double *origins, double *dirs, drt_ray_hit *hits,
                    uint32_t flags);
int drt_group_cast_rays(drt_group *g, const double *origins, const double *dirs, uint64_t n, drt_ray_hit *hits);
int drt_group_test_visibility(drt_group *g, const double *p0, const double *p1, uint64_t n, uint8_t *visible);
int drt_group_cast_pixels(drt_group *g, const uint32_t *xy, const uint32_t *samples, uint64_t n, double *origins, double *dirs, drt_ray_hit *hits);

typedef struct drt_ray_table
{
    const double *origins, *dirs, *weights;
    uint32_t      n_layers, flags;
} drt_ray_table;
int drt_bind_rays(drt_context *ctx, const drt_ray_table *t);
int drt_group_bind_rays(drt_group *g, const drt_ray_table *t);

#define DRT_MAX_DEPTH_CUTS 8
int drt_bind_depth_cuts(drt_context *ctx, const uint32_t *depths, uint32_t n);
int drt_read_depth_film(drt_context *ctx, uint32_t cut, double *pixels, double *avgs, double *vars);
int drt_depth_film_device_ptrs(drt_context *ctx, uint32_t cut, void **d_pixels, void **d_avgs, void **d_vars);
int drt_read_depth_xyz(drt_context *ctx, uint32_t cut, double *xyz);
int drt_read_depth_bgra(drt_context *ctx, uint32_t cut, int which, uint8_t *bgra);
int drt_group_bind_depth_cuts(drt_group *g, const uint32_t *depths, uint32_t n);
int drt_group_read_depth_film(drt_group *g, uint32_t cut, double *pixels, double *avgs, double *vars);

#define DRT_SURFACES_DEVICE  1u
#define DRT_SURFACES_REBUILD 2u
int drt_set_camera(drt_context *ctx, const drt_camera *camera);
int drt_update_surfaces(drt_context *ctx, const drt_surface *surfaces, uint32_t first, uint32_t count, uint32_t flags);
int drt_group_reset_film(drt_group *g);
int drt_group_set_camera(drt_group *g, const drt_camera *camera);
int drt_group_update_surfaces(drt_group *g, const drt_surface *surfaces, uint32_t first, uint32_t count, uint32_t flags);
typedef struct drt_update_report
{
    uint32_t updates;
    uint32_t refits_since_build;
    double   extent;
    double   kernel_ms;
} drt_update_report;
int drt_get_update_report(drt_context *ctx, drt_update_report *out);

#define DRT_SPECTRA_DEVICE 1u
int drt_update_spectra(drt_context *ctx, const double *rows , uint32_t first_row, uint32_t count, uint32_t flags);
int drt_update_materials(drt_context *ctx, const drt_material *materials, uint32_t first, uint32_t count, uint32_t flags );
int drt_group_update_spectra(drt_group *g, const double *rows, uint32_t first_row, uint32_t count, uint32_t flags );
int drt_group_update_materials(drt_group *g, const drt_material *materials, uint32_t first, uint32_t count, uint32_t flags );

int drt_bvh_stats(const drt_scene *scene, uint32_t *nodes, uint32_t *leaf_surfaces, uint32_t *depth, uint32_t *stack_entries);

int drt_selftest_arith(int device, int op, const double *a, const double *b, double *out, uint64_t n);

int drt_selftest_path_ids(int device, const uint64_t *bases, uint32_t n_draws, const uint32_t *steps, uint32_t n_steps, uint32_t n_samples,
                          uint32_t tile_w, uint64_t *out);

int drt_selftest_unit(int device, int func, const double *in, uint32_t in_stride, double *out, uint32_t out_stride, uint64_t n);

int drt_selftest_material(drt_context *ctx, int func, const double *in, uint32_t in_stride, double *out, uint32_t out_stride, uint64_t n);

int drt_selftest_build_sort(int device, const uint64_t *keys, uint32_t m, uint64_t *keys_out, uint32_t *pos_out);
int drt_selftest_build_topology(int device, const uint64_t *sorted_keys, uint32_t m, int32_t *child, int32_t *count, uint32_t *level_count,
                                uint32_t *levels_out);
int drt_selftest_live_resources(uint64_t out[4]);

int drt_rebuild_hierarchy(drt_context *ctx, uint32_t flags);
int drt_group_rebuild_hierarchy(drt_group *g, uint32_t flags);
typedef struct drt_hierarchy_report
{
    uint32_t nodes, leaf_surfaces;
    uint32_t depth;
    uint32_t device_builds;
    uint32_t built_by;
    uint32_t pad;
    double   kernel_ms;
} drt_hierarchy_report;
int drt_get_hierarchy_report(drt_context *ctx, drt_hierarchy_report *out);
int drt_read_hierarchy(drt_context *ctx, void *nodes, uint32_t n_nodes, uint32_t *leaf_surface, uint32_t n_leaf);

int drt_live_window_of(const drt_scene *scene, const drt_camera *camera, const drt_params *params, uint32_t out[4]);
int drt_live_window(drt_context *ctx, uint32_t out[4]);

#ifdef __cplusplus
}
#endif
#endif
```

Before: 2203.

## Replace f64 divisions with reciprocal multiplies and precomputed glass index ratios

Swaps the RNG divide by 2^31-1 for an exact FMA-based reciprocal multiply, though the BVH path-tracing kernel keeps the division through a false template flag. Vector normalisation now computes one shared reciprocal and reuses it for all three components, falling back to plain division when the scale factors differ. Per-material refraction ratios are precomputed once into LDS at kernel start, and the shadow direction is reused instead of being normalised twice. The aim is to cut expensive f64 divide sequences on the hot path, at the cost of extra code complexity, a wave-wide __any check, and a larger material struct in LDS.

After: 2240, median of 6. +1.7%, better.

```diff
diff --git a/daily-ray-trace_amd/csrc/drt_bvh_kernels.h b/daily-ray-trace_amd/csrc/drt_bvh_kernels.h
--- a/daily-ray-trace_amd/csrc/drt_bvh_kernels.h
+++ b/daily-ray-trace_amd/csrc/drt_bvh_kernels.h
@@ -3,6 +3,9 @@
 #include "drt_kernels.h"
 
 #define BVH_LDS_STACK BVH_STACK
+
+#define BOUNCE_DRAW_BY_RECIPROCAL false
+__device__ __forceinline__ double bounce_rng(uint64_t &state, uint32_t &draws) { return drt_rng<BOUNCE_DRAW_BY_RECIPROCAL>(state, draws); }
 
 struct PrimaryHit
 {
@@ -427,7 +430,7 @@
                 uint32_t camera_draws = 0;
                 V3 ro, rd;
                 if (RAYS) (void)table_ray(rt, tp.width, path_tile_pixel<LIST>(tp, ps), ps.x, ps.y, ps.sample, ro, rd);
-                else camera_ray(cam, tp.pixel_scheme, ps.x, ps.y, rs, camera_draws, ro, rd);
+                else camera_ray<BOUNCE_DRAW_BY_RECIPROCAL>(cam, tp.pixel_scheme, ps.x, ps.y, rs, camera_draws, ro, rd);
                 hdr = headers + ps.slot * REC_HEADER_WORDS;
                 const PrimaryHit ph = primary[ps.slot];
                 hit_point_from_scan(sv, sc, ip, v_sum(ro, v_mul(rd, DRT_VIS_FUDGE)), rd, ph.min_dist, ph.index);
@@ -468,8 +471,8 @@
             }
             else if (ltype == DRT_GEO_SPHERE)
             {
-                double u = drt_rng(rs, n_draws);
-                double v = drt_rng(rs, n_draws);
+                double u = bounce_rng(rs, n_draws);
+                double v = bounce_rng(rs, n_draws);
                 double r = __builtin_sqrt(1.0 - u * u);
                 double t = (2.0 * DRT_PI) * v;
                 double st, ct;
@@ -479,8 +482,8 @@
             }
             else if (ltype == DRT_GEO_PLANE)
             {
-                double u = drt_rng(rs, n_draws);
-                double v = drt_rng(rs, n_draws);
+                double u = bounce_rng(rs, n_draws);
+                double v = bounce_rng(rs, n_draws);
                 V3 lu = v3(sv.lights[LF_UX * sv.n_lights + l], sv.lights[LF_UY * sv.n_lights + l], sv.lights[LF_UZ * sv.n_lights + l]);
                 V3 lv = v3(sv.lights[LF_VX * sv.n_lights + l], sv.lights[LF_VY * sv.n_lights + l], sv.lights[LF_VZ * sv.n_lights + l]);
                 light_position = v_sum(v_sum(lpos, v_mul(lu, u)), v_mul(lv, v));
@@ -557,7 +560,7 @@
             uint64_t *vrec = records + (uint64_t)blk * tp.block_words + (uint64_t)(shaded & (REC_BLOCK_VERTICES - 1u)) * tp.vertex_words;
             V3 in;
             double dir_pdf;
-            sample_direction_by_material(sc, sv, ip, rs, n_draws, in, dir_pdf);
+            sample_direction_by_material<BOUNCE_DRAW_BY_RECIPROCAL>(sc, sv, ip, rs, n_draws, in, dir_pdf);
             EvalCoef e = eval_coefficients_by_material(sc, sv, ip, in);
             vrec[0] = mat.bdsf_packed;
             vrec[1] = (uint64_t)mat.num_bdsfs | ((uint64_t)(e.flags | mat.vertex_flags) << 8) | ((uint64_t)((uint32_t)mat.diffuse_spd & 0xFFFFu) << 16) |
diff --git a/daily-ray-trace_amd/csrc/drt_const_rule.h b/daily-ray-trace_amd/csrc/drt_const_rule.h
--- /dev/null
+++ b/daily-ray-trace_amd/csrc/drt_const_rule.h
@@ -0,0 +1,48 @@
+#ifndef DRT_CONST_RULE_H
+#define DRT_CONST_RULE_H
+
+#include <cstdint>
+
+#if defined(__HIPCC__) || defined(__CUDACC__)
+#define DRT_CONST_FN __host__ __device__ __forceinline__
+#else
+#define DRT_CONST_FN static inline
+#endif
+
+#define DRT_DRAW_DIVISOR 2147483647.0
+#define DRT_DRAW_RECIPROCAL 0x1.00000002p-31
+static_assert(DRT_DRAW_RECIPROCAL == 1.0 / DRT_DRAW_DIVISOR, "R is the double nearest 1 / (2^31 - 1)");
+
+DRT_CONST_FN double drt_draw_quotient(uint32_t n)
+{
+    const double y = (double)n * 0x1p-31;
+    return __builtin_fma(y, DRT_DRAW_RECIPROCAL, y);
+}
+
+struct DrtGlassConst
+{
+    double at_wl;
+    double rel_out[3];
+    double rel_in[3];
+};
+
+DRT_CONST_FN double drt_glass_index(double wl, double w0, double w1, double i0, double i1)
+{
+    return i0 + ((wl - w0) * ((i1 - i0) / (w1 - w0)));
+}
+
+DRT_CONST_FN DrtGlassConst drt_glass_constants(double wl, double w0, double w1, double base_i0, double base_i1, double i0, double i1)
+{
+    DrtGlassConst g;
+    const double base_wl = drt_glass_index(wl, w0, w1, base_i0, base_i1);
+    g.at_wl = drt_glass_index(wl, w0, w1, i0, i1);
+    g.rel_out[0] = base_i0 / i0;
+    g.rel_out[1] = base_i1 / i1;
+    g.rel_out[2] = base_wl / g.at_wl;
+    g.rel_in[0] = i0 / base_i0;
+    g.rel_in[1] = i1 / base_i1;
+    g.rel_in[2] = g.at_wl / base_wl;
+    return g;
+}
+
+#endif
diff --git a/daily-ray-trace_amd/csrc/drt_device.h b/daily-ray-trace_amd/csrc/drt_device.h
--- a/daily-ray-trace_amd/csrc/drt_device.h
+++ b/daily-ray-trace_amd/csrc/drt_device.h
@@ -2,6 +2,15 @@
 
 #include <hip/hip_runtime.h>
 #include <stdint.h>
+#include "drt_const_rule.h"
+
+#ifndef DRT_DRAW_BY_RECIPROCAL
+#define DRT_DRAW_BY_RECIPROCAL 1
+#endif
+
+#ifndef DRT_GLASS_CONSTANTS
+#define DRT_GLASS_CONSTANTS 1
+#endif
 
 #define DRT_PI 3.14159265358979323846
 #define DRT_VIS_FUDGE 0.0001
@@ -26,6 +35,39 @@
 __device__ __forceinline__ V3 v_div(V3 v, double f) { return v3(v.x / f, v.y / f, v.z / f); }
 __device__ __forceinline__ double v_length(V3 v) { return __builtin_sqrt(v_dot(v, v)); }
 __device__ __forceinline__ V3 v_normalise(V3 v) { return v_div(v, v_length(v)); }
+
+#ifndef DRT_SHARED_RCP_DIV
+#define DRT_SHARED_RCP_DIV 1
+#endif
+__device__ __forceinline__ double drt_div_with_rcp(double x, double f, double d, double r)
+{
+    bool flag;
+    const double n = __builtin_amdgcn_div_scale(x, f, true, &flag);
+    double q = n * r;
+    const double t = __builtin_fma(-d, q, n);
+    q = __builtin_amdgcn_div_fmas(t, r, q, flag);
+    return __builtin_amdgcn_div_fixup(q, f, x);
+}
+__device__ __forceinline__ V3 v_div_shared(V3 v, double f)
+{
+#if DRT_SHARED_RCP_DIV
+    bool unused;
+    const double dx = __builtin_amdgcn_div_scale(v.x, f, false, &unused);
+    const double dy = __builtin_amdgcn_div_scale(v.y, f, false, &unused);
+    const double dz = __builtin_amdgcn_div_scale(v.z, f, false, &unused);
+    const long long bx = __double_as_longlong(dx);
+    if (__any(bx != __double_as_longlong(dy) || bx != __double_as_longlong(dz))) return v_div(v, f);
+    double r = __builtin_amdgcn_rcp(dx);
+    double e = __builtin_fma(-dx, r, 1.0);
+    r = __builtin_fma(r, e, r);
+    e = __builtin_fma(-dx, r, 1.0);
+    r = __builtin_fma(r, e, r);
+    return v3(drt_div_with_rcp(v.x, f, dx, r), drt_div_with_rcp(v.y, f, dx, r), drt_div_with_rcp(v.z, f, dx, r));
+#else
+    return v_div(v, f);
+#endif
+}
+__device__ __forceinline__ V3 v_normalise_shared(V3 v) { return v_div_shared(v, v_length(v)); }
 __device__ __forceinline__ V3 v_reverse(V3 v) { return v3(-v.x, -v.y, -v.z); }
 
 __device__ __forceinline__ V3 v_reflect(V3 v, V3 n)
@@ -34,10 +76,9 @@
     return v_sub(v, v_mul(n, f));
 }
 
-__device__ __forceinline__ V3 v_transmit(V3 v, V3 n, double ir, double tr)
+__device__ __forceinline__ V3 v_transmit_rel(V3 v, V3 n, double rel_ref)
 {
     double vn_dot = v_dot(v, n);
-    double rel_ref = ir / tr;
     V3 m = v_mul(n, vn_dot);
     v = v_sub(m, v);
     V3 perpend = v_reverse(v_mul(v, rel_ref));
@@ -45,6 +86,7 @@
     V3 parallel = v_mul(n, perpend_dot);
     return v_sum(perpend, parallel);
 }
+__device__ __forceinline__ V3 v_transmit(V3 v, V3 n, double ir, double tr) { return v_transmit_rel(v, n, ir / tr); }
 
 __device__ __forceinline__ V3 m_vmul(const M33 &m, V3 v)
 {
@@ -91,6 +133,7 @@
     z ^= z >> 31;
     return z ? z : 1ull;
 }
+template <bool BY_RECIPROCAL = (DRT_DRAW_BY_RECIPROCAL != 0)>
 __device__ __forceinline__ double drt_rng(uint64_t &state, uint32_t &draws)
 {
     uint64_t x = state;
@@ -99,6 +142,7 @@
     x ^= x << 17;
     state = x;
     draws += 1;
+    if (BY_RECIPROCAL) return drt_draw_quotient((uint32_t)(x >> 33));
     return (double)(uint32_t)(x >> 33) / 2147483647.0;
 }
 
@@ -128,10 +172,11 @@
     c = (n == 0) ? kc : (n == 1) ? -ks : (n == 2) ? -kc : ks;
 }
 
+template <bool BY_RECIPROCAL = (DRT_DRAW_BY_RECIPROCAL != 0)>
 __device__ __forceinline__ V3 uniform_sample_sphere(uint64_t &rs, uint32_t &draws)
 {
-    double u = drt_rng(rs, draws);
-    double v = drt_rng(rs, draws);
+    double u = drt_rng<BY_RECIPROCAL>(rs, draws);
+    double v = drt_rng<BY_RECIPROCAL>(rs, draws);
     double r = __builtin_sqrt(1.0 - u * u);
     double t = (2.0 * DRT_PI) * v;
     double st, ct;
@@ -139,10 +184,11 @@
     return v3(r * ct, r * st, u);
 }
 
+template <bool BY_RECIPROCAL = (DRT_DRAW_BY_RECIPROCAL != 0)>
 __device__ __forceinline__ V3 uniform_sample_disc(uint64_t &rs, uint32_t &draws)
 {
-    double r_x = drt_rng(rs, draws);
-    double r_y = drt_rng(rs, draws);
+    double r_x = drt_rng<BY_RECIPROCAL>(rs, draws);
+    double r_y = drt_rng<BY_RECIPROCAL>(rs, draws);
     double o_x = 2.0 * r_x - 1.0;
     double o_y = 2.0 * r_y - 1.0;
     if (o_x == 0.0 && o_y == 0.0) return v3(0.0, 0.0, 0.0);
@@ -246,9 +292,8 @@
 }
 
 
-__device__ __forceinline__ double dielectric_reflectance(double ir, double tr, double inc_cos, double inc_sin_sq)
-{
-    double rel = ir / tr;
+__device__ __forceinline__ double dielectric_reflectance_rel(double rel, double ir, double tr, double inc_cos, double inc_sin_sq)
+{
     double ts_sin_sq = rel * rel * inc_sin_sq;
     if (ts_sin_sq >= 1.0) return 1.0;
     double ts_cos = __builtin_sqrt(1.0 - ts_sin_sq * ts_sin_sq);
@@ -261,6 +306,10 @@
     par *= par;
     per *= per;
     return 0.5 * (par + per);
+}
+__device__ __forceinline__ double dielectric_reflectance(double ir, double tr, double inc_cos, double inc_sin_sq)
+{
+    return dielectric_reflectance_rel(ir / tr, ir, tr, inc_cos, inc_sin_sq);
 }
 
 __device__ __forceinline__ double conductor_reflectance(double ir, double tr, double te, double inc_cos, double inc_cos_sq,
diff --git a/daily-ray-trace_amd/csrc/drt_kernels.h b/daily-ray-trace_amd/csrc/drt_kernels.h
--- a/daily-ray-trace_amd/csrc/drt_kernels.h
+++ b/daily-ray-trace_amd/csrc/drt_kernels.h
@@ -59,6 +59,7 @@
     int32_t  emission_spd, diffuse_spd, glossy_spd, mirror_spd, refract_spd, extinct_spd;
     double   shininess, roughness;
     double   refract_i0, refract_i1;
+    DrtGlassConst glass;
     uint32_t bdsfs[DRT_MAX_BDSFS];
     uint64_t bdsf_packed;
     uint32_t vertex_flags;
@@ -223,6 +224,7 @@
     const BvhNode     *bvh_nodes;
     const BvhLeafPrim *bvh_leaf;
     const double      *rows = nullptr;
+    bool               glass_ready = false;
     uint32_t           n_surf, n_lights;
 };
 
@@ -378,9 +380,9 @@
 }
 
 template <bool ROWS = false>
-__device__ __forceinline__ bool points_mutually_visible(const SceneView &sv, V3 p0, V3 p1 DRT_SCAN_STATS_PARAM)
-{
-    V3 dir = v_normalise(v_sub(p1, p0));
+__device__ __forceinline__ bool points_mutually_visible(const SceneView &sv, V3 p0, V3 p1, V3 &dir DRT_SCAN_STATS_PARAM)
+{
+    dir = v_normalise_shared(v_sub(p1, p0));
     V3 o = v_sum(p0, v_mul(dir, DRT_VIS_FUDGE));
     double vis_dist = v_length(v_sub(p1, o)) - DRT_VIS_FUDGE;
     bool visible = true;
@@ -394,6 +396,12 @@
         if (!__any(visible)) break;
     }
     return visible;
+}
+template <bool ROWS = false>
+__device__ __forceinline__ bool points_mutually_visible(const SceneView &sv, V3 p0, V3 p1 DRT_SCAN_STATS_PARAM)
+{
+    V3 dir;
+    return points_mutually_visible<ROWS>(sv, p0, p1, dir DRT_SCAN_STATS_ARG(scan_stats));
 }
 
 struct HitPoint
@@ -449,7 +457,7 @@
         uint32_t type = sv.surf_type[index];
         uint32_t smat = sv.surf_mat[index];
         ip.position = v_sum(ro, v_mul(rd, min_dist));
-        if (type == DRT_GEO_SPHERE) ip.normal = v_normalise(v_sub(ip.position, sf3(sv, SF_PX, index)));
+        if (type == DRT_GEO_SPHERE) ip.normal = v_normalise_shared(v_sub(ip.position, sf3(sv, SF_PX, index)));
         else ip.normal = sf3(sv, SF_NX, index);
         ip.out = v_reverse(rd);
         ip.on_dot = v_dot(ip.normal, ip.out);
@@ -519,9 +527,16 @@
     if (dirs_need_refl(mat)) vd.refl = v_reflect(w, ip.normal);
     if (dirs_need_trans(mat))
     {
-        double ir = refract_at_trans_wl(sc, sv.mats[incident_mat_of(sc, ip)]);
-        double tr = refract_at_trans_wl(sc, sv.mats[transmit_mat_of(sc, ip)]);
-        vd.trans = v_transmit(w, ip.normal, ir, tr);
+        const uint32_t im = incident_mat_of(sc, ip), tm = transmit_mat_of(sc, ip);
+        const bool p_out = im == sc.base_mat && tm == ip.surface_mat, p_in = im == ip.surface_mat && tm == sc.base_mat;
+        double rel;
+        if (DRT_GLASS_CONSTANTS && sv.glass_ready)
+        {
+            rel = p_out ? mat.glass.rel_out[2] : mat.glass.rel_in[2];
+            if (!(p_out || p_in)) rel = sv.mats[im].glass.at_wl / sv.mats[tm].glass.at_wl;
+        }
+        else rel = refract_at_trans_wl(sc, sv.mats[im]) / refract_at_trans_wl(sc, sv.mats[tm]);
+        vd.trans = v_transmit_rel(w, ip.normal, rel);
     }
     return vd;
 }
@@ -541,7 +556,7 @@
     double n_half = 0.0;
     if (needs & (NEED_GLOSSY | NEED_CT))
     {
-        half = v_normalise(v_sum(ip.out, in));
+        half = v_normalise_shared(v_sum(ip.out, in));
         n_half = v_dot(ip.normal, half);
     }
     if (needs & NEED_GLOSSY) e.spec = drt_pow_shininess((0.0 > n_half) ? 0.0 : n_half, mat.shininess);
@@ -583,8 +598,16 @@
         const DevMaterial &im = sv.mats[incident_mat_of(sc, ip)];
         const DevMaterial &tm = sv.mats[transmit_mat_of(sc, ip)];
         double inc_sin_sq = 1.0 - ip.on_dot * ip.on_dot;
-        double r0 = dielectric_reflectance(im.refract_i0, tm.refract_i0, ip.on_dot, inc_sin_sq);
-        double r1 = dielectric_reflectance(im.refract_i1, tm.refract_i1, ip.on_dot, inc_sin_sq);
+        const uint32_t imi = incident_mat_of(sc, ip), tmi = transmit_mat_of(sc, ip);
+        const bool p_out = imi == sc.base_mat && tmi == ip.surface_mat, p_in = imi == ip.surface_mat && tmi == sc.base_mat;
+        double rel0 = p_out ? mat.glass.rel_out[0] : mat.glass.rel_in[0], rel1 = p_out ? mat.glass.rel_out[1] : mat.glass.rel_in[1];
+        if (!(DRT_GLASS_CONSTANTS && sv.glass_ready && (p_out || p_in)))
+        {
+            rel0 = im.refract_i0 / tm.refract_i0;
+            rel1 = im.refract_i1 / tm.refract_i1;
+        }
+        double r0 = dielectric_reflectance_rel(rel0, im.refract_i0, tm.refract_i0, ip.on_dot, inc_sin_sq);
+        double r1 = dielectric_reflectance_rel(rel1, im.refract_i1, tm.refract_i1, ip.on_dot, inc_sin_sq);
         double rd = drt_lerp(sc.trans_wl, sc.trans_w0, sc.trans_w1, r0, r1);
         double f = drt_rng(rs, draws);
         const bool reflect = f < rd;
@@ -701,6 +724,7 @@
     return e;
 }
 
+template <bool DRAW_BY_RECIPROCAL>
 __device__ __forceinline__ void sample_direction_by_material(const DevScene &sc, const SceneView &sv, const HitPoint &ip, uint64_t &rs,
                                                  uint32_t &draws, V3 &dir, double &recip_pdf)
 {
@@ -713,7 +737,7 @@
             V3 q;
             for (;;)
             {
-                q = uniform_sample_disc(rs, draws);
+                q = uniform_sample_disc<DRAW_BY_RECIPROCAL>(rs, draws);
                 if (v_dot(q, q) < 1.0) break;
             }
             q.z = __builtin_sqrt(1.0 - v_dot(q, q));
@@ -724,7 +748,7 @@
         }
         case DRT_DIRF_uniform_sample_hemisphere:
         {
-            V3 s = uniform_sample_sphere(rs, draws);
+            V3 s = uniform_sample_sphere<DRAW_BY_RECIPROCAL>(rs, draws);
             M33 r = rotation_between(zaxis, ip.normal);
             dir = m_vmul(r, s);
             recip_pdf = 2.0 * DRT_PI;
@@ -754,7 +778,7 @@
             double rd = drt_lerp(sc.trans_wl, sc.trans_w0, sc.trans_w1, r0, r1);
             double ir = refract_at_trans_wl(sc, im);
             double tr = refract_at_trans_wl(sc, tm);
-            double f = drt_rng(rs, draws);
+            double f = drt_rng<DRAW_BY_RECIPROCAL>(rs, draws);
             V3 w = v_reverse(ip.out);
             if (f < rd)
             {
@@ -772,8 +796,8 @@
         {
             do
             {
-                double f = drt_rng(rs, draws);
-                double g = drt_rng(rs, draws);
+                double f = drt_rng<DRAW_BY_RECIPROCAL>(rs, draws);
+                double g = drt_rng<DRAW_BY_RECIPROCAL>(rs, draws);
                 double phi_mn = (2.0 * DRT_PI) * g;
                 double tan_mn = (mat.roughness * __builtin_sqrt(f)) / __builtin_sqrt(1.0 - f);
                 double cos_mn = 1.0 / __builtin_sqrt(1.0 + tan_mn * tan_mn);
@@ -811,12 +835,13 @@
     w[3] = (uint64_t)__double_as_longlong(e.ct_coef);
 }
 
+template <bool BY_RECIPROCAL = (DRT_DRAW_BY_RECIPROCAL != 0)>
 __device__ __forceinline__ void camera_ray(const DevCamera &cam, uint32_t scheme, uint32_t x, uint32_t y, uint64_t &rs,
                                            uint32_t &draws, V3 &ro, V3 &rd)
 {
     double px = 0.0, py = 0.0;
     if (scheme == DRT_FILM_SAMPLE_CENTER) { px = 0.5; py = 0.5; }
-    else if (scheme == DRT_FILM_SAMPLE_RANDOM) { px = drt_rng(rs, draws); py = drt_rng(rs, draws); }
+    else if (scheme == DRT_FILM_SAMPLE_RANDOM) { px = drt_rng<BY_RECIPROCAL>(rs, draws); py = drt_rng<BY_RECIPROCAL>(rs, draws); }
     double film_x = ((double)x + px) * cam.pixel_width;
     double film_y = ((double)y + py) * cam.pixel_height;
     V3 bottom = v_mul(cam.up, film_y);
@@ -828,7 +853,7 @@
         focus_dir = v_mul(focus_dir, cam.focal_depth / v_dot(focus_dir, cam.forward));
         V3 focus_point = v_sum(pixel_point, focus_dir);
         M33 r = rotation_between(v3(0.0, 0.0, 1.0), cam.forward);
-        V3 disc_point = v_mul(uniform_sample_disc(rs, draws), cam.aperture_radius);
+        V3 disc_point = v_mul(uniform_sample_disc<BY_RECIPROCAL>(rs, draws), cam.aperture_radius);
         V3 lens_point = m_vmul(r, disc_point);
         ro = v_sum(cam.aperture_position, lens_point);
         rd = v_normalise(v_sub(focus_point, ro));
@@ -1038,6 +1063,13 @@
         uint64_t *dst = (uint64_t *)l_mats;
         for (uint32_t k = threadIdx.x; k < sc.n_mat * (uint32_t)(sizeof(DevMaterial) / 8); k += TRACE_BLOCK) dst[k] = src[k];
         __syncthreads();
+#if DRT_GLASS_CONSTANTS
+        for (uint32_t k = threadIdx.x; k < sc.n_mat; k += TRACE_BLOCK)
+            l_mats[k].glass = drt_glass_constants(sc.trans_wl, sc.trans_w0, sc.trans_w1, l_mats[sc.base_mat].refract_i0, l_mats[sc.base_mat].refract_i1,
+                                                  l_mats[k].refract_i0, l_mats[k].refract_i1);
+        __syncthreads();
+        sv.glass_ready = true;
+#endif
         sv.surf = l_surf;
         sv.lights = l_lights;
         sv.surf_type = l_u32;
@@ -1450,12 +1482,13 @@
                         V3 lv = v3(sv.lights[LF_VX * sv.n_lights + l], sv.lights[LF_VY * sv.n_lights + l], sv.lights[LF_VZ * sv.n_lights + l]);
                         light_position = v_sum(v_sum(lpos, v_mul(lu, u)), v_mul(lv, v));
                     }
-                    bool visible = points_mutually_visible<SCENE_IN_LDS>(sv, ip.position, light_position DRT_SCAN_STATS_ARG(bs + 18));
+                    V3 shadow_dir;
+                    bool visible = points_mutually_visible<SCENE_IN_LDS>(sv, ip.position, light_position, shadow_dir DRT_SCAN_STATS_ARG(bs + 18));
                     uint64_t *lrec = vrec + REC_VERTEX_WORDS + (uint64_t)l * REC_LIGHT_WORDS;
                     uint32_t lflags = 0;
                     if (visible)
                     {
-                        V3 incoming = v_normalise(v_sub(light_position, ip.position));
+                        V3 incoming = shadow_dir;
                         EvalCoef e = eval_coefficients(sv, ip, vd, incoming);
                         lflags = e.flags | FLAG_VISIBLE;
                         if (l == 0 && shaded < 8u) vis0_mask |= 1u << shaded;
@@ -3052,6 +3085,50 @@
 
 enum
 {
+    DRT_DIVISION_SHARED = 0,
+    DRT_DIVISION_DRAW,
+    DRT_DIVISION_COUNT
+};
+#define DRT_DIVISION_SHARED_IN 4
+#define DRT_DIVISION_SHARED_OUT 8
+#define DRT_DIVISION_DRAW_IN 1
+#define DRT_DIVISION_DRAW_OUT 3
+
+__global__ void drt_division_kernel(int func, const double *__restrict__ in, uint32_t in_stride, double *__restrict__ out, uint32_t out_stride,
+                                    uint64_t n)
+{
+    uint64_t i = (uint64_t)blockIdx.x * blockDim.x + threadIdx.x;
+    if (i >= n) return;
+    const double *a = in + i * in_stride;
+    double *o = out + i * out_stride;
+    if (func == DRT_DIVISION_SHARED)
+    {
+        const V3 v = v3(a[0], a[1], a[2]);
+        const double f = a[3];
+        const V3 s = v_div_shared(v, f);
+        const V3 p = v_div(v, f);
+        bool unused;
+        const long long bx = __double_as_longlong(__builtin_amdgcn_div_scale(v.x, f, false, &unused));
+        const long long by = __double_as_longlong(__builtin_amdgcn_div_scale(v.y, f, false, &unused));
+        const long long bz = __double_as_longlong(__builtin_amdgcn_div_scale(v.z, f, false, &unused));
+        const bool differ = bx != by || bx != bz;
+        o[0] = s.x; o[1] = s.y; o[2] = s.z;
+        o[3] = p.x; o[4] = p.y; o[5] = p.z;
+        o[6] = differ ? 0.0 : 1.0;
+        o[7] = (DRT_SHARED_RCP_DIV && !__any(differ)) ? 1.0 : 0.0;
+    }
+    else if (func == DRT_DIVISION_DRAW)
+    {
+        uint64_t rs = (uint64_t)__double_as_longlong(a[0]);
+        uint32_t draws = 0;
+        o[0] = drt_rng(rs, draws);
+        o[1] = (double)(uint32_t)(rs >> 33) / 2147483647.0;
+        o[2] = __longlong_as_double((long long)rs);
+    }
+}
+
+enum
+{
     DRT_MAT_EVALUATE = 0,
     DRT_MAT_SAMPLE,
     DRT_MAT_COUNT
diff --git a/daily-ray-trace_amd/csrc/drt_launcher.hip b/daily-ray-trace_amd/csrc/drt_launcher.hip
--- a/daily-ray-trace_amd/csrc/drt_launcher.hip
+++ b/daily-ray-trace_amd/csrc/drt_launcher.hip
@@ -5294,6 +5294,30 @@
     return 0;
 }
 
+extern "C" int drt_selftest_division(int device, int func, const double *in, uint32_t in_stride, double *out, uint32_t out_stride, uint64_t n)
+{
+    g_last_error.clear();
+    if (func < 0 || func >= DRT_DIVISION_COUNT) return fail(-1, "unknown division function %d", func);
+    if (!in || !out) return fail(-1, "null argument");
+    static const uint32_t need_in[DRT_DIVISION_COUNT] = {DRT_DIVISION_SHARED_IN, DRT_DIVISION_DRAW_IN};
+    static const uint32_t need_out[DRT_DIVISION_COUNT] = {DRT_DIVISION_SHARED_OUT, DRT_DIVISION_DRAW_OUT};
+    if (in_stride < need_in[func] || out_stride < need_out[func])
+        return fail(-1, "division function %d needs %u doubles in and %u out per record", func, need_in[func], need_out[func]);
+    if (n == 0) return 0;
+    if (n > BUILD_SELFTEST_MAX) return fail(-1, "drt_selftest_division: %llu records, more than %u", (unsigned long long)n, BUILD_SELFTEST_MAX);
+    HIP_TRY(hipSetDevice(device));
+    DevBuf<double> din, dout;
+    HIP_TRY(din.need(n * in_stride));
+    HIP_TRY(dout.need(n * out_stride));
+    HIP_TRY(hipMemcpy(din, in, n * in_stride * 8, hipMemcpyHostToDevice));
+    HIP_TRY(hipMemset(dout, 0, n * out_stride * 8));
+    hipLaunchKernelGGL(drt_division_kernel, dim3((unsigned)((n + 255) / 256)), dim3(256), 0, 0, func, din, in_stride, dout, out_stride, n);
+    HIP_TRY(hipGetLastError());
+    HIP_TRY(hipDeviceSynchronize());
+    HIP_TRY(hipMemcpy(out, dout, n * out_stride * 8, hipMemcpyDeviceToHost));
+    return 0;
+}
+
 static int bdsf_fresnel_kind(uint32_t b)
 {
     if (b == DRT_BDSF_fs_dielectric_reflectance_bdsf || b == DRT_BDSF_fs_dielectric_transmittance_bdsf) return 1;
diff --git a/daily-ray-trace_amd/pydrt.py b/daily-ray-trace_amd/pydrt.py
--- a/daily-ray-trace_amd/pydrt.py
+++ b/daily-ray-trace_amd/pydrt.py
@@ -713,6 +713,9 @@
             L.drt_selftest_build_topology.argtypes = [C.c_int, u64p, C.c_uint32, C.POINTER(C.c_int32), C.POINTER(C.c_int32), u32p, u32p]
         if hasattr(L, "drt_selftest_live_resources"):
             L.drt_selftest_live_resources.argtypes = [C.POINTER(C.c_uint64)]
+        if hasattr(L, "drt_selftest_division"):
+            L.drt_selftest_division.argtypes = [C.c_int, C.c_int, C.POINTER(C.c_double), C.c_uint32, C.POINTER(C.c_double), C.c_uint32,
+                                                C.c_uint64]
         _hip = L
     return _hip
 
@@ -741,7 +744,7 @@
                "drt_bind_depth_cuts", "drt_read_depth_film", "drt_depth_film_device_ptrs", "drt_read_depth_xyz", "drt_read_depth_bgra",
                "drt_group_bind_depth_cuts", "drt_group_read_depth_film",
                "drt_render_sample_map", "drt_group_render_sample_map",
-               "drt_live_window_of", "drt_live_window"]
+               "drt_live_window_of", "drt_live_window", "drt_selftest_division"]
 
 MAX_DEPTH_CUTS = 8
 
@@ -1363,6 +1366,21 @@
     return out
 
 
+DIVISION_SHARED, DIVISION_DRAW = 0, 1
+_DIVISION_OUT = {DIVISION_SHARED: 8, DIVISION_DRAW: 3}
+
+
+def selftest_division(func, records, device=0):
+    rec = np.ascontiguousarray(records, dtype=np.float64)
+    if rec.ndim == 1:
+        rec = rec.reshape(-1, 1)
+    n, k = rec.shape
+    m = _DIVISION_OUT[func]
+    out = np.zeros((n, m), dtype=np.float64)
+    _check(hip_lib().drt_selftest_division(device, func, _ptr(rec, C.c_double), k, _ptr(out, C.c_double), m, n), "drt_selftest_division")
+    return out
+
+
 BUILD_LEVEL_COUNTS = 33
 
 
diff --git a/include/drt_hip.h b/include/drt_hip.h
--- a/include/drt_hip.h
+++ b/include/drt_hip.h
@@ -344,6 +344,8 @@
 
 int drt_selftest_unit(int device, int func, const double *in, uint32_t in_stride, double *out, uint32_t out_stride, uint64_t n);
 
+int drt_selftest_division(int device, int func, const double *in, uint32_t in_stride, double *out, uint32_t out_stride, uint64_t n);
+
 int drt_selftest_material(drt_context *ctx, int func, const double *in, uint32_t in_stride, double *out, uint32_t out_stride, uint64_t n);
 
 int drt_selftest_build_sort(int device, const uint64_t *keys, uint32_t m, uint64_t *keys_out, uint32_t *pos_out);
```
